# HengyiWang/spann3r

Measured on AMD Instinct MI355X. Metric: frames/sec/GPU (224px, 10-frame seq) + mem-bank cross-attn HBM GB/s, higher is better.
Workload: dtype bf16; 1 GPU; Spann3R.forward, 10-frame 224x224 sequence, batch 1, ViT-L enc / ViT-B dec / DPT heads, eval memory policy; parallelism=sequences sharded 1/GPU x1, hip_graphs=True

## Files before the change

include/spann3r_hip.h:

```cpp
#ifndef SPANN3R_HIP_H
#define SPANN3R_HIP_H

#include <stdint.h>

#ifdef __cplusplus
extern "C" {
#endif

enum { SP3_F32 = 0, SP3_BF16 = 1 };
enum { SP3_ACT_NONE = 0, SP3_ACT_GELU = 1, SP3_ACT_RELU = 2 };
enum { SP3_EPI_PLAIN = 0, SP3_EPI_ROPE_VT = 1, SP3_EPI_PIXSHUF = 2, SP3_EPI_PARTIAL = 3 };
enum { SP3_LOAD_PLAIN = 0, SP3_LOAD_CONV3X3 = 1, SP3_LOAD_SOFTMAX = 2 };

const char* sp3_last_error(void);
int sp3_version(void);

typedef struct sp3_gemm_desc {
  const float* A;
  const float* A2;
  const void* W;
  void* C;
  const float* bias;
  const float* res1;
  const float* res2;
  int32_t M, N, K;
  int32_t batch;
  int32_t K1;
  int64_t lda, lda2, ldw, ldc, ldr1, ldr2;
  int64_t strideA, strideW, strideC;
  float alpha;
  int32_t wdtype;
  int32_t act;
  int32_t out_bf16;
  int32_t relu_in;
  int32_t loader;
  int32_t conv_H, conv_W, conv_C, conv_OH, conv_OW, conv_stride;
  int32_t epi;
  const float* rope_cos;
  const float* rope_sin;
  const int32_t* pos;
  int32_t rope_cols;
  void* vt;
  int32_t tokens;
  int32_t heads;
  int64_t vt_ld;
  int32_t ps_k, ps_H, ps_W, ps_C;
  int32_t tile;
  int32_t a_bf16;
  int32_t splitk;
  int32_t a_packed;
  const float* ln_stats;
  const float* ln_s;
  int32_t ln_nt;
  int32_t ln_C;
  float ln_eps;
  float* stats_out;
  void* c2;
  int32_t qkv_packed;
  int32_t out_packed;
  int32_t w_packed;
  int64_t sb_A2, sb_bias, sb_ln_stats, sb_ln_s, sb_stats_out, sb_c2, sb_vt;
  int64_t* trace;
  float* sm_stats_out;
  const float* sm_stats;
  int32_t sm_nt;
  float sm_thresh;
  float* sm_zout;
  int32_t f32x3;
  int32_t res_bf16;
  const int32_t* dyn_n;
  int32_t res2_up_H, res2_up_W;
} sp3_gemm_desc;
int sp3_gemm(const sp3_gemm_desc* desc_host, void* stream);
int sp3_gemm_n(const sp3_gemm_desc* const* descs, int n, void* stream);
int sp3_gemm_plan_n(const sp3_gemm_desc* const* descs, int n, int* tiles);
int sp3_gemm_plan(const sp3_gemm_desc* desc_host);

int sp3_layernorm(const float* x, int64_t ldx, const float* gamma, const float* beta, float eps,
                  void* out, int64_t ldo, int out_bf16, int rows, int C, void* stream);
int sp3_layernorm_packed(const float* x, int64_t ldx, const float* gamma, const float* beta, float eps,
                         void* out, int out_bf16, int rows, int C, void* stream);
int sp3_layernorm_dual(const float* x, int64_t ldx, const float* gamma, const float* beta, float eps, float* out, int64_t ldo,
                       void* out_packed_bf16, int rows, int C, int group_rows, int group_rows_pad, void* stream);
int sp3_layernorm_t(const float* x, int64_t ldx, const float* gamma, const float* beta, float eps,
                    void* out, int64_t ldo, int out_bf16, int rows, int C, void* stream);

typedef struct sp3_reduce_ln_desc {
  const float* partial;
  int64_t split_stride;
  const float* bias;
  const float* res;
  int64_t ldres;
  float* x_out;
  int64_t ldx;
  const float* g1; const float* b1; void* out1; int64_t ld1; int32_t out1_bf16;
  const float* g2; const float* b2; void* out2; int64_t ld2; int32_t out2_bf16;
  float eps;
  int32_t splits, rows, C;
  int32_t out1_packed, out2_packed;
  int32_t act;
  const float* res2;
  int64_t ldres2;
} sp3_reduce_ln_desc;
int sp3_reduce_ln(const sp3_reduce_ln_desc* desc_host, void* stream);

int sp3_rope_2d(void* tokens, int dtype, int B, int N, int H, int D, int64_t sB, int64_t sN, int64_t sH,
                const int64_t* positions, float base, float fwd, void* stream);

int sp3_attention(const void* q, int64_t sq, int64_t ldq, const void* k, int64_t sk, int64_t ldk,
                  const void* vt, int64_t vt_ld, void* out, int64_t ldo, int out_bf16,
                  int B, int heads, int Nq, int Nk, float scale, int dtype, void* stream);
int sp3_attention_ex(const void* q, int64_t sq, int64_t ldq, const void* k, int64_t sk, int64_t ldk,
                     const void* vt, int64_t vt_ld, void* out, int64_t ldo, int out_bf16, int out_packed,
                     int B, int heads, int Nq, int Nk, float scale, int dtype, void* stream);

int sp3_attention_packed(const void* qp, int q_cols, int q_col0, int npad_q, const void* kp, int k_cols, int k_col0, int npad_k,
                         const void* vtp, void* out, int64_t ldo, int out_bf16, int out_packed,
                         int B, int heads, int Nq, int Nk, float scale, int o_group, int o_group_rows, void* stream);

typedef struct sp3_attn_qproj_desc {
  const void* x_packed; int64_t x_group_stride;
  const float* ln_stats; int64_t stats_group_stride;
  const void* w_packed; int64_t w_group_stride;
  const float* ln_s; const float* bias; int64_t vec_group_stride;
  const int32_t* pos; const float* rope_cos; const float* rope_sin;
  float ln_eps; int32_t D;
  const void* kp; int32_t k_cols, k_col0, npad_k; const void* vtp;
  void* out; int64_t ldo; int32_t out_bf16, out_packed;
  int32_t B, heads, Nq, Nk; float scale; int32_t o_group, o_group_rows;
} sp3_attn_qproj_desc;
int sp3_attention_packed_qproj(const sp3_attn_qproj_desc* desc_host, void* stream);

typedef struct sp3_bank_write_desc {
  const float* feat_k;
  const float* feat_v;
  float* k_raw;
  float* v_raw;
  void* k_hat;
  void* v_hat_t;
  float* s_bank;
  float* b_bank;
  const float *gamma_k, *beta_k, *gamma_v, *beta_v, *gamma_q, *beta_q;
  float eps;
  float alpha;
  int32_t M, P, C, cap;
  int32_t wdtype;
  const int32_t* state;
} sp3_bank_write_desc;
int sp3_bank_write(const sp3_bank_write_desc* desc_host, void* stream);
int sp3_softmax_thresh(const float* S, float* P, int64_t ld, int64_t strideS, int rows, int M, int Mpad,
                       float thresh, int batch, void* P_packed, int64_t stride_packed, int packed_bf16, void* stream);
int sp3_softmax_pack(const float* S, int64_t ld, int64_t strideS, int rows, int M, float thresh, int batch, void* P_packed,
                     int64_t stride_packed, int packed_bf16, float* rowstat_ws, void* stream);
int sp3_colsum_accum(const float* P, int64_t ld, int rows, int M, float* mem_attn, void* stream);
int sp3_colsum_packed(const void* P_packed, int packed_bf16, int rows, int M, float* mem_attn, void* stream);
int sp3_colsum_softmax(const float* S, int64_t ld, int rows, int M, const float* rowz, float thresh, float* mem_attn,
                       float* mem_count, int append_P, void* stream);
int sp3_pack_stats(const float* x, int64_t ldx, int rows, int C, void* packed, int packed_bf16, float* stats, void* stream);
int sp3_gather_packed_rows(const void* src, void* dst, const int32_t* sel, int n_sel, int C, int elem_size, void* stream);
int sp3_gather_packed_cols(const void* src, void* dst, const int32_t* sel, int n_sel, int n_fill, int C, int cap,
                           int elem_size, void* stream);
int sp3_cos_sim(const float* k, const float* wm, int T, int P, int C, float* scratch, float* score, void* stream);
int sp3_bank_state_set(int32_t* state, int M, int wm, void* stream);
int sp3_prob_merge(const float* stats, float* scale, int rows, int M, int cap, const int32_t* dyn_n, void* stream);
int sp3_colsum_prob(const void* P_packed, const float* scale, int rows, int M, int cap, const int32_t* dyn_n, float* mem_attn, void* stream);
int sp3_cos_sim_state(const float* k, const float* k_raw, int Tmax, int P, int C, const int32_t* state, float* scratch, float* score,
                      void* stream);
int sp3_mem_append(float* count, float* attn, int M, int P, void* stream);
int sp3_prune_select(const float* attn, const float* count, int M, float protect, int top_k,
                     int32_t* sel, void* stream);
int sp3_gather_rows(const void* src, void* dst, const int32_t* sel, int n_sel, int C, int elem_size, void* stream);
int sp3_gather_cols(const void* src, int64_t ld_src, void* dst, int64_t ld_dst, const int32_t* sel, int n_sel,
                    int n_fill, int C, int elem_size, void* stream);
int sp3_gather_1d(const float* src, float* dst, const int32_t* sel, int n_sel, void* stream);

int sp3_conv3x3_tile(const void* x, int in_bf16, const void* w_packed, const float* bias, const float* res1,
                     const float* res2, void* out, int out_bf16, int B, int H, int W, int Cin, int Cout,
                     int relu_in, int act, void* stream);
int sp3_im2col_patch(const float* img, int64_t sb, int64_t sc, int64_t sy, int64_t sx, int B, int C, int H, int W,
                     int p, void* out, int out_bf16, int out_packed, void* stream);
int sp3_upsample2x(const float* in, float* out, int B, int H, int W, int C, int outH, int outW, void* stream);
int sp3_upsample2x_bf16(const void* in, void* out, int B, int H, int W, int C, int outH, int outW, void* stream);
int sp3_head_final(const float* feat, const float* w, const float* b, int64_t pixels, int C, float* pts,
                   float* conf, float* raw, void* stream);
int sp3_head_final_bf16(const void* feat, const float* w, const float* b, int64_t pixels, int C, float* pts, float* conf,
                        float* raw, void* stream);

int sp3_preprocess_image(const uint8_t* src, int64_t src_row_stride, int crop_l, int crop_t, int H1, int W1,
                         const int32_t* hbounds, const int32_t* hcoef, int hksize, int W2,
                         const int32_t* vbounds, const int32_t* vcoef, int vksize, int H2,
                         int crop2_l, int crop2_t, int outW, int outH, int transpose, uint8_t* tmp, float* out, void* stream);

int64_t sp3_conf_loss_ws_bytes(int n, int B);
int sp3_conf_loss_forward(const float* P, const float* Cf, const float* G, const uint8_t* V, const float* pose0, int n, int B, int HW,
                          float alpha, int fix_first, void* ws, float* out7, float* ent_out, void* stream);
int sp3_conf_loss_backward(const float* P, const float* Cf, const float* G, const uint8_t* V, const float* pose0, int n, int B, int HW,
                           float alpha, int fix_first, const void* ws, const float* grad_scale2, float* dP, float* dC, void* stream);
int64_t sp3_ssi_loss_ws_bytes(int n, int B, int HW);
int sp3_ssi_loss_forward(const float* P, const float* G, const uint8_t* V, const float* pose0, int n, int B, int HW, int fix_first,
                         int gt_scale, void* ws, float* out, void* stream);

int sp3_transpose(const float* src, int64_t ld_src, float* dst, int64_t ld_dst, int rows, int cols, void* stream);
int sp3_transpose_batched(const float* src, int64_t ld_src, int64_t stride_src, float* dst, int64_t ld_dst, int64_t stride_dst, int rows,
                          int cols, int batch, void* stream);
int sp3_transpose_pad(const float* src, int64_t ld_src, int64_t stride_src, float* dst, int64_t ld_dst, int64_t stride_dst, int rows,
                      int cols, int batch, int pad_to, void* stream);
int sp3_gelu(const float* x, float* y, int64_t n, void* stream);
int sp3_gelu_bwd(const float* x, const float* dy, float* dx, int64_t n, void* stream);
int sp3_im2col3x3(const float* x, float* col, int B, int H, int W, int C, int stride, void* stream);
int sp3_col2im3x3(const float* dcol, float* dx, int B, int H, int W, int C, int stride, void* stream);
int sp3_relu(const float* x, float* y, int64_t n, void* stream);
int sp3_relu_bwd(const float* x, const float* dy, float* dx, int64_t n, void* stream);
int sp3_upsample2x_bwd(const float* dy, float* dx, int B, int H, int W, int C, int outH, int outW, void* stream);
int sp3_postprocess(const float* raw, float* pts, float* conf, int64_t M, void* stream);
int sp3_postprocess_bwd(const float* raw, const float* dpts, const float* dconf, float* draw, int64_t M, void* stream);
int sp3_adamw(float* p, const float* g, float* m, float* v, int64_t n, float lr, float beta1, float beta2, float eps, float weight_decay,
              int step, float grad_scale, void* stream);
int sp3_mul(const float* a, const float* b, float* out, int64_t n, void* stream);
int sp3_pack_bf16(const float* src, int64_t ld, int rows, int cols, void* dst, void* dstT, void* stream);
int sp3_pack_bf16_conv3x3(const float* x, int B, int H, int W, int C, int stride, int act, void* dst, void* dstT, void* stream);
int sp3_pack_bf16_act(const float* src, int64_t ld, int rows, int cols, void* dst, void* dstT, int act, void* stream);
int sp3_pack_bf16_colsum(const float* src, int64_t ld, int rows, int cols, void* dst, void* dstT, float* colsum, int accumulate,
                         float* partial_ws, void* stream);
int64_t sp3_sumsq_blocks(int64_t n);
int64_t sp3_colsum_rows_ws(int rows, int N);
int sp3_colsum_rows(const float* x, int64_t ld, int rows, int N, float* out, int accumulate, float* scratch, void* stream);
int sp3_sumsq_partial(const float* g, int64_t n, double* partial, void* stream);
int sp3_clip_coef(const double* partial, int count, float max_norm, float extra_scale, float* out, int* step_counter, void* stream);
int sp3_adamw_flat(float* p, const float* g, float* m, float* v, int64_t n, const float* chunk_table, float lr, float beta1, float beta2,
                   float eps, int step, const float* grad_scale_dev, float grad_scale, const int* step_dev, const float* lr_dev, void* stream);
int sp3_softmax_bwd(const float* A, const float* dAd, const float* mask, float* dS, int64_t ld, int rows, int T, float alpha, void* stream);
int sp3_softmax_bwd_pad(const float* A, const float* dAd, const float* mask, float* dS, int64_t ld, int rows, int T, int Tpad, float alpha,
                        void* stream);
typedef struct sp3_head_part {
  const float* src;
  int64_t s_b, s_n, s_h;
  float* dst;
  int64_t d_b, d_n, d_h;
  float* dstT;
  const int64_t* pos;
  int32_t N;
  float fwd;
  int64_t ldT;
} sp3_head_part;
int sp3_head_shuffle(const sp3_head_part* parts, int nparts, int B, int H, int hd, float rope_base, const float* cos_tab,
                     const float* sin_tab, int tab_len, void* stream);
int sp3_attention_train_fwd(const float* q, int64_t sq, int64_t ldq, const float* k, int64_t sk, int64_t ldk, const float* vt, int64_t vt_ld,
                            float* out, int64_t ldo, float* lse, int B, int heads, int Nq, int Nk, float scale, int bf16_products, void* stream);
typedef struct sp3_attn_bwd_desc {
  const float *q, *k, *v, *dout;
  int64_t sq, ldq, sk, ldk, sv, ldv, sdo, lddo;
  const float *qT, *kT, *doT;
  int64_t ldTq, ldTk;
  const float* lse;
  float* D;
  float *dq, *dk, *dv;
  int64_t sdq, lddq, sdk, lddk, sdv, lddv;
  int32_t B, heads, Nq, Nk;
  float scale;
  int32_t bf16_products;
} sp3_attn_bwd_desc;
int sp3_attention_train_bwd(const sp3_attn_bwd_desc* d, void* stream);
int sp3_layernorm_bwd(const float* x, int64_t ldx, const float* gamma, const float* dy, int64_t ldy, const float* dx_add, int64_t ld_add,
                      float* dx, int64_t ld_dx, float* dgamma, float* dbeta, int accumulate, float* scratch, int rows, int C, float eps,
                      void* stream);

int sp3_focal_weiszfeld(const float* pts3d, int B, int H, int W, float ppx, float ppy, int iters, float focal_min, float focal_max,
                        float* focal, void* stream);
int sp3_conf_filter(const float* conf, const float* pts, const float* rgb, int64_t n, float thresh, int* scratch, int64_t* total,
                    float* out_pts, float* out_rgb, void* stream);

int sp3_pnp_dlt_accum(const float* pts, int F, int H, int W, float focal, float cx, float cy, const float* norm4, const float* Rt,
                      float thresh, int cv_mode, double* out41, void* stream);
int sp3_pnp_gn_accum(const float* pts, int F, int H, int W, float focal, float cx, float cy, const double* Rt, const float* Rt_mask,
                     float thresh, double* out29, void* stream);
int sp3_pnp_score(const float* pts, int F, int H, int W, float focal, float cx, float cy, const float* Rt, int n_hyp, float thresh,
                  int cv_mode, int* counts, void* stream);

int sp3_copy_multi(int n, const void* const* src, void* const* dst, const int64_t* bytes, void* stream);
int sp3_copy2d_f32(const float* src, int64_t lds, float* dst, int64_t ldd, int rows, int cols, void* stream);
int sp3_fill_f32(float* p, float v, int64_t n, void* stream);
int sp3_cast_f32_to_bf16(const float* src, void* dst, int64_t n, void* stream);
int sp3_spin(int64_t cycles, int64_t* ticks_100mhz, void* stream);

#ifdef __cplusplus
}
#endif
#endif
```

spann3r_amd/csrc/dpt.hip:

```cpp
#include "common.h"
#include <math.h>

namespace {

__global__ __launch_bounds__(256) void im2col_patch_kernel(const float* __restrict__ img, int64_t sb, int64_t sc, int64_t sy,
                                                           int64_t sx, int C, int H, int W, int p, void* __restrict__ out,
                                                           int out_bf16, int out_packed, int64_t total) {
  const int64_t idx = (int64_t)blockIdx.x * 256 + threadIdx.x;
  if (idx >= total) return;
  const int K = C * p * p;
  const int64_t row = idx / K;
  const int k = (int)(idx - row * K);
  const int nw = W / p, nh = H / p;
  const int b = (int)(row / (nh * nw));
  const int rem = (int)(row - (int64_t)b * nh * nw);
  const int ty = rem / nw, tx = rem - ty * nw;
  const int c = k / (p * p), r2 = k - c * p * p;
  const int iy = r2 / p, ix = r2 - iy * p;
  const float val = img[b * sb + c * sc + (int64_t)(ty * p + iy) * sy + (int64_t)(tx * p + ix) * sx];
  const int64_t o = out_packed ? packed_off((int)row, k, K, out_bf16 != 0) : idx;
  if (out_bf16) reinterpret_cast<__bf16*>(out)[o] = (__bf16)val;
  else reinterpret_cast<float*>(out)[o] = val;
}

__device__ __forceinline__ float4 ld4(const float* p) { return *reinterpret_cast<const float4*>(p); }
__device__ __forceinline__ float4 ld4(const __bf16* p) {
  const bf16x4 t = *reinterpret_cast<const bf16x4*>(p);
  return make_float4((float)t[0], (float)t[1], (float)t[2], (float)t[3]);
}
__device__ __forceinline__ void st4(float* p, const float4 v) { st_out(reinterpret_cast<float4*>(p), v); }
__device__ __forceinline__ void st4(__bf16* p, const float4 v) {
  bf16x4 t;
  t[0] = (__bf16)v.x; t[1] = (__bf16)v.y; t[2] = (__bf16)v.z; t[3] = (__bf16)v.w;
  st_out(reinterpret_cast<bf16x4*>(p), t);
}

template <typename T>
__global__ __launch_bounds__(256) void upsample2x_kernel(const T* __restrict__ in, T* __restrict__ out, int H, int W,
                                                         int C, int outH, int outW, int64_t total4) {
  const int64_t idx = (int64_t)blockIdx.x * 256 + threadIdx.x;
  if (idx >= total4) return;
  const int c4 = C >> 2;
  const int cc = (int)(idx % c4);
  int64_t pix = idx / c4;
  const int ox = (int)(pix % outW);
  pix /= outW;
  const int oy = (int)(pix % outH);
  const int b = (int)(pix / outH);
  const int OH = 2 * H, OW = 2 * W;
  const float sh = OH > 1 ? (float)(H - 1) / (float)(OH - 1) : 0.f;
  const float sw = OW > 1 ? (float)(W - 1) / (float)(OW - 1) : 0.f;
  const float fy = sh * (float)oy, fx = sw * (float)ox;
  int y0 = (int)fy, x0 = (int)fx;
  y0 = y0 < H - 1 ? y0 : H - 1;
  x0 = x0 < W - 1 ? x0 : W - 1;
  const int y1 = y0 < H - 1 ? y0 + 1 : y0, x1 = x0 < W - 1 ? x0 + 1 : x0;
  const float ly = fy - (float)y0, lx = fx - (float)x0;
  const float hy = 1.f - ly, hx = 1.f - lx;
  const T* base = in + (int64_t)b * H * W * C;
  const float4 v00 = ld4(base + (((int64_t)y0 * W + x0) * c4 + cc) * 4);
  const float4 v01 = ld4(base + (((int64_t)y0 * W + x1) * c4 + cc) * 4);
  const float4 v10 = ld4(base + (((int64_t)y1 * W + x0) * c4 + cc) * 4);
  const float4 v11 = ld4(base + (((int64_t)y1 * W + x1) * c4 + cc) * 4);
  float4 o;
  o.x = hy * (hx * v00.x + lx * v01.x) + ly * (hx * v10.x + lx * v11.x);
  o.y = hy * (hx * v00.y + lx * v01.y) + ly * (hx * v10.y + lx * v11.y);
  o.z = hy * (hx * v00.z + lx * v01.z) + ly * (hx * v10.z + lx * v11.z);
  o.w = hy * (hx * v00.w + lx * v01.w) + ly * (hx * v10.w + lx * v11.w);
  st4(out + idx * 4, o);
}

__global__ __launch_bounds__(256) void upsample2x_bf16x8_kernel(const __bf16* __restrict__ in, __bf16* __restrict__ out, int H, int W,
                                                                int C, int outH, int outW) {
  const int c8 = C >> 3;
  const int t = blockIdx.x * 256 + threadIdx.x;
  if (t >= outW * c8) return;
  const int ox = t / c8, cg = t - ox * c8;
  const int oy = blockIdx.y, b = blockIdx.z;
  const int OH = 2 * H, OW = 2 * W;
  const float sh = OH > 1 ? (float)(H - 1) / (float)(OH - 1) : 0.f;
  const float sw = OW > 1 ? (float)(W - 1) / (float)(OW - 1) : 0.f;
  const float fy = sh * (float)oy, fx = sw * (float)ox;
  int y0 = (int)fy, x0 = (int)fx;
  y0 = y0 < H - 1 ? y0 : H - 1;
  x0 = x0 < W - 1 ? x0 : W - 1;
  const int y1 = y0 < H - 1 ? y0 + 1 : y0, x1 = x0 < W - 1 ? x0 + 1 : x0;
  const float ly = fy - (float)y0, lx = fx - (float)x0;
  const float hy = 1.f - ly, hx = 1.f - lx;
  const __bf16* base = in + (int64_t)b * H * W * C + cg * 8;
  const bf16x8 v00 = *reinterpret_cast<const bf16x8*>(base + ((int64_t)y0 * W + x0) * C);
  const bf16x8 v01 = *reinterpret_cast<const bf16x8*>(base + ((int64_t)y0 * W + x1) * C);
  const bf16x8 v10 = *reinterpret_cast<const bf16x8*>(base + ((int64_t)y1 * W + x0) * C);
  const bf16x8 v11 = *reinterpret_cast<const bf16x8*>(base + ((int64_t)y1 * W + x1) * C);
  bf16x8 o;
#pragma unroll
  for (int e = 0; e < 8; ++e)
    o[e] = (__bf16)(hy * (hx * (float)v00[e] + lx * (float)v01[e]) + ly * (hx * (float)v10[e] + lx * (float)v11[e]));
  st_out(reinterpret_cast<bf16x8*>(out + (((int64_t)b * outH + oy) * outW + ox) * C + cg * 8), o);
}

template <typename T>
__global__ __launch_bounds__(256) void head_final_kernel(const T* __restrict__ feat, const float* __restrict__ w,
                                                         const float* __restrict__ bias, int64_t pixels, int C,
                                                         float* __restrict__ pts, float* __restrict__ conf,
                                                         float* __restrict__ raw) {
  const int64_t gid = (int64_t)blockIdx.x * 256 + threadIdx.x;
  const int64_t pix = gid >> 3;
  const int sub = (int)(gid & 7);
  const bool valid = pix < pixels;
  const int64_t pp = valid ? pix : pixels - 1;
  float a0 = 0.f, a1 = 0.f, a2 = 0.f, a3 = 0.f;
  const T* f = feat + pp * C;
  for (int c = sub * 4; c < C; c += 32) {
    const float4 x = ld4(f + c);
    const float4 w0 = *reinterpret_cast<const float4*>(w + c);
    const float4 w1 = *reinterpret_cast<const float4*>(w + C + c);
    const float4 w2 = *reinterpret_cast<const float4*>(w + 2 * C + c);
    const float4 w3 = *reinterpret_cast<const float4*>(w + 3 * C + c);
    a0 += (x.x * w0.x + x.y * w0.y) + (x.z * w0.z + x.w * w0.w);
    a1 += (x.x * w1.x + x.y * w1.y) + (x.z * w1.z + x.w * w1.w);
    a2 += (x.x * w2.x + x.y * w2.y) + (x.z * w2.z + x.w * w2.w);
    a3 += (x.x * w3.x + x.y * w3.y) + (x.z * w3.z + x.w * w3.w);
  }
#pragma unroll
  for (int o = 1; o < 8; o <<= 1) {
    a0 += __shfl_xor(a0, o); a1 += __shfl_xor(a1, o); a2 += __shfl_xor(a2, o); a3 += __shfl_xor(a3, o);
  }
  if (valid && sub == 0) {
    const float x = a0 + bias[0], y = a1 + bias[1], z = a2 + bias[2], c = a3 + bias[3];
    if (raw) { raw[pix * 4 + 0] = x; raw[pix * 4 + 1] = y; raw[pix * 4 + 2] = z; raw[pix * 4 + 3] = c; }
    const float d = sqrtf(x * x + y * y + z * z);
    const float sc = expm1f(d) / fmaxf(d, 1e-8f);
    pts[pix * 3 + 0] = x * sc; pts[pix * 3 + 1] = y * sc; pts[pix * 3 + 2] = z * sc;
    conf[pix] = 1.0f + expf(c);
  }
}

template <int LP, int PPT>
__global__ __launch_bounds__(256) void head_final_bf16x8_kernel(const __bf16* __restrict__ feat, const float* __restrict__ w,
                                                                const float* __restrict__ bias, int64_t pixels, float* __restrict__ pts,
                                                                float* __restrict__ conf, float* __restrict__ raw) {
  constexpr int C = 8 * LP, PPB = 256 / LP;
  const int li = threadIdx.x % LP, pl = threadIdx.x / LP;
  float wr[4][8];
#pragma unroll
  for (int f = 0; f < 4; ++f) {
    const float4 a = *reinterpret_cast<const float4*>(w + f * C + li * 8), b = *reinterpret_cast<const float4*>(w + f * C + li * 8 + 4);
    wr[f][0] = a.x; wr[f][1] = a.y; wr[f][2] = a.z; wr[f][3] = a.w; wr[f][4] = b.x; wr[f][5] = b.y; wr[f][6] = b.z; wr[f][7] = b.w;
  }
  const float b0 = bias[0], b1 = bias[1], b2 = bias[2], b3 = bias[3];
  const int64_t p0 = (int64_t)blockIdx.x * PPB * PPT + pl;
  bf16x8 x[PPT];
#pragma unroll
  for (int q = 0; q < PPT; ++q) {
    int64_t pix = p0 + (int64_t)q * PPB;
    pix = pix < pixels ? pix : pixels - 1;
    x[q] = *reinterpret_cast<const bf16x8*>(feat + pix * C + li * 8);
  }
#pragma unroll
  for (int q = 0; q < PPT; ++q) {
    const int64_t pix = p0 + (int64_t)q * PPB;
    float a[4];
#pragma unroll
    for (int f = 0; f < 4; ++f) {
      float t0 = 0.f, t1 = 0.f;
#pragma unroll
      for (int e = 0; e < 4; ++e) { t0 = fmaf((float)x[q][e], wr[f][e], t0); t1 = fmaf((float)x[q][4 + e], wr[f][4 + e], t1); }
      a[f] = t0 + t1;
    }
#pragma unroll
    for (int o = 1; o < LP; o <<= 1) {
      a[0] += __shfl_xor(a[0], o); a[1] += __shfl_xor(a[1], o); a[2] += __shfl_xor(a[2], o); a[3] += __shfl_xor(a[3], o);
    }
    if (li == 0 && pix < pixels) {
      const float X = a[0] + b0, Y = a[1] + b1, Z = a[2] + b2, Cc = a[3] + b3;
      if (raw) *reinterpret_cast<float4*>(raw + pix * 4) = make_float4(X, Y, Z, Cc);
      const float d = sqrtf(X * X + Y * Y + Z * Z);
      const float sc = expm1f(d) / fmaxf(d, 1e-8f);
      pts[pix * 3 + 0] = X * sc; pts[pix * 3 + 1] = Y * sc; pts[pix * 3 + 2] = Z * sc;
      conf[pix] = 1.0f + expf(Cc);
    }
  }
}

}

#define ST(s) reinterpret_cast<hipStream_t>(s)

extern "C" int sp3_im2col_patch(const float* img, int64_t sb, int64_t sc, int64_t sy, int64_t sx, int B, int C, int H, int W,
                                int p, void* out, int out_bf16, int out_packed, void* stream) {
  SP3_CHECK(img && out && B > 0 && C > 0 && p > 0, "sp3_im2col_patch: bad arguments");
  SP3_CHECK(H % p == 0 && W % p == 0, "Input image size (%d,%d) is not a multiple of patch size (%d)", H, W, p);
  const int64_t total = (int64_t)B * (H / p) * (W / p) * C * p * p;
  hipLaunchKernelGGL(im2col_patch_kernel, dim3((unsigned)((total + 255) / 256)), dim3(256), 0, ST(stream), img, sb, sc, sy, sx,
                     C, H, W, p, out, out_bf16, out_packed, total);
  SP3_LAUNCH_CHECK("sp3_im2col_patch");
  return 0;
}

extern "C" int sp3_upsample2x(const float* in, float* out, int B, int H, int W, int C, int outH, int outW, void* stream) {
  SP3_CHECK(in && out && B > 0 && H > 0 && W > 0 && C > 0 && C % 4 == 0, "sp3_upsample2x: bad arguments");
  SP3_CHECK(outH > 0 && outH <= 2 * H && outW > 0 && outW <= 2 * W, "sp3_upsample2x: bad crop");
  const int64_t total4 = (int64_t)B * outH * outW * (C / 4);
  hipLaunchKernelGGL(upsample2x_kernel<float>, dim3((unsigned)((total4 + 255) / 256)), dim3(256), 0, ST(stream), in, out, H, W, C,
                     outH, outW, total4);
  SP3_LAUNCH_CHECK("sp3_upsample2x");
  return 0;
}

extern "C" int sp3_upsample2x_bf16(const void* in, void* out, int B, int H, int W, int C, int outH, int outW, void* stream) {
  SP3_CHECK(in && out && B > 0 && H > 0 && W > 0 && C > 0 && C % 4 == 0, "sp3_upsample2x_bf16: bad arguments");
  SP3_CHECK(outH > 0 && outH <= 2 * H && outW > 0 && outW <= 2 * W, "sp3_upsample2x_bf16: bad crop");
  if (C % 8 == 0 && outH <= 65535 && B <= 65535) {
    hipLaunchKernelGGL(upsample2x_bf16x8_kernel, dim3((unsigned)((outW * (C / 8) + 255) / 256), outH, B), dim3(256), 0, ST(stream),
                       reinterpret_cast<const __bf16*>(in), reinterpret_cast<__bf16*>(out), H, W, C, outH, outW);
    SP3_LAUNCH_CHECK("sp3_upsample2x_bf16");
    return 0;
  }
  const int64_t total4 = (int64_t)B * outH * outW * (C / 4);
  hipLaunchKernelGGL(upsample2x_kernel<__bf16>, dim3((unsigned)((total4 + 255) / 256)), dim3(256), 0, ST(stream),
                     reinterpret_cast<const __bf16*>(in), reinterpret_cast<__bf16*>(out), H, W, C, outH, outW, total4);
  SP3_LAUNCH_CHECK("sp3_upsample2x_bf16");
  return 0;
}

extern "C" int sp3_head_final(const float* feat, const float* w, const float* b, int64_t pixels, int C, float* pts, float* conf,
                              float* raw, void* stream) {
  SP3_CHECK(feat && w && b && pts && conf && pixels > 0 && C > 0 && C % 32 == 0, "sp3_head_final: bad arguments");
  const int64_t threads = pixels * 8;
  hipLaunchKernelGGL(head_final_kernel<float>, dim3((unsigned)((threads + 255) / 256)), dim3(256), 0, ST(stream), feat, w, b, pixels, C,
                     pts, conf, raw);
  SP3_LAUNCH_CHECK("sp3_head_final");
  return 0;
}

extern "C" int sp3_head_final_bf16(const void* feat, const float* w, const float* b, int64_t pixels, int C, float* pts, float* conf,
                                   float* raw, void* stream) {
  SP3_CHECK(feat && w && b && pts && conf && pixels > 0 && C > 0 && C % 32 == 0, "sp3_head_final_bf16: bad arguments");
  if (C == 128 && (reinterpret_cast<uintptr_t>(feat) & 15) == 0 && (reinterpret_cast<uintptr_t>(w) & 15) == 0 && (!raw || (reinterpret_cast<uintptr_t>(raw) & 15) == 0)) {
    constexpr int LP = 16, PPT = 4, PPB = 256 / LP;
    hipLaunchKernelGGL((head_final_bf16x8_kernel<LP, PPT>), dim3((unsigned)((pixels + PPB * PPT - 1) / (PPB * PPT))), dim3(256), 0, ST(stream),
                       reinterpret_cast<const __bf16*>(feat), w, b, pixels, pts, conf, raw);
    SP3_LAUNCH_CHECK("sp3_head_final_bf16");
    return 0;
  }
  const int64_t threads = pixels * 8;
  hipLaunchKernelGGL(head_final_kernel<__bf16>, dim3((unsigned)((threads + 255) / 256)), dim3(256), 0, ST(stream),
                     reinterpret_cast<const __bf16*>(feat), w, b, pixels, C, pts, conf, raw);
  SP3_LAUNCH_CHECK("sp3_head_final_bf16");
  return 0;
}
```

spann3r_amd/csrc/memory.hip:

```cpp
#include "common.h"
#include <math.h>

namespace {

__device__ __forceinline__ float block_reduce_max(float v, float* sh) {
  v = wave_max(v);
  const int lane = threadIdx.x & 63, w = threadIdx.x >> 6;
  __syncthreads();
  if (lane == 0) sh[w] = v;
  __syncthreads();
  float r = sh[0];
  for (int i = 1; i < (int)(blockDim.x >> 6); ++i) r = fmaxf(r, sh[i]);
  return r;
}
__device__ __forceinline__ float block_reduce_sum(float v, float* sh) {
  v = wave_sum(v);
  const int lane = threadIdx.x & 63, w = threadIdx.x >> 6;
  __syncthreads();
  if (lane == 0) sh[w] = v;
  __syncthreads();
  float r = sh[0];
  for (int i = 1; i < (int)(blockDim.x >> 6); ++i) r += sh[i];
  return r;
}
// ... 8 lines not shown
  for (int j = threadIdx.x; j < M; j += 256) {
    const float v = s[j];
    if (v > mx) { sum = sum * expf(mx - v) + 1.0f; mx = v; }
    else sum += expf(v - mx);
  }
  const float gmx = block_reduce_max(mx, sh);
  sum = block_reduce_sum(mx == -INFINITY ? 0.f : sum * expf(mx - gmx), sh);
  mx = gmx;
  float inv = 1.0f / sum, rk = 1.0f;
  if (thresh > 0.f) {
    float kept = 0.f;
    for (int j = threadIdx.x; j < M; j += 256) {
      float v = expf(s[j] - mx) * inv;
      v = v < thresh ? 0.f : v;
      kept += v;
    }
    rk = block_reduce_sum(kept, sh);
  }
  auto prob = [&](int j) -> float {
    float v = expf(s[j] - mx) * inv;
    if (thresh > 0.f) v = (v < thresh ? 0.f : v) / rk;
    return v;
  };
  if (P) {
    float* p = P + (int64_t)blockIdx.y * strideS + (int64_t)blockIdx.x * ld;
    for (int j = threadIdx.x; j < M; j += 256) p[j] = prob(j);
    for (int j = M + threadIdx.x; j < Mpad; j += 256) p[j] = 0.f;
  }
  if (Pk) {
    constexpr int E = 16 / (int)sizeof(TP);
    TP* pk = Pk + (int64_t)blockIdx.y * stridePk;
    const int row = blockIdx.x;
    for (int j0 = threadIdx.x * E; j0 < Kp; j0 += 256 * E) {
      TP o[E];
#pragma unroll
      for (int e = 0; e < E; ++e) o[e] = (TP)((j0 + e) < M ? prob(j0 + e) : 0.f);
      typedef __attribute__((ext_vector_type(4))) unsigned int u4;
      *reinterpret_cast<u4*>(pk + packed_off(row, j0, Kp, sizeof(TP) == 2)) = *reinterpret_cast<const u4*>(o);
    }
  }
}

__global__ __launch_bounds__(256) void softmax_rowstat_kernel(const float* __restrict__ S, int64_t ld, int64_t strideS, int rows, int M, float thresh,
                                                              float4* __restrict__ rowstat) {
  __shared__ float sh[8];
  const float* s = S + (int64_t)blockIdx.y * strideS + (int64_t)blockIdx.x * ld;
  const bool vec = ((ld & 3) == 0) && ((reinterpret_cast<uintptr_t>(S) & 15) == 0) && ((strideS & 3) == 0);
  const int M4 = vec ? (M & ~3) : 0;
  float mx = -INFINITY, sum = 0.f;
  auto upd = [&](float v) {
    if (v > mx) { sum = sum * __expf(mx - v) + 1.0f; mx = v; }
    else sum += __expf(v - mx);
  };
  for (int j = threadIdx.x * 4; j < M4; j += 1024) {
    const float4 v = *reinterpret_cast<const float4*>(s + j);
    const float m4 = fmaxf(fmaxf(v.x, v.y), fmaxf(v.z, v.w));
    if (m4 > mx) { sum *= __expf(mx - m4); mx = m4; }
    sum += (__expf(v.x - mx) + __expf(v.y - mx)) + (__expf(v.z - mx) + __expf(v.w - mx));
  }
  for (int j = M4 + threadIdx.x; j < M; j += 256) upd(s[j]);
  const float gmx = block_reduce_max(mx, sh);
  sum = block_reduce_sum(mx == -INFINITY ? 0.f : sum * __expf(mx - gmx), sh);
  const float inv = 1.0f / sum;
  float rk = 1.0f;
  if (thresh > 0.f) {
    float kept = 0.f;
    for (int j = threadIdx.x * 4; j < M4; j += 1024) {
      const float4 v = *reinterpret_cast<const float4*>(s + j);
      const float p[4] = {__expf(v.x - gmx) * inv, __expf(v.y - gmx) * inv, __expf(v.z - gmx) * inv, __expf(v.w - gmx) * inv};
#pragma unroll
      for (int e = 0; e < 4; ++e) kept += p[e] < thresh ? 0.f : p[e];
    }
    for (int j = M4 + threadIdx.x; j < M; j += 256) { const float p = __expf(s[j] - gmx) * inv; kept += p < thresh ? 0.f : p; }
    rk = 1.0f / block_reduce_sum(kept, sh);
  }
  if (threadIdx.x == 0) rowstat[(int64_t)blockIdx.y * rows + blockIdx.x] = make_float4(gmx, inv, rk, 0.f);
}

template <typename TP>
__global__ __launch_bounds__(256) void softmax_pack_kernel(const float* __restrict__ S, int64_t ld, int64_t strideS, int rows, int M, int Kp,
                                                           float thresh, const float4* __restrict__ rowstat, TP* __restrict__ Pk,
                                                           int64_t stridePk) {
  constexpr int E = 16 / (int)sizeof(TP), KB = 8 * E;
  const int t = threadIdx.x & 127, kb = blockIdx.x * 2 + (threadIdx.x >> 7), nkb = Kp / KB;
  if (kb >= nkb) return;
  const int h = t >> 6, g = (t >> 4) & 3, r = t & 15;
  const int row = blockIdx.y * 16 + r;
  const int k0 = kb * KB + g * 2 * E + h * E;
  float p[E];
#pragma unroll
  for (int e = 0; e < E; ++e) p[e] = 0.f;
  if (row < rows && k0 < M) {
    const float* s = S + (int64_t)blockIdx.z * strideS + (int64_t)row * ld + k0;
    const float4 st = rowstat[(int64_t)blockIdx.z * rows + row];
    float v[E];
    if (k0 + E <= M && ((reinterpret_cast<uintptr_t>(s) & 15) == 0)) {
#pragma unroll
      for (int q = 0; q < E / 4; ++q) {
        const float4 x = reinterpret_cast<const float4*>(s)[q];
        v[4 * q] = x.x; v[4 * q + 1] = x.y; v[4 * q + 2] = x.z; v[4 * q + 3] = x.w;
      }
    } else {
#pragma unroll
      for (int e = 0; e < E; ++e) v[e] = (k0 + e) < M ? s[e] : -INFINITY;
    }
#pragma unroll
    for (int e = 0; e < E; ++e) {
      float q = __expf(v[e] - st.x) * st.y;
      if (thresh > 0.f) q = (q < thresh ? 0.f : q) * st.z;
      p[e] = (k0 + e) < M ? q : 0.f;
    }
  }
  TP o[E];
#pragma unroll
  for (int e = 0; e < E; ++e) o[e] = (TP)p[e];
  typedef __attribute__((ext_vector_type(4))) unsigned int u4;
  TP* dst = Pk + (int64_t)blockIdx.z * stridePk + (((int64_t)blockIdx.y * nkb + kb) * 128 + t) * E;
  *reinterpret_cast<u4*>(dst) = *reinterpret_cast<const u4*>(o);
}

template <typename TP>
__global__ __launch_bounds__(256) void colsum_packed_kernel(const TP* __restrict__ Pk, int rows, int M, int Kp,
                                                            float* __restrict__ mem_attn) {
  constexpr int E = 16 / (int)sizeof(TP), KB = 8 * E, TPB = 2048 / 16;
  __shared__ float sh[2][KB][17];
  const int kb = blockIdx.x, nkb = Kp / KB, nrb = (rows + 15) / 16;
  const int t = threadIdx.x & (TPB - 1), half_wg = threadIdx.x / TPB;
  const int h = t >> 6, l = t & 63, g = l >> 4, r = l & 15;
  float acc[E];
#pragma unroll
  for (int e = 0; e < E; ++e) acc[e] = 0.f;
  for (int rb = half_wg; rb < nrb; rb += 2) {
    typedef __attribute__((ext_vector_type(4))) unsigned int u4;
    const u4 raw = *reinterpret_cast<const u4*>(reinterpret_cast<const char*>(Pk) + ((int64_t)rb * nkb + kb) * 2048 + t * 16);
    const TP* v = reinterpret_cast<const TP*>(&raw);
    const bool ok = rb * 16 + r < rows;
#pragma unroll
    for (int e = 0; e < E; ++e) acc[e] += ok ? (float)v[e] : 0.f;
  }
#pragma unroll
  for (int e = 0; e < E; ++e) sh[half_wg][g * 2 * E + h * E + e][r] = acc[e];
  __syncthreads();
  if (threadIdx.x < KB) {
    const int j = kb * KB + threadIdx.x;
    float sum = 0.f;
#pragma unroll
    for (int q = 0; q < 2; ++q)
#pragma unroll
      for (int rr = 0; rr < 16; ++rr) sum += sh[q][threadIdx.x][rr];
    if (j < M) mem_attn[j] += sum;
  }
}

__global__ __launch_bounds__(1024) void colsum_softmax_kernel(const float* __restrict__ S, int64_t ld, int rows, int M,
                                                              const float4* __restrict__ rowz, float thr, float* __restrict__ mem_attn,
                                                              float* __restrict__ mem_count, int app_P) {
  __shared__ float sh[16][64];
  const int lane = threadIdx.x & 63, w = threadIdx.x >> 6;
  const int j = blockIdx.x * 64 + lane;
  const int jc = j < M ? j : M - 1;
  float acc = 0.f;
  for (int r0 = w; r0 < rows && blockIdx.x * 64 < M; r0 += 16 * 8) {
    float sv[8];
    float4 rz[8];
#pragma unroll
    for (int c = 0; c < 8; ++c) {
      const int r = r0 + 16 * c, rc = r < rows ? r : rows - 1;
      sv[c] = S[(int64_t)rc * ld + jc];
      rz[c] = rowz[rc];
    }
#pragma unroll
    for (int c = 0; c < 8; ++c) {
      const float p = __expf(sv[c] - rz[c].y) * rz[c].z;
      acc += (p < thr || r0 + 16 * c >= rows) ? 0.f : p / rz[c].x;
    }
  }
  sh[w][lane] = acc;
  __syncthreads();
  if (w == 0 && j < M) {
    float t = 0.f;
#pragma unroll
    for (int q = 0; q < 16; ++q) t += sh[q][lane];
    mem_attn[j] += t;
  }
  if (w == 0 && app_P > 0) {
    if (j < M) mem_count[j] += 1.0f;
    else if (j < M + app_P) { mem_count[j] = 0.f; mem_attn[j] = 0.f; }
  }
}

__global__ __launch_bounds__(256) void colsum_accum_kernel(const float* __restrict__ P, int64_t ld, int rows, int M,
                                                           float* __restrict__ mem_attn) {
  __shared__ float sh[4][64];
  const int lane = threadIdx.x & 63, w = threadIdx.x >> 6;
  const int j = blockIdx.x * 64 + lane;
  float s0 = 0.f, s1 = 0.f;
  if (j < M) {
    int r = w;
    for (; r + 4 < rows; r += 8) { s0 += P[(int64_t)r * ld + j]; s1 += P[(int64_t)(r + 4) * ld + j]; }
    if (r < rows) s0 += P[(int64_t)r * ld + j];
  }
  sh[w][lane] = s0 + s1;
  __syncthreads();
  if (w == 0 && j < M) mem_attn[j] += (sh[0][lane] + sh[1][lane]) + (sh[2][lane] + sh[3][lane]);
}

__global__ __launch_bounds__(256) void cos_pair_kernel(const float* __restrict__ k, const float* __restrict__ wm, int TP, int P, int C,
                                                       float* __restrict__ cosv, const int* __restrict__ state) {
  const int lane = threadIdx.x & 63, j = blockIdx.x * 4 + (threadIdx.x >> 6);
  if (state) {
    const int M = state[0], T = state[1];
    TP = T * P < TP ? T * P : TP;
    wm += (int64_t)(M - TP) * C;
  }
  if (j >= TP) return;
  const float* a = k + (int64_t)(j % P) * C;
  const float* b = wm + (int64_t)j * C;
  float dot = 0.f, na = 0.f, nb = 0.f;
  for (int c = lane * 4; c < C; c += 256) {
    const float4 x = *reinterpret_cast<const float4*>(a + c);
    const float4 y = *reinterpret_cast<const float4*>(b + c);
    dot += (x.x * y.x + x.y * y.y) + (x.z * y.z + x.w * y.w);
    na += (x.x * x.x + x.y * x.y) + (x.z * x.z + x.w * x.w);
    nb += (y.x * y.x + y.y * y.y) + (y.z * y.z + y.w * y.w);
  }
  dot = wave_sum(dot); na = wave_sum(na); nb = wave_sum(nb);
  if (lane == 0) cosv[j] = dot / (fmaxf(sqrtf(na), 1e-12f) * fmaxf(sqrtf(nb), 1e-12f));
}

__global__ __launch_bounds__(256) void cos_mean_kernel(const float* __restrict__ cosv, int P, float* __restrict__ score, const int* __restrict__ state) {
  __shared__ float sh[4];
  const int t = blockIdx.x, lane = threadIdx.x & 63, w = threadIdx.x >> 6;
  if (state && t >= state[1]) return;
  float acc = 0.f;
  for (int p = threadIdx.x; p < P; p += 256) acc += cosv[(int64_t)t * P + p];
  acc = wave_sum(acc);
  if (lane == 0) sh[w] = acc;
  __syncthreads();
  if (threadIdx.x == 0) score[t] = ((sh[0] + sh[1]) + (sh[2] + sh[3])) / (float)P;
}

__global__ __launch_bounds__(1024) void prob_merge_kernel(const float2* __restrict__ stats, float* __restrict__ scale, int rows, long rows_pad,
                                                          int Mk, const int* __restrict__ dyn) {
  __shared__ float red[64][17];
  __shared__ float rowm[16], rowiz[16];
  const int r = threadIdx.x & 15, gl = threadIdx.x >> 4, row = blockIdx.x * 16 + r;
  if (dyn) Mk = dyn[0];
  const int ng = (Mk + 63) >> 6;
  const float2* st = stats + row;
  float mx = -INFINITY;
  for (int gq = gl; gq < ng; gq += 64) mx = fmaxf(mx, st[(long)gq * rows_pad].x);
  red[gl][r] = mx;
  __syncthreads();
  if (gl == 0) {
    float m = red[0][r];
#pragma unroll 8
    for (int j = 1; j < 64; ++j) m = fmaxf(m, red[j][r]);
    rowm[r] = m;
  }
  __syncthreads();
  const float m = rowm[r];
  float z = 0.f;
  for (int gq = gl; gq < ng; gq += 64) {
    const float2 v = st[(long)gq * rows_pad];
    z += v.y * __expf(v.x - m);
  }
  __syncthreads();
  red[gl][r] = z;
  __syncthreads();
  if (gl == 0) {
    float t = 0.f;
#pragma unroll 8
    for (int j = 0; j < 64; ++j) t += red[j][r];
    rowiz[r] = 1.0f / t;
  }
  __syncthreads();
  const float iz = row < rows ? rowiz[r] : 0.f;
  for (int gq = gl; gq < ng; gq += 64) scale[(long)gq * rows_pad + row] = row < rows ? __expf(st[(long)gq * rows_pad].x - m) * iz : 0.f;
}

__global__ __launch_bounds__(256) void colsum_prob_kernel(const __bf16* __restrict__ P, const float* __restrict__ scale, int rows, long rows_pad,
                                                          int nkbc, int Mk, const int* __restrict__ dyn, float* __restrict__ mem_attn) {
  __shared__ float part[4][64];
  if (dyn) Mk = dyn[0];
  const int kb = blockIdx.x;
  if (kb * 64 >= Mk) return;
  const int lane = threadIdx.x & 63, w = threadIdx.x >> 6, g = lane >> 4, r = lane & 15;
  const int nrb = (rows + 15) >> 4;
  float sum[16];
#pragma unroll
  for (int e = 0; e < 16; ++e) sum[e] = 0.f;
  for (int rb = w; rb < nrb; rb += 4) {
    const __bf16* piece = P + ((long)rb * nkbc + kb) * 1024 + lane * 8;
    const bf16x8 p0 = *reinterpret_cast<const bf16x8*>(piece), p1 = *reinterpret_cast<const bf16x8*>(piece + 512);
    const float sc = scale[(long)kb * rows_pad + rb * 16 + r];
#pragma unroll
    for (int e = 0; e < 8; ++e) {
      sum[e] = fmaf(sc, (float)p0[e], sum[e]);
      sum[8 + e] = fmaf(sc, (float)p1[e], sum[8 + e]);
    }
  }
#pragma unroll
  for (int e = 0; e < 16; ++e) {
    float v = sum[e];
    v += __shfl_xor(v, 1); v += __shfl_xor(v, 2); v += __shfl_xor(v, 4); v += __shfl_xor(v, 8);
    if (r == 0) part[w][g * 16 + e] = v;
  }
  __syncthreads();
  if (threadIdx.x < 64) {
    const int key = kb * 64 + threadIdx.x;
    if (key < Mk) mem_attn[key] += (part[0][threadIdx.x] + part[1][threadIdx.x]) + (part[2][threadIdx.x] + part[3][threadIdx.x]);
  }
}

__global__ void bank_state_kernel(int* __restrict__ state, int M, int wm) {
  if (threadIdx.x == 0) { state[0] = M; state[1] = wm; }
}

__global__ __launch_bounds__(256) void mem_append_kernel(float* __restrict__ count, float* __restrict__ attn, int M, int P) {
  const int j = blockIdx.x * 256 + threadIdx.x;
  if (j < M) count[j] += 1.0f;
  else if (j < M + P) { count[j] = 0.f; attn[j] = 0.f; }
}

struct CopyMultiArgs { const char* src[8]; char* dst[8]; int64_t bytes[8]; };
__global__ __launch_bounds__(256) void copy_multi_kernel(const CopyMultiArgs a) {
  const int e = blockIdx.y;
  const int64_t n16 = a.bytes[e] >> 4;
  const uint4* s = reinterpret_cast<const uint4*>(a.src[e]);
  uint4* d = reinterpret_cast<uint4*>(a.dst[e]);
  for (int64_t i = (int64_t)blockIdx.x * 256 + threadIdx.x; i < n16; i += (int64_t)gridDim.x * 256) d[i] = s[i];
}

constexpr int PRUNE_MAX = 16384;
__global__ __launch_bounds__(1024) void prune_select_kernel(const float* __restrict__ attn, const float* __restrict__ count,
                                                            int M, float protect, int top_k, int32_t* __restrict__ sel) {
  extern __shared__ __attribute__((aligned(16))) unsigned char raw[];
  float* w = reinterpret_cast<float*>(raw);
  int32_t* id = reinterpret_cast<int32_t*>(raw + PRUNE_MAX * sizeof(float));
  int n = 1;
  while (n < M) n <<= 1;
  for (int j = threadIdx.x; j < n; j += 1024) {
    if (j < M) {
      const float c = count[j];
      w[j] = c < protect ? 1e8f : attn[j] / c;
      id[j] = j;
    } else {
      w[j] = -INFINITY;
      id[j] = 0x7fffffff;
    }
  }
  __syncthreads();
  for (int k = 2; k <= n; k <<= 1) {
    for (int s = k >> 1; s > 0; s >>= 1) {
      for (int j = threadIdx.x; j < n; j += 1024) {
        const int l = j ^ s;
        if (l > j) {
          const float wj = w[j], wl = w[l];
          const int ij = id[j], il = id[l];
          const bool j_first = (wj > wl) || (wj == wl && ij < il);
          const bool up = (j & k) == 0;
          if (up != j_first) { w[j] = wl; w[l] = wj; id[j] = il; id[l] = ij; }
        }
      }
      __syncthreads();
    }
  }
  for (int j = threadIdx.x; j < top_k; j += 1024) sel[j] = id[j];
}

template <typename T>
__global__ __launch_bounds__(256) void gather_rows_kernel(const T* __restrict__ src, T* __restrict__ dst,
                                                          const int32_t* __restrict__ sel, int C) {
  const int i = blockIdx.x;
  const T* s = src + (int64_t)sel[i] * C;
  T* d = dst + (int64_t)i * C;
  for (int c = threadIdx.x; c < C; c += 256) d[c] = s[c];
}

template <typename T>
__global__ __launch_bounds__(256) void gather_cols_kernel(const T* __restrict__ src, int64_t ld_src, T* __restrict__ dst,
                                                          int64_t ld_dst, const int32_t* __restrict__ sel, int n_sel, int n_fill) {
  const int c = blockIdx.y;
  const int i = blockIdx.x * 256 + threadIdx.x;
  if (i < n_sel) dst[(int64_t)c * ld_dst + i] = src[(int64_t)c * ld_src + sel[i]];
  else if (i < n_fill) dst[(int64_t)c * ld_dst + i] = (T)0.f;
}

__global__ __launch_bounds__(256) void gather_1d_kernel(const float* __restrict__ src, float* __restrict__ dst,
                                                        const int32_t* __restrict__ sel, int n) {
  const int i = blockIdx.x * 256 + threadIdx.x;
  if (i < n) dst[i] = src[sel[i]];
}

__global__ __launch_bounds__(256) void fill_kernel(float* __restrict__ p, float v, int64_t n) {
  const int64_t i = (int64_t)blockIdx.x * 256 + threadIdx.x;
  if (i < n) p[i] = v;
}

__global__ __launch_bounds__(256) void copy2d_kernel(const float* __restrict__ s, int64_t lds, float* __restrict__ d, int64_t ldd,
                                                     int cols4, int64_t total4) {
  const int64_t i = (int64_t)blockIdx.x * 256 + threadIdx.x;
  if (i >= total4) return;
  const int64_t r = i / cols4;
  const int c = (int)(i - r * cols4);
  reinterpret_cast<float4*>(d + r * ldd)[c] = reinterpret_cast<const float4*>(s + r * lds)[c];
}

__global__ __launch_bounds__(256) void cast_bf16_kernel(const float* __restrict__ s, __bf16* __restrict__ d, int64_t n) {
  const int64_t i = (int64_t)blockIdx.x * 256 + threadIdx.x;
  if (i < n) d[i] = (__bf16)s[i];
}


struct BankWriteArgs {
  const float *fk, *fv;
  float *k_raw, *v_raw;
  void *k_hat, *v_hat_t;
  float *s_bank, *b_bank;
  const float *gk, *bk, *gv, *bv, *gq, *bq;
  float eps, alpha;
  int M, P, C, cap;
  const int* state;
};

template <typename TW>
__global__ __launch_bounds__(128 * (16 / (int)sizeof(TW))) void bank_write_kernel(const BankWriteArgs a) {
  constexpr int TG = 16 / (int)sizeof(TW), NTH = 128 * TG;
  constexpr bool BF = sizeof(TW) == 2;
  extern __shared__ __attribute__((aligned(16))) unsigned char raw_[];
  TW* stage = reinterpret_cast<TW*>(raw_);
  const int lane = threadIdx.x & 63, wave = threadIdx.x >> 6;
  const int M0 = a.state ? __builtin_amdgcn_readfirstlane(a.state[0]) : a.M;
  const int t0 = (M0 / TG + blockIdx.x) * TG;
  const int C = a.C;
  {
    const int j = wave % TG;
    const bool is_key = wave < TG;
    const int t = t0 + j;
    const bool live = t >= M0 && t < M0 + a.P;
    const int pr = t - M0;
    if (live && is_key) {
      const float* x = a.fk + (int64_t)pr * C;
      float s1 = 0.f, s2 = 0.f;
      for (int c = lane * 4; c < C; c += 256) {
        const float4 v = *reinterpret_cast<const float4*>(x + c);
        *reinterpret_cast<float4*>(a.k_raw + (int64_t)t * C + c) = v;
        s1 += (v.x + v.y) + (v.z + v.w);
        s2 += (v.x * v.x + v.y * v.y) + (v.z * v.z + v.w * v.w);
      }
      s1 = wave_sum(s1); s2 = wave_sum(s2);
      const float mean = s1 / (float)C;
      const float rstd = 1.0f / sqrtf(fmaxf(s2 / (float)C - mean * mean, 0.f) + a.eps);
      float ss = 0.f, sb = 0.f;
      for (int c = lane * 4; c < C; c += 256) {
        const float4 v = *reinterpret_cast<const float4*>(x + c);
        const float4 g = *reinterpret_cast<const float4*>(a.gk + c), be = *reinterpret_cast<const float4*>(a.bk + c);
        const float4 gq = *reinterpret_cast<const float4*>(a.gq + c), bq = *reinterpret_cast<const float4*>(a.bq + c);
        const float kh[4] = {(v.x - mean) * rstd * g.x + be.x, (v.y - mean) * rstd * g.y + be.y,
                             (v.z - mean) * rstd * g.z + be.z, (v.w - mean) * rstd * g.w + be.w};
        const float gqa[4] = {gq.x, gq.y, gq.z, gq.w}, bqa[4] = {bq.x, bq.y, bq.z, bq.w};
        TW w[4];
#pragma unroll
        for (int e = 0; e < 4; ++e) {
          w[e] = (TW)(kh[e] * gqa[e]);
          ss += (float)w[e];
          sb += bqa[e] * kh[e];
        }
        TW* dst = reinterpret_cast<TW*>(a.k_hat) + packed_off(t, c, C, BF);
        if constexpr (BF) {
          bf16x4 o4;
          o4[0] = w[0]; o4[1] = w[1]; o4[2] = w[2]; o4[3] = w[3];
          *reinterpret_cast<bf16x4*>(dst) = o4;
        } else {
#pragma unroll
          for (int e = 0; e < 4; ++e) dst[e] = w[e];
        }
      }
      ss = wave_sum(ss); sb = wave_sum(sb);
      if (lane == 0) { a.s_bank[t] = a.alpha * ss; a.b_bank[t] = a.alpha * sb; }
    }
    if (live && !is_key) {
      const float* x = a.fv + (int64_t)pr * C;
      float s1 = 0.f, s2 = 0.f;
// ... 106 lines not shown
  float4* rs = reinterpret_cast<float4*>(rowstat_ws);
  hipLaunchKernelGGL(softmax_rowstat_kernel, dim3(rows, batch), dim3(256), 0, ST(stream), S, ld, strideS, rows, M, thresh, rs);
  const int KB = packed_bf16 ? 64 : 32, Kp = (M + KB - 1) / KB * KB, nkb = Kp / KB, nrb = (rows + 15) / 16;
  const dim3 grid((nkb + 1) / 2, nrb, batch);
  if (packed_bf16) hipLaunchKernelGGL(softmax_pack_kernel<__bf16>, grid, dim3(256), 0, ST(stream), S, ld, strideS, rows, M, Kp, thresh, rs,
                                      reinterpret_cast<__bf16*>(P_packed), stride_packed);
  else hipLaunchKernelGGL(softmax_pack_kernel<float>, grid, dim3(256), 0, ST(stream), S, ld, strideS, rows, M, Kp, thresh, rs,
                          reinterpret_cast<float*>(P_packed), stride_packed);
  SP3_LAUNCH_CHECK("sp3_softmax_pack");
  return 0;
}

extern "C" int sp3_colsum_packed(const void* P_packed, int packed_bf16, int rows, int M, float* mem_attn, void* stream) {
  SP3_CHECK(P_packed && mem_attn && rows > 0 && M > 0, "sp3_colsum_packed: bad arguments");
  if (packed_bf16) {
    const int Kp = (M + 63) / 64 * 64;
    hipLaunchKernelGGL(colsum_packed_kernel<__bf16>, dim3(Kp / 64), dim3(256), 0, ST(stream), (const __bf16*)P_packed, rows, M, Kp, mem_attn);
  } else {
    const int Kp = (M + 31) / 32 * 32;
    hipLaunchKernelGGL(colsum_packed_kernel<float>, dim3(Kp / 32), dim3(256), 0, ST(stream), (const float*)P_packed, rows, M, Kp, mem_attn);
  }
  SP3_LAUNCH_CHECK("sp3_colsum_packed");
  return 0;
}

extern "C" int sp3_colsum_softmax(const float* S, int64_t ld, int rows, int M, const float* rowz, float thresh, float* mem_attn,
                                  float* mem_count, int append_P, void* stream) {
  SP3_CHECK(S && rowz && mem_attn && rows > 0 && M > 0 && ld >= M, "sp3_colsum_softmax: bad arguments");
  SP3_CHECK((reinterpret_cast<uintptr_t>(rowz) & 15) == 0, "sp3_colsum_softmax: rowz must be 16-byte aligned");
  SP3_CHECK(append_P == 0 || (append_P > 0 && mem_count), "sp3_colsum_softmax: append needs mem_count");
  hipLaunchKernelGGL(colsum_softmax_kernel, dim3((M + append_P + 63) / 64), dim3(1024), 0, ST(stream), S, ld, rows, M,
                     reinterpret_cast<const float4*>(rowz), thresh, mem_attn, mem_count, append_P);
  SP3_LAUNCH_CHECK("sp3_colsum_softmax");
  return 0;
}

extern "C" int sp3_bank_write(const sp3_bank_write_desc* dp, void* stream) {
  SP3_CHECK(dp != nullptr, "sp3_bank_write: null descriptor");
  const sp3_bank_write_desc& d = *dp;
  SP3_CHECK(d.feat_k && d.feat_v && d.k_raw && d.v_raw && d.k_hat && d.v_hat_t && d.s_bank && d.b_bank, "sp3_bank_write: null pointer");
  SP3_CHECK(d.gamma_k && d.beta_k && d.gamma_v && d.beta_v && d.gamma_q && d.beta_q, "sp3_bank_write: null LayerNorm parameter");
  SP3_CHECK(d.P > 0 && d.C > 0 && d.C % 256 == 0 && d.cap % 64 == 0 && (d.state ? d.P <= d.cap : (d.M >= 0 && d.M + d.P <= d.cap)),
            "sp3_bank_write: bad geometry M=%d P=%d C=%d cap=%d", d.M, d.P, d.C, d.cap);
  SP3_CHECK(d.wdtype == SP3_F32 || d.wdtype == SP3_BF16, "sp3_bank_write: bad wdtype %d", d.wdtype);
  BankWriteArgs a{d.feat_k, d.feat_v, d.k_raw, d.v_raw, d.k_hat, d.v_hat_t, d.s_bank, d.b_bank, d.gamma_k, d.beta_k,
                  d.gamma_v, d.beta_v, d.gamma_q, d.beta_q, d.eps, d.alpha, d.M, d.P, d.C, d.cap, d.state};
  const int TG = d.wdtype == SP3_BF16 ? 8 : 4;
  const int groups = d.state ? (d.P + TG - 1) / TG + 1 : (d.M + d.P + TG - 1) / TG - d.M / TG;
  const size_t lds = (size_t)TG * d.C * (d.wdtype == SP3_BF16 ? 2 : 4);
  if (d.wdtype == SP3_BF16) hipLaunchKernelGGL(bank_write_kernel<__bf16>, dim3(groups), dim3(1024), lds, ST(stream), a);
  else hipLaunchKernelGGL(bank_write_kernel<float>, dim3(groups), dim3(512), lds, ST(stream), a);
  SP3_LAUNCH_CHECK("sp3_bank_write");
  return 0;
}

extern "C" int sp3_pack_stats(const float* x, int64_t ldx, int rows, int C, void* packed, int packed_bf16, float* stats, void* stream) {
  SP3_CHECK(x && packed && stats && rows > 0 && C > 0 && C % 256 == 0 && ldx % 4 == 0, "sp3_pack_stats: bad arguments");
  if (packed_bf16) hipLaunchKernelGGL(pack_stats_kernel<__bf16>, dim3((rows + 3) / 4), dim3(256), 0, ST(stream), x, ldx, rows, C, (__bf16*)packed, stats);
  else hipLaunchKernelGGL(pack_stats_kernel<float>, dim3((rows + 3) / 4), dim3(256), 0, ST(stream), x, ldx, rows, C, (float*)packed, stats);
  SP3_LAUNCH_CHECK("sp3_pack_stats");
  return 0;
}

extern "C" int sp3_gather_packed_rows(const void* src, void* dst, const int32_t* sel, int n_sel, int C, int elem_size, void* stream) {
  SP3_CHECK(src && dst && sel && n_sel > 0 && C > 0 && C % 64 == 0 && (elem_size == 2 || elem_size == 4), "sp3_gather_packed_rows: bad arguments");
  hipLaunchKernelGGL(gather_packed_rows_kernel, dim3(n_sel), dim3(256), 0, ST(stream), (const char*)src, (char*)dst, sel, C, elem_size);
  SP3_LAUNCH_CHECK("sp3_gather_packed_rows");
  return 0;
}

extern "C" int sp3_gather_packed_cols(const void* src, void* dst, const int32_t* sel, int n_sel, int n_fill, int C, int cap,
                                      int elem_size, void* stream) {
  SP3_CHECK(src && dst && sel && n_sel > 0 && C > 0 && C % 16 == 0 && cap % 64 == 0 && n_fill <= cap && n_sel <= n_fill,
            "sp3_gather_packed_cols: bad arguments");
  const int TG = 16 / elem_size;
  dim3 grid((n_fill / TG + 255) / 256, C);
  if (elem_size == 2)
    hipLaunchKernelGGL(gather_packed_cols_kernel<__bf16>, grid, dim3(256), 0, ST(stream), (const __bf16*)src, (__bf16*)dst, sel, n_sel, n_fill, cap);
  else if (elem_size == 4)
    hipLaunchKernelGGL(gather_packed_cols_kernel<float>, grid, dim3(256), 0, ST(stream), (const float*)src, (float*)dst, sel, n_sel, n_fill, cap);
  else SP3_CHECK(false, "sp3_gather_packed_cols: elem_size %d", elem_size);
  SP3_LAUNCH_CHECK("sp3_gather_packed_cols");
  return 0;
}

extern "C" int sp3_colsum_accum(const float* P, int64_t ld, int rows, int M, float* mem_attn, void* stream) {
  SP3_CHECK(P && mem_attn && rows > 0 && M > 0, "sp3_colsum_accum: bad arguments");
  hipLaunchKernelGGL(colsum_accum_kernel, dim3((M + 63) / 64), dim3(256), 0, ST(stream), P, ld, rows, M, mem_attn);
  SP3_LAUNCH_CHECK("sp3_colsum_accum");
  return 0;
}

extern "C" int sp3_cos_sim(const float* k, const float* wm, int T, int P, int C, float* scratch, float* score, void* stream) {
  SP3_CHECK(k && wm && scratch && score && T > 0 && P > 0 && C > 0 && C % 4 == 0, "sp3_cos_sim: bad arguments");
  hipLaunchKernelGGL(cos_pair_kernel, dim3((T * P + 3) / 4), dim3(256), 0, ST(stream), k, wm, T * P, P, C, scratch, (const int*)nullptr);
  hipLaunchKernelGGL(cos_mean_kernel, dim3(T), dim3(256), 0, ST(stream), scratch, P, score, (const int*)nullptr);
  SP3_LAUNCH_CHECK("sp3_cos_sim");
  return 0;
}

extern "C" int sp3_cos_sim_state(const float* k, const float* k_raw, int Tmax, int P, int C, const int32_t* state, float* scratch, float* score,
                                 void* stream) {
  SP3_CHECK(k && k_raw && state && scratch && score && Tmax > 0 && P > 0 && C > 0 && C % 4 == 0, "sp3_cos_sim_state: bad arguments");
  hipLaunchKernelGGL(cos_pair_kernel, dim3((Tmax * P + 3) / 4), dim3(256), 0, ST(stream), k, k_raw, Tmax * P, P, C, scratch, state);
  hipLaunchKernelGGL(cos_mean_kernel, dim3(Tmax), dim3(256), 0, ST(stream), scratch, P, score, state);
  SP3_LAUNCH_CHECK("sp3_cos_sim_state");
  return 0;
}

extern "C" int sp3_prob_merge(const float* stats, float* scale, int rows, int M, int cap, const int32_t* dyn_n, void* stream) {
  SP3_CHECK(stats && scale && rows > 0 && M > 0 && cap % 64 == 0 && M <= cap, "sp3_prob_merge: bad arguments");
  const long rows_pad = (long)((rows + 255) & ~255);
  hipLaunchKernelGGL(prob_merge_kernel, dim3((unsigned)(rows_pad / 16)), dim3(1024), 0, ST(stream), reinterpret_cast<const float2*>(stats), scale, rows,
                     rows_pad, M, dyn_n);
  SP3_LAUNCH_CHECK("sp3_prob_merge");
  return 0;
}

extern "C" int sp3_colsum_prob(const void* P_packed, const float* scale, int rows, int M, int cap, const int32_t* dyn_n, float* mem_attn, void* stream) {
  SP3_CHECK(P_packed && scale && mem_attn && rows > 0 && M > 0 && cap % 64 == 0 && M <= cap, "sp3_colsum_prob: bad arguments");
  const long rows_pad = (long)((rows + 255) & ~255);
  hipLaunchKernelGGL(colsum_prob_kernel, dim3((unsigned)((M + 63) / 64)), dim3(256), 0, ST(stream), reinterpret_cast<const __bf16*>(P_packed), scale, rows,
                     rows_pad, cap / 64, M, dyn_n, mem_attn);
  SP3_LAUNCH_CHECK("sp3_colsum_prob");
  return 0;
}

extern "C" int sp3_bank_state_set(int32_t* state, int M, int wm, void* stream) {
  SP3_CHECK(state && M >= 0 && wm >= 0, "sp3_bank_state_set: bad arguments");
  hipLaunchKernelGGL(bank_state_kernel, dim3(1), dim3(64), 0, ST(stream), state, M, wm);
  SP3_LAUNCH_CHECK("sp3_bank_state_set");
  return 0;
}

extern "C" int sp3_copy_multi(int n, const void* const* src, void* const* dst, const int64_t* bytes, void* stream) {
  SP3_CHECK(n >= 1 && n <= 8 && src && dst && bytes, "sp3_copy_multi: 1..8 copies");
  CopyMultiArgs a;
  int64_t mx = 0;
  for (int i = 0; i < 8; ++i) {
    const int j = i < n ? i : 0;
    SP3_CHECK(src[j] && dst[j] && bytes[j] > 0 && bytes[j] % 16 == 0 &&
              ((reinterpret_cast<uintptr_t>(src[j]) | reinterpret_cast<uintptr_t>(dst[j])) & 15) == 0,
              "sp3_copy_multi: copy %d must be non-empty, 16-byte aligned and a multiple of 16 bytes", j);
    a.src[i] = reinterpret_cast<const char*>(src[j]); a.dst[i] = reinterpret_cast<char*>(dst[j]); a.bytes[i] = bytes[j];
    mx = bytes[j] > mx ? bytes[j] : mx;
  }
  int64_t bx = (mx / 16 + 256 * 4 - 1) / (256 * 4);
  bx = bx < 1 ? 1 : (bx > 1024 ? 1024 : bx);
  hipLaunchKernelGGL(copy_multi_kernel, dim3((unsigned)bx, n), dim3(256), 0, ST(stream), a);
  SP3_LAUNCH_CHECK("sp3_copy_multi");
  return 0;
}

extern "C" int sp3_mem_append(float* count, float* attn, int M, int P, void* stream) {
  SP3_CHECK(count && attn && M >= 0 && P > 0, "sp3_mem_append: bad arguments");
  hipLaunchKernelGGL(mem_append_kernel, dim3((M + P + 255) / 256), dim3(256), 0, ST(stream), count, attn, M, P);
  SP3_LAUNCH_CHECK("sp3_mem_append");
  return 0;
}

extern "C" int sp3_prune_select(const float* attn, const float* count, int M, float protect, int top_k, int32_t* sel,
                                void* stream) {
  SP3_CHECK(attn && count && sel, "sp3_prune_select: null pointer");
  SP3_CHECK(M > 0 && M <= PRUNE_MAX && top_k > 0 && top_k <= M, "sp3_prune_select: M=%d top_k=%d (M <= %d)", M, top_k, PRUNE_MAX);
  static bool raised = false;
  if (!raised) {
    hipError_t e = hipFuncSetAttribute(reinterpret_cast<const void*>(prune_select_kernel), hipFuncAttributeMaxDynamicSharedMemorySize, PRUNE_MAX * 8);
    SP3_CHECK(e == hipSuccess, "sp3_prune_select: cannot raise dynamic LDS: %s", hipGetErrorString(e));
    raised = true;
  }
  hipLaunchKernelGGL(prune_select_kernel, dim3(1), dim3(1024), PRUNE_MAX * 8, ST(stream), attn, count, M, protect, top_k, sel);
  SP3_LAUNCH_CHECK("sp3_prune_select");
  return 0;
}

extern "C" int sp3_gather_rows(const void* src, void* dst, const int32_t* sel, int n_sel, int C, int elem_size, void* stream) {
  SP3_CHECK(src && dst && sel && n_sel > 0 && C > 0, "sp3_gather_rows: bad arguments");
  if (elem_size == 4)
    hipLaunchKernelGGL(gather_rows_kernel<float>, dim3(n_sel), dim3(256), 0, ST(stream), (const float*)src, (float*)dst, sel, C);
  else if (elem_size == 2)
    hipLaunchKernelGGL(gather_rows_kernel<uint16_t>, dim3(n_sel), dim3(256), 0, ST(stream), (const uint16_t*)src, (uint16_t*)dst, sel, C);
  else SP3_CHECK(false, "sp3_gather_rows: elem_size %d", elem_size);
  SP3_LAUNCH_CHECK("sp3_gather_rows");
  return 0;
}

extern "C" int sp3_gather_cols(const void* src, int64_t ld_src, void* dst, int64_t ld_dst, const int32_t* sel, int n_sel,
                               int n_fill, int C, int elem_size, void* stream) {
  SP3_CHECK(src && dst && sel && n_sel > 0 && C > 0, "sp3_gather_cols: bad arguments");
  const int n = n_fill > n_sel ? n_fill : n_sel;
  dim3 grid((n + 255) / 256, C);
  if (elem_size == 4)
    hipLaunchKernelGGL(gather_cols_kernel<float>, grid, dim3(256), 0, ST(stream), (const float*)src, ld_src, (float*)dst, ld_dst, sel, n_sel, n);
  else if (elem_size == 2)
    hipLaunchKernelGGL(gather_cols_kernel<__bf16>, grid, dim3(256), 0, ST(stream), (const __bf16*)src, ld_src, (__bf16*)dst, ld_dst, sel, n_sel, n);
  else SP3_CHECK(false, "sp3_gather_cols: elem_size %d", elem_size);
  SP3_LAUNCH_CHECK("sp3_gather_cols");
  return 0;
}

extern "C" int sp3_gather_1d(const float* src, float* dst, const int32_t* sel, int n_sel, void* stream) {
  SP3_CHECK(src && dst && sel && n_sel > 0, "sp3_gather_1d: bad arguments");
  hipLaunchKernelGGL(gather_1d_kernel, dim3((n_sel + 255) / 256), dim3(256), 0, ST(stream), src, dst, sel, n_sel);
  SP3_LAUNCH_CHECK("sp3_gather_1d");
  return 0;
}

__global__ void spin_kernel(int64_t cycles, int64_t* ticks) {
  const int64_t t0 = wall_clock64();
  const int64_t c0 = clock64();
  while (clock64() - c0 < cycles) __builtin_amdgcn_s_sleep(2);
  if (threadIdx.x == 0) ticks[0] = wall_clock64() - t0;
}

extern "C" int sp3_spin(int64_t cycles, int64_t* ticks_100mhz, void* stream) {
  SP3_CHECK(ticks_100mhz && cycles >= 0, "sp3_spin: bad arguments");
  hipLaunchKernelGGL(spin_kernel, dim3(1), dim3(64), 0, ST(stream), cycles, ticks_100mhz);
  SP3_LAUNCH_CHECK("sp3_spin");
  return 0;
}

extern "C" int sp3_fill_f32(float* p, float v, int64_t n, void* stream) {
  SP3_CHECK(p && n > 0, "sp3_fill_f32: bad arguments");
  hipLaunchKernelGGL(fill_kernel, dim3((unsigned)((n + 255) / 256)), dim3(256), 0, ST(stream), p, v, n);
  SP3_LAUNCH_CHECK("sp3_fill_f32");
  return 0;
}

extern "C" int sp3_cast_f32_to_bf16(const float* src, void* dst, int64_t n, void* stream) {
  SP3_CHECK(src && dst && n > 0, "sp3_cast_f32_to_bf16: bad arguments");
  hipLaunchKernelGGL(cast_bf16_kernel, dim3((unsigned)((n + 255) / 256)), dim3(256), 0, ST(stream), src, (__bf16*)dst, n);
  SP3_LAUNCH_CHECK("sp3_cast_f32_to_bf16");
  return 0;
}

extern "C" int sp3_copy2d_f32(const float* src, int64_t lds, float* dst, int64_t ldd, int rows, int cols, void* stream) {
  SP3_CHECK(src && dst && rows > 0 && cols > 0 && cols % 4 == 0 && lds % 4 == 0 && ldd % 4 == 0, "sp3_copy2d_f32: bad arguments");
  const int64_t total4 = (int64_t)rows * (cols / 4);
  hipLaunchKernelGGL(copy2d_kernel, dim3((unsigned)((total4 + 255) / 256)), dim3(256), 0, ST(stream), src, lds, dst, ldd, cols / 4, total4);
  SP3_LAUNCH_CHECK("sp3_copy2d_f32");
  return 0;
}
```

spann3r_amd/engine.py:

```python
import math
import os

import torch

from . import ops
from .lib import ACT_NONE, ACT_GELU, ACT_RELU
from .config import Spann3RConfig


def _rope_tables(max_pos, base, device):
    half = 32
    inv_freq = 1.0 / (base ** (torch.arange(0, half, 2).float() / half))
    t = torch.arange(max_pos, dtype=torch.float32)
    ang = torch.einsum("i,j->ij", t, inv_freq)
    return ang.cos().contiguous().to(device), ang.sin().contiguous().to(device)


def _rope_tables_narrow(max_pos, base, head_dim, device):
    D = head_dim // 2
    nf = D // 2
    assert nf <= 16 and head_dim % 4 == 0
    inv_freq = 1.0 / (base ** (torch.arange(0, D, 2).float() / D))
    t = torch.arange(max_pos, dtype=torch.float32)
    ang = torch.einsum("i,j->ij", t, inv_freq)
# ... 439 lines not shown
        if f1p is not None and f2p is not None:
            dA = f2p.data_ptr() - f1p.data_ptr()
            assert dA % 16 == 0
            ops.gemm(f1p, w["dec_embed.w"], x[0], M=R, N=D, K=E, lda=E, ldc=D, bias=w["dec_embed.b"], stats_out=st[0], c2=xp[0],
                     batch=2, strideA=dA // 2, strideC=R * D, sb={"stats_out": sb_st, "c2": xp[0].stride * es})
        else:
            dA = f2.data_ptr() - f1.data_ptr()
            assert dA % 16 == 0 and f1.dtype == f2.dtype == torch.float32
            ops.gemm(f1, w["dec_embed.w"], x[0], M=R, N=D, K=E, lda=E, ldc=D, bias=w["dec_embed.b"], stats_out=st[0], c2=xp[0],
                     batch=2, strideA=dA // 4, strideC=R * D, sb={"stats_out": sb_st, "c2": xp[0].stride * es})
        rope = dict(pos=pos, cos=self.cos, sin=self.sin, tokens=P, heads=Hh, qkv_packed=True, batch=2)
        for i in range(depth):
            cur, nx = i % 2, (i + 1) % 2
            g = "decg_%d." % i
            last = i == depth - 1
            xi, xo = x[i], x[i + 1]

            def upd(A, K, pre, res, stats, c2):
                sb = {"bias": D * 4}
                if stats is not None:
                    sb["stats_out"], sb["c2"] = sb_st, c2.stride * es
                ops.gemm(A, w[g + pre + ".w"], xo, M=R, N=D, K=K, lda=K, ldc=D, bias=w[g + pre + ".b"], res1=res, ldr1=D,
                         stats_out=stats, c2=c2, batch=2, strideA=A.stride, strideW=w[g + pre + ".w"].stride, strideC=R * D, sb=sb)

            with ops.pair():
                ops.proj_rope_vt(xp[cur], w[g + "qkv.w"], w[g + "qkv.b"], qkp, 0, vtp, npad, M=R, N=3 * D, K=D, lda=D, rope_cols=2 * D,
                                 ln=ops.LnFold(st[cur], D, w[g + "qkv.s"], 1e-6, sb_stats=sb_st, sb_s=3 * D * 4),
                                 strideA=xp[cur].stride, strideW=w[g + "qkv.w"].stride, strideC=B * npad * 2 * D,
                                 sb={"bias": 3 * D * 4, "vt": sb_vt}, **rope)
                ops.proj_rope_vt(xp[cur].at(1), w[g + "ckv.w"], w[g + "ckv.b"], ckp, 0, cvtp, npad, M=R, N=2 * D, K=D, lda=D, rope_cols=D,
                                 ln=ops.LnFold(st[cur][1], D, w[g + "ckv.s"], 1e-6, sb_stats=-sb_st, sb_s=2 * D * 4),
                                 strideA=-xp[cur].stride, strideW=w[g + "ckv.w"].stride, strideC=B * npad * D,
                                 sb={"bias": 2 * D * 4, "vt": sb_vt}, **rope)
            ops.attention_packed(qkp, 2 * D, 0, npad, qkp, 2 * D, D, npad, vtp, ao, D, B=2 * B, heads=Hh, Nq=P, Nk=P,
                                 scale=64 ** -0.5, o_group=B, o_group_rows=Rp)
            upd(ao, D, "proj", xi, stq, xq)
            if self.fuse_cross_q and P < 512 and D == 768 and ops.LEAN:
                ops.attention_packed_qproj(xq, stq, w[g + "cq.w"], w[g + "cq.s"], w[g + "cq.b"], pos, self.cos, self.sin, ckp, D, 0, npad, cvtp,
                                           ao, D, B=2 * B, heads=Hh, Nq=P, Nk=P, scale=64 ** -0.5, o_group=B, o_group_rows=Rp, eps=1e-6,
                                           stats_group_stride=sb_st // 4, vec_group_stride=D)
            else:
                ops.proj_rope_vt(xq, w[g + "cq.w"], w[g + "cq.b"], cqp, 0, None, npad, M=R, N=D, K=D, lda=D, rope_cols=D,
                                 ln=ops.LnFold(stq, D, w[g + "cq.s"], 1e-6, sb_stats=sb_st, sb_s=D * 4),
                                 strideA=xq.stride, strideW=w[g + "cq.w"].stride, strideC=B * npad * D, sb={"bias": D * 4}, **rope)
                ops.attention_packed(cqp, D, 0, npad, ckp, D, 0, npad, cvtp, ao, D, B=2 * B, heads=Hh, Nq=P, Nk=P,
                                     scale=64 ** -0.5, o_group=B, o_group_rows=Rp)
            upd(ao, D, "cproj", xo, stq, xq)
            Hd = D * cfg.mlp_ratio
            ops.gemm(xq, w[g + "fc1.w"], h, M=R, N=Hd, K=D, lda=D, ldc=Hd, bias=w[g + "fc1.b"], act=ACT_GELU,
                     ln=ops.LnFold(stq, D, w[g + "fc1.s"], 1e-6, sb_stats=sb_st, sb_s=Hd * 4),
                     batch=2, strideA=xq.stride, strideW=w[g + "fc1.w"].stride, strideC=h.stride, sb={"bias": Hd * 4})
            if last:
                upd(h, Hd, "fc2", xo, None, None)
            else:
                upd(h, Hd, "fc2", xo, st[nx], xp[nx])
        normed = self.ws("decg_normed", (2, R, D))
        ops.layernorm(x[depth], w["dec_norm.w"], w["dec_norm.b"], 1e-6, normed, rows=2 * R, C_=D,
                      dual=self.wspg("decg_normed_packed", R, D) if self.adt == torch.bfloat16 else None, group_rows=R)
        outs = {}
        for s_ in (0, 1):
            outs[s_] = [(f1, f2)[s_]] + [x[l][s_].view(B, P, D) for l in range(1, depth)] + [normed[s_].view(B, P, D)]
        return outs[0], outs[1]

    def key_aux(self, R):
        E = self.cfg.enc_dim
        return self.wspg("keyg_packed", R, E), self.ws("keyg_stats", (2, R, E // 32, 2))

    def encode_feat_keys_grouped(self, feat1, feat2, normed1, normed2, R, out1, out2, feat1p=None, feat2p=None):
        self.activate()
        cfg, w = self.cfg, self.w
        E, D, Kd = cfg.enc_dim, cfg.dec_dim, cfg.key_dim
        dF, dN, dO = feat2.data_ptr() - feat1.data_ptr(), normed2.data_ptr() - normed1.data_ptr(), out2.data_ptr() - out1.data_ptr()
        assert dF % 16 == 0 and dN % 16 == 0 and dO % 16 == 0
        es = 2 if self.adt == torch.bfloat16 else 4
        h = self.wspg("keyg_hidden", R, Kd)
        packed = None
        if feat1p is not None and feat2p is not None and self.adt == torch.bfloat16 and ops.LEAN:
            np_ = self.wspg("decg_normed_packed", R, D)
            dFp = feat2p.data_ptr() - feat1p.data_ptr()
            assert dFp % 16 == 0
            packed = dict(A2=np_, lda2=D, K1=E, batch=2, strideA=dFp // 2, strideW=w["keyg.0.w"].stride, strideC=h.stride,
                          sb={"bias": Kd * 4, "A2": np_.stride * 2})
            ok = self._splitA_plan.get(R)
            if ok is None:
                ok = self._splitA_plan[R] = ops.gemm(feat1p, w["keyg.0.w"], h, M=R, N=Kd, K=Kd, lda=E, ldc=Kd, bias=w["keyg.0.b"],
                                                     act=ACT_GELU, plan_only=True, **packed) >= 30
            if not ok:
                packed = None
        if packed is not None:
            ops.gemm(feat1p, w["keyg.0.w"], h, M=R, N=Kd, K=Kd, lda=E, ldc=Kd, bias=w["keyg.0.b"], act=ACT_GELU, **packed)
        else:
            ops.gemm(feat1, w["keyg.0.w"], h, M=R, N=Kd, K=Kd, lda=E, ldc=Kd, bias=w["keyg.0.b"], act=ACT_GELU, A2=normed1, lda2=D, K1=E,
                     batch=2, strideA=dF // 4, strideW=w["keyg.0.w"].stride, strideC=h.stride, sb={"bias": Kd * 4, "A2": dN})
        kp, kst = self.key_aux(R)
        ops.gemm(h, w["keyg.2.w"], out1, M=R, N=E, K=Kd, lda=Kd, ldc=E, bias=w["keyg.2.b"], stats_out=kst, c2=kp,
                 batch=2, strideA=h.stride, strideW=w["keyg.2.w"].stride, strideC=dO // 4,
                 sb={"bias": E * 4, "stats_out": R * (E // 32) * 8, "c2": kp.stride * es})
        return kp.at(1), kst[1]

    def encode_feat_key(self, feat, dec_last, R, num, out, aux=False):
        self.activate()
        cfg, w = self.cfg, self.w
        E, D, Kd = cfg.enc_dim, cfg.dec_dim, cfg.key_dim
        h = self.wsp("key_hidden%d" % num, R, Kd)
        pre = "key%d." % num
        ops.gemm(feat, w[pre + "0.w"], h, M=R, N=Kd, K=Kd, lda=E, ldc=Kd, bias=w[pre + "0.b"], act=ACT_GELU,
                 A2=dec_last, lda2=D, K1=E)
        if aux:
            kp, kst = self.key_aux(R)
            ops.gemm(h, w[pre + "2.w"], out, M=R, N=E, K=Kd, lda=Kd, ldc=E, bias=w[pre + "2.b"], stats_out=kst[num - 1],
                     c2=kp.at(num - 1))
            return kp.at(num - 1), kst[num - 1]
        ops.gemm(h, w[pre + "2.w"], out, M=R, N=E, K=Kd, lda=Kd, ldc=E, bias=w[pre + "2.b"])
        return out

    def _conv_ws(self, head):
        return self.ws("conv_splitk_ws" + str(head), (1 << 23,))

    def _rcu_c1(self, x, pre, B, H, W_, tag=""):
        w, F = self.w, self.cfg.dpt_feat
        t = self.ws("rcu_tmp" + tag, (B * H * W_, F), self.mdt)
        ops.conv3x3(x, w[pre + "c1.w"], t, B=B, H=H, W_=W_, Cin=F, Cout=F, bias=w[pre + "c1.b"], relu_in=True, act=ACT_RELU,
                    splitk_ws=self._conv_ws(tag[:1]))
        return t

    def _rcu(self, x, pre, B, H, W_, out, extra_res=None, tag="", c1_done=False, extra_up=None):
        w, F = self.w, self.cfg.dpt_feat
        t = self.ws("rcu_tmp" + tag, (B * H * W_, F), self.mdt)
        if not c1_done:
            self._rcu_c1(x, pre, B, H, W_, tag)
        ops.conv3x3(t, w[pre + "c2.w"], out, B=B, H=H, W_=W_, Cin=F, Cout=F, bias=w[pre + "c2.b"], res1=x, res2=extra_res,
                    splitk_ws=self._conv_ws(tag[:1]), res2_up=extra_up)
        return out

    def _fusion(self, pre, B, H, W_, x0, x1, tag, crop=None, c1_done=False, x0_up=None, fold_up=False):
        w, F = self.w, self.cfg.dpt_feat
        M = B * H * W_
        cur = x0
        if x1 is not None:
            s = self.ws("fus_sum_" + tag, (M, F), self.mdt)
            self._rcu(x1, pre + "u1", B, H, W_, s, extra_res=x0, tag=tag, c1_done=c1_done, extra_up=x0_up)
            cur = s
        r = self.ws("fus_rcu2_" + tag, (M, F), self.mdt)
        self._rcu(cur, pre + "u2", B, H, W_, r, tag=tag, c1_done=c1_done and x1 is None)
        oc = self.ws("fus_oc_" + tag, (M, F), self.mdt)
        ops.gemm(r, w[pre + "out.w"], oc, M=M, N=F, K=F, lda=F, ldc=F, bias=w[pre + "out.b"])
        OH, OW = (2 * H, 2 * W_) if crop is None else crop
        if fold_up:
            return oc, OH, OW
        up = self.ws("fus_up_" + tag, (B * OH * OW, F), self.mdt)
        ops.upsample2x(oc, up, B=B, H=H, W_=W_, C_=F, outH=OH, outW=OW)
        return up, OH, OW

    def dpt_head(self, dec, B, nh, nw, num, want_raw=False):
        self.activate()
        cfg, w = self.cfg, self.w
        F, Lc = cfg.dpt_feat, cfg.dpt_last
        pre = "dpt%d." % num
        R = B * nh * nw
        hk = cfg.hooks
        dims = (cfg.enc_dim, cfg.dec_dim, cfg.dec_dim, cfg.dec_dim)
        ld = (96, 192, 384, 768)
        mdt = self.mdt
        t = [self.ws("dpt%d_pp%d" % (num, i), (R, ld[i]), mdt) for i in range(4)]
        import contextlib
        lv = ops.HEAD_LEVELS
        group = ops.level if len({dec[hk[i]].dtype for i in range(4)}) == 1 else contextlib.nullcontext
        with (group if lv else contextlib.nullcontext)():
            for i0 in (0, 2):
                with (contextlib.nullcontext if lv else group)():
                    for i in (i0, i0 + 1):
                        ops.gemm(dec[hk[i]], w[pre + "pp%d.w" % i], t[i], M=R, N=ld[i], K=dims[i], lda=dims[i], ldc=ld[i], bias=w[pre + "pp%d.b" % i])
        c0 = 128 if self.wdt == torch.bfloat16 else ld[0]
        l0 = self.ws("dpt%d_l0" % num, (B * 16 * nh * nw, c0), mdt)
        l1 = self.ws("dpt%d_l1" % num, (B * 4 * nh * nw, ld[1]), mdt)
        with group():
            ops.conv_transpose_ks(t[0], w[pre + "pp0t.w"], l0, B=B, H=nh, W_=nw, Cin=ld[0], Cout=c0, ks=4, bias=w[pre + "pp0t.b"])
            ops.conv_transpose_ks(t[1], w[pre + "pp1t.w"], l1, B=B, H=nh, W_=nw, Cin=ld[1], Cout=ld[1], ks=2, bias=w[pre + "pp1t.b"])
        l2 = t[2]
        h3, w3 = (nh - 1) // 2 + 1, (nw - 1) // 2 + 1
        l3 = self.ws("dpt%d_l3" % num, (B * h3 * w3, ld[3]), mdt)
        sk = self._conv_ws(num)
        geo = ((4 * nh, 4 * nw), (2 * nh, 2 * nw), (nh, nw), (h3, w3))
        srcs = (l0, l1, l2, l3)
        rn = [self.ws("dpt%d_rn%d" % (num, i), (B * geo[i][0] * geo[i][1], F), mdt) for i in range(4)]

        def layer_rn(i):
            ops.conv3x3(srcs[i], w[pre + "rn%d.w" % i], rn[i], B=B, H=geo[i][0], W_=geo[i][1], Cin=(c0 if i == 0 else ld[i]), Cout=F, splitk_ws=sk)

        def pp3c():
            ops.conv3x3(t[3], w[pre + "pp3c.w"], l3, B=B, H=nh, W_=nw, Cin=ld[3], Cout=ld[3], stride=2, bias=w[pre + "pp3c.b"], splitk_ws=sk)

        refs = [(pre + "ref%d." % (4 - j), "%d_%d" % (num, 4 - j)) for j in range(4)]
        if lv:
            with ops.level():
                pp3c()
                layer_rn(2)
            with ops.level():
                layer_rn(0)
                layer_rn(1)
                layer_rn(3)
                self._rcu_c1(rn[2], refs[1][0] + "u1", B, geo[2][0], geo[2][1], refs[1][1])
            with ops.level():
                self._rcu_c1(rn[3], refs[0][0] + "u2", B, geo[3][0], geo[3][1], refs[0][1])
                self._rcu_c1(rn[1], refs[2][0] + "u1", B, geo[1][0], geo[1][1], refs[2][1])
                self._rcu_c1(rn[0], refs[3][0] + "u1", B, geo[0][0], geo[0][1], refs[3][1])
        else:
            pp3c()
            for i in range(4):
                layer_rn(i)
        path, up, Hc, Wc = rn[3], None, h3, w3
        for j in range(4):
            Hn, Wn = geo[3 - j]
            fold = lv and j < 3 and ops.conv3x3_takes_res2_up(w[refs[j + 1][0] + "u1c2.w"], mdt, B, *geo[2 - j])
            nxt, OH_, OW_ = self._fusion(refs[j][0], B, Hn, Wn, path, rn[3 - j] if j else None, refs[j][1], crop=(nh, nw) if j == 0 else None,
                                         c1_done=lv, x0_up=up, fold_up=fold)
            path, up = nxt, ((Hn, Wn) if fold else None)
        p1, H1, W1 = path, OH_, OW_
        a = self.ws("dpt%d_h0" % num, (B * H1 * W1, Lc), mdt)
        ops.conv3x3(p1, w[pre + "h0.w"], a, B=B, H=H1, W_=W1, Cin=F, Cout=Lc, bias=w[pre + "h0.b"])
        OH, OW = 2 * H1, 2 * W1
        u = self.ws("dpt%d_h0up" % num, (B * OH * OW, Lc), mdt)
        ops.upsample2x(a, u, B=B, H=H1, W_=W1, C_=Lc)
        c = self.ws("dpt%d_h2" % num, (B * OH * OW, Lc), mdt)
        ops.conv3x3(u, w[pre + "h2.w"], c, B=B, H=OH, W_=OW, Cin=Lc, Cout=Lc, bias=w[pre + "h2.b"], act=ACT_RELU)
        pts = self.ws("dpt_pts%d" % num, (B, OH, OW, 3))
        conf = self.ws("dpt_conf%d" % num, (B, OH, OW))
        raw = self.ws("dpt_raw%d" % num, (B, OH, OW, 4)) if want_raw else None
        ops.head_final(c, w[pre + "h4.w"], w[pre + "h4.b"], B * OH * OW, Lc, pts, conf, raw)
        return pts, conf, raw

    def encode_cur_value_feat(self, tok, out, res, pos32=None):
        self.activate()
        cfg, w = self.cfg, self.w
        B, P, Cv = tok.shape
        assert Cv == cfg.val_dim
        R, E = B * P, cfg.enc_dim
        zero_pos = self.ws("valf_zero_pos", (R, 2), torch.int32, zero=True)
        rope_tab = None
        if cfg.mem_pos_enc:
            assert pos32 is not None and self.rope_narrow is not None
            zero_pos, rope_tab = pos32, self.rope_narrow
        x = self.ws("valf_x", (R, Cv))
        xpA, xpB = self.wsp("valf_xpA", R, Cv), self.wsp("valf_xpB", R, Cv)
        stA, stB = self.stats("valf_stA", R, Cv), self.stats("valf_stB", R, Cv)
        ops.copy2d(tok.reshape(R, Cv), Cv, x, Cv, R, Cv)
        ops.pack_stats(x, xpA, stA, rows=R, C_=Cv)
        for i in range(cfg.val_depth):
            self._block(x, xpA, stA, xpB, stB, R, B, P, Cv, cfg.enc_heads, "val%d." % i, zero_pos, tag="_valf",
                        head_dim=Cv // cfg.enc_heads, rope_tab=rope_tab)
        ops.gemm(xpA, w["value_out.w"], out, M=R, N=E, K=Cv, lda=Cv, ldc=E, bias=w["value_out.b"], res1=res, ldr1=E,
                 ln=ops.LnFold(stA, Cv, w["value_out.s"], 1e-6))
        return out

    def encode_cur_value(self, pts3d, out, res):
        self.activate()
        cfg, w = self.cfg, self.w
        B, H, W_, _ = pts3d.shape
        p, E = cfg.patch, cfg.enc_dim
        nh, nw = H // p, W_ // p
        P = nh * nw
        R = B * P
        _, pos32, zero_pos = self.positions(B, nh, nw)
        col = self.wsp("im2col_val", R, 3 * p * p)
        sb, sy, sx, sc = pts3d.stride()
        ops.im2col_patch(pts3d, col, B=B, C_=3, H=H, W_=W_, p=p, strides=(sb, sc, sy, sx))
        x, xp, st = self._vit(col, R, B, P, "pospatch", "val", cfg.val_depth, pos32 if cfg.mem_pos_enc else zero_pos, tag="_val")
        ops.gemm(xp, w["value_out.w"], out, M=R, N=E, K=E, lda=E, ldc=E, bias=w["value_out.b"], res1=res, ldr1=E,
                 ln=ops.LnFold(st, E, w["value_out.s"], 1e-6))
        return out
```

spann3r_amd/lib.py:

```python
import ctypes as C
import os

import torch

_HERE = os.path.dirname(os.path.abspath(__file__))
LIB_PATH = os.environ.get("SP3_LIB_PATH") or os.path.join(_HERE, "libspann3r_hip.so")

F32, BF16 = 0, 1
ACT_NONE, ACT_GELU, ACT_RELU = 0, 1, 2
EPI_PLAIN, EPI_ROPE_VT, EPI_PIXSHUF, EPI_PARTIAL = 0, 1, 2, 3
LOAD_PLAIN, LOAD_CONV3X3, LOAD_SOFTMAX = 0, 1, 2


class GemmDesc(C.Structure):
    _fields_ = [
        ("A", C.c_void_p), ("A2", C.c_void_p), ("W", C.c_void_p), ("C", C.c_void_p), ("bias", C.c_void_p),
        ("res1", C.c_void_p), ("res2", C.c_void_p),
        ("M", C.c_int32), ("N", C.c_int32), ("K", C.c_int32), ("batch", C.c_int32),
        ("K1", C.c_int32),
        ("lda", C.c_int64), ("lda2", C.c_int64), ("ldw", C.c_int64), ("ldc", C.c_int64),
        ("ldr1", C.c_int64), ("ldr2", C.c_int64),
        ("strideA", C.c_int64), ("strideW", C.c_int64), ("strideC", C.c_int64),
        ("alpha", C.c_float), ("wdtype", C.c_int32), ("act", C.c_int32), ("out_bf16", C.c_int32),
        ("relu_in", C.c_int32), ("loader", C.c_int32),
        ("conv_H", C.c_int32), ("conv_W", C.c_int32), ("conv_C", C.c_int32),
        ("conv_OH", C.c_int32), ("conv_OW", C.c_int32), ("conv_stride", C.c_int32),
        ("epi", C.c_int32),
        ("rope_cos", C.c_void_p), ("rope_sin", C.c_void_p), ("pos", C.c_void_p),
        ("rope_cols", C.c_int32), ("vt", C.c_void_p), ("tokens", C.c_int32), ("heads", C.c_int32),
        ("vt_ld", C.c_int64),
        ("ps_k", C.c_int32), ("ps_H", C.c_int32), ("ps_W", C.c_int32), ("ps_C", C.c_int32),
        ("tile", C.c_int32), ("a_bf16", C.c_int32), ("splitk", C.c_int32), ("a_packed", C.c_int32),
        ("ln_stats", C.c_void_p), ("ln_s", C.c_void_p), ("ln_nt", C.c_int32), ("ln_C", C.c_int32), ("ln_eps", C.c_float),
        ("stats_out", C.c_void_p), ("c2", C.c_void_p), ("qkv_packed", C.c_int32), ("out_packed", C.c_int32), ("w_packed", C.c_int32),
        ("sb_A2", C.c_int64), ("sb_bias", C.c_int64), ("sb_ln_stats", C.c_int64), ("sb_ln_s", C.c_int64),
        ("sb_stats_out", C.c_int64), ("sb_c2", C.c_int64), ("sb_vt", C.c_int64),
        ("trace", C.c_void_p),
        ("sm_stats_out", C.c_void_p), ("sm_stats", C.c_void_p), ("sm_nt", C.c_int32), ("sm_thresh", C.c_float), ("sm_zout", C.c_void_p),
        ("f32x3", C.c_int32), ("res_bf16", C.c_int32), ("dyn_n", C.c_void_p),
        ("res2_up_H", C.c_int32), ("res2_up_W", C.c_int32),
    ]


class HeadPart(C.Structure):
    _fields_ = [
        ("src", C.c_void_p), ("s_b", C.c_int64), ("s_n", C.c_int64), ("s_h", C.c_int64),
        ("dst", C.c_void_p), ("d_b", C.c_int64), ("d_n", C.c_int64), ("d_h", C.c_int64),
        ("dstT", C.c_void_p), ("pos", C.c_void_p), ("N", C.c_int32), ("fwd", C.c_float), ("ldT", C.c_int64),
    ]


class AttnBwdDesc(C.Structure):
    _fields_ = ([(n, C.c_void_p) for n in ("q", "k", "v", "dout")]
                + [(n, C.c_int64) for n in ("sq", "ldq", "sk", "ldk", "sv", "ldv", "sdo", "lddo")]
                + [(n, C.c_void_p) for n in ("qT", "kT", "doT")] + [("ldTq", C.c_int64), ("ldTk", C.c_int64)]
                + [("lse", C.c_void_p), ("D", C.c_void_p), ("dq", C.c_void_p), ("dk", C.c_void_p), ("dv", C.c_void_p)]
                + [(n, C.c_int64) for n in ("sdq", "lddq", "sdk", "lddk", "sdv", "lddv")]
                + [("B", C.c_int32), ("heads", C.c_int32), ("Nq", C.c_int32), ("Nk", C.c_int32), ("scale", C.c_float), ("bf16_products", C.c_int32)])


class AttnQProjDesc(C.Structure):
    _fields_ = [
        ("x_packed", C.c_void_p), ("x_group_stride", C.c_int64), ("ln_stats", C.c_void_p), ("stats_group_stride", C.c_int64),
        ("w_packed", C.c_void_p), ("w_group_stride", C.c_int64), ("ln_s", C.c_void_p), ("bias", C.c_void_p), ("vec_group_stride", C.c_int64),
        ("pos", C.c_void_p), ("rope_cos", C.c_void_p), ("rope_sin", C.c_void_p), ("ln_eps", C.c_float), ("D", C.c_int32),
        ("kp", C.c_void_p), ("k_cols", C.c_int32), ("k_col0", C.c_int32), ("npad_k", C.c_int32), ("vtp", C.c_void_p),
        ("out", C.c_void_p), ("ldo", C.c_int64), ("out_bf16", C.c_int32), ("out_packed", C.c_int32),
        ("B", C.c_int32), ("heads", C.c_int32), ("Nq", C.c_int32), ("Nk", C.c_int32), ("scale", C.c_float),
        ("o_group", C.c_int32), ("o_group_rows", C.c_int32),
    ]


class ReduceLnDesc(C.Structure):
    _fields_ = [
        ("partial", C.c_void_p), ("split_stride", C.c_int64), ("bias", C.c_void_p), ("res", C.c_void_p),
        ("ldres", C.c_int64), ("x_out", C.c_void_p), ("ldx", C.c_int64),
        ("g1", C.c_void_p), ("b1", C.c_void_p), ("out1", C.c_void_p), ("ld1", C.c_int64), ("out1_bf16", C.c_int32),
        ("g2", C.c_void_p), ("b2", C.c_void_p), ("out2", C.c_void_p), ("ld2", C.c_int64), ("out2_bf16", C.c_int32),
        ("eps", C.c_float), ("splits", C.c_int32), ("rows", C.c_int32), ("C", C.c_int32),
        ("out1_packed", C.c_int32), ("out2_packed", C.c_int32),
            ("act", C.c_int32), ("res2", C.c_void_p), ("ldres2", C.c_int64),
    ]


class BankWriteDesc(C.Structure):
    _fields_ = [
        ("feat_k", C.c_void_p), ("feat_v", C.c_void_p), ("k_raw", C.c_void_p), ("v_raw", C.c_void_p),
        ("k_hat", C.c_void_p), ("v_hat_t", C.c_void_p), ("s_bank", C.c_void_p), ("b_bank", C.c_void_p),
        ("gamma_k", C.c_void_p), ("beta_k", C.c_void_p), ("gamma_v", C.c_void_p), ("beta_v", C.c_void_p),
        ("gamma_q", C.c_void_p), ("beta_q", C.c_void_p),
        ("eps", C.c_float), ("alpha", C.c_float),
        ("M", C.c_int32), ("P", C.c_int32), ("C", C.c_int32), ("cap", C.c_int32), ("wdtype", C.c_int32), ("state", C.c_void_p),
    ]


_lib = None

_PROTOS = {
    "sp3_gemm": [C.POINTER(GemmDesc), C.c_void_p],
    "sp3_gemm_n": [C.POINTER(C.POINTER(GemmDesc)), C.c_int, C.c_void_p],
    "sp3_gemm_plan_n": [C.POINTER(C.POINTER(GemmDesc)), C.c_int, C.POINTER(C.c_int)],
    "sp3_gemm_plan": [C.POINTER(GemmDesc)],
    "sp3_layernorm": [C.c_void_p, C.c_int64, C.c_void_p, C.c_void_p, C.c_float, C.c_void_p, C.c_int64, C.c_int,
                      C.c_int, C.c_int, C.c_void_p],
    "sp3_reduce_ln": [C.POINTER(ReduceLnDesc), C.c_void_p],
    "sp3_layernorm_dual": [C.c_void_p, C.c_int64, C.c_void_p, C.c_void_p, C.c_float, C.c_void_p, C.c_int64, C.c_void_p, C.c_int, C.c_int,
                           C.c_int, C.c_int, C.c_void_p],
    "sp3_layernorm_packed": [C.c_void_p, C.c_int64, C.c_void_p, C.c_void_p, C.c_float, C.c_void_p, C.c_int,
                             C.c_int, C.c_int, C.c_void_p],
    "sp3_attention_ex": [C.c_void_p, C.c_int64, C.c_int64, C.c_void_p, C.c_int64, C.c_int64, C.c_void_p, C.c_int64,
                         C.c_void_p, C.c_int64, C.c_int, C.c_int, C.c_int, C.c_int, C.c_int, C.c_int, C.c_float, C.c_int,
                         C.c_void_p],
    "sp3_layernorm_t": [C.c_void_p, C.c_int64, C.c_void_p, C.c_void_p, C.c_float, C.c_void_p, C.c_int64, C.c_int,
                        C.c_int, C.c_int, C.c_void_p],
    "sp3_rope_2d": [C.c_void_p, C.c_int, C.c_int, C.c_int, C.c_int, C.c_int, C.c_int64, C.c_int64, C.c_int64,
                    C.c_void_p, C.c_float, C.c_float, C.c_void_p],
    "sp3_attention": [C.c_void_p, C.c_int64, C.c_int64, C.c_void_p, C.c_int64, C.c_int64, C.c_void_p, C.c_int64,
                      C.c_void_p, C.c_int64, C.c_int, C.c_int, C.c_int, C.c_int, C.c_int, C.c_float, C.c_int, C.c_void_p],
    "sp3_attention_packed": [C.c_void_p, C.c_int, C.c_int, C.c_int, C.c_void_p, C.c_int, C.c_int, C.c_int, C.c_void_p,
                             C.c_void_p, C.c_int64, C.c_int, C.c_int, C.c_int, C.c_int, C.c_int, C.c_int, C.c_float, C.c_int, C.c_int,
                             C.c_void_p],
    "sp3_attention_packed_qproj": [C.POINTER(AttnQProjDesc), C.c_void_p],
    "sp3_softmax_thresh": [C.c_void_p, C.c_void_p, C.c_int64, C.c_int64, C.c_int, C.c_int, C.c_int, C.c_float,
                           C.c_int, C.c_void_p, C.c_int64, C.c_int, C.c_void_p],
    "sp3_softmax_pack": [C.c_void_p, C.c_int64, C.c_int64, C.c_int, C.c_int, C.c_float, C.c_int, C.c_void_p, C.c_int64, C.c_int, C.c_void_p,
                         C.c_void_p],
    "sp3_colsum_packed": [C.c_void_p, C.c_int, C.c_int, C.c_int, C.c_void_p, C.c_void_p],
    "sp3_colsum_softmax": [C.c_void_p, C.c_int64, C.c_int, C.c_int, C.c_void_p, C.c_float, C.c_void_p, C.c_void_p, C.c_int, C.c_void_p],
    "sp3_bank_write": [C.POINTER(BankWriteDesc), C.c_void_p],
    "sp3_pack_stats": [C.c_void_p, C.c_int64, C.c_int, C.c_int, C.c_void_p, C.c_int, C.c_void_p, C.c_void_p],
    "sp3_gather_packed_rows": [C.c_void_p, C.c_void_p, C.c_void_p, C.c_int, C.c_int, C.c_int, C.c_void_p],
    "sp3_gather_packed_cols": [C.c_void_p, C.c_void_p, C.c_void_p, C.c_int, C.c_int, C.c_int, C.c_int, C.c_int, C.c_void_p],
    "sp3_colsum_accum": [C.c_void_p, C.c_int64, C.c_int, C.c_int, C.c_void_p, C.c_void_p],
    "sp3_cos_sim": [C.c_void_p, C.c_void_p, C.c_int, C.c_int, C.c_int, C.c_void_p, C.c_void_p, C.c_void_p],
    "sp3_mem_append": [C.c_void_p, C.c_void_p, C.c_int, C.c_int, C.c_void_p],
    "sp3_bank_state_set": [C.c_void_p, C.c_int, C.c_int, C.c_void_p],
    "sp3_prob_merge": [C.c_void_p, C.c_void_p, C.c_int, C.c_int, C.c_int, C.c_void_p, C.c_void_p],
    "sp3_colsum_prob": [C.c_void_p, C.c_void_p, C.c_int, C.c_int, C.c_int, C.c_void_p, C.c_void_p, C.c_void_p],
    "sp3_cos_sim_state": [C.c_void_p, C.c_void_p, C.c_int, C.c_int, C.c_int, C.c_void_p, C.c_void_p, C.c_void_p, C.c_void_p],
    "sp3_prune_select": [C.c_void_p, C.c_void_p, C.c_int, C.c_float, C.c_int, C.c_void_p, C.c_void_p],
    "sp3_gather_rows": [C.c_void_p, C.c_void_p, C.c_void_p, C.c_int, C.c_int, C.c_int, C.c_void_p],
    "sp3_gather_cols": [C.c_void_p, C.c_int64, C.c_void_p, C.c_int64, C.c_void_p, C.c_int, C.c_int, C.c_int,
                        C.c_int, C.c_void_p],
    "sp3_gather_1d": [C.c_void_p, C.c_void_p, C.c_void_p, C.c_int, C.c_void_p],
    "sp3_im2col_patch": [C.c_void_p, C.c_int64, C.c_int64, C.c_int64, C.c_int64, C.c_int, C.c_int, C.c_int, C.c_int,
                         C.c_int, C.c_void_p, C.c_int, C.c_int, C.c_void_p],
    "sp3_conv3x3_tile": [C.c_void_p, C.c_int, C.c_void_p, C.c_void_p, C.c_void_p, C.c_void_p, C.c_void_p, C.c_int, C.c_int, C.c_int,
                         C.c_int, C.c_int, C.c_int, C.c_int, C.c_int, C.c_void_p],
    "sp3_upsample2x": [C.c_void_p, C.c_void_p, C.c_int, C.c_int, C.c_int, C.c_int, C.c_int, C.c_int, C.c_void_p],
    "sp3_head_final": [C.c_void_p, C.c_void_p, C.c_void_p, C.c_int64, C.c_int, C.c_void_p, C.c_void_p, C.c_void_p,
                       C.c_void_p],
    "sp3_upsample2x_bf16": [C.c_void_p, C.c_void_p, C.c_int, C.c_int, C.c_int, C.c_int, C.c_int, C.c_int, C.c_void_p],
    "sp3_head_final_bf16": [C.c_void_p, C.c_void_p, C.c_void_p, C.c_int64, C.c_int, C.c_void_p, C.c_void_p, C.c_void_p,
                            C.c_void_p],
    "sp3_fill_f32": [C.c_void_p, C.c_float, C.c_int64, C.c_void_p],
    "sp3_cast_f32_to_bf16": [C.c_void_p, C.c_void_p, C.c_int64, C.c_void_p],
    "sp3_copy2d_f32": [C.c_void_p, C.c_int64, C.c_void_p, C.c_int64, C.c_int, C.c_int, C.c_void_p],
    "sp3_spin": [C.c_int64, C.c_void_p, C.c_void_p],
    "sp3_conf_loss_forward": [C.c_void_p, C.c_void_p, C.c_void_p, C.c_void_p, C.c_void_p, C.c_int, C.c_int, C.c_int, C.c_float, C.c_int,
                              C.c_void_p, C.c_void_p, C.c_void_p, C.c_void_p],
    "sp3_conf_loss_backward": [C.c_void_p, C.c_void_p, C.c_void_p, C.c_void_p, C.c_void_p, C.c_int, C.c_int, C.c_int, C.c_float, C.c_int,
                               C.c_void_p, C.c_void_p, C.c_void_p, C.c_void_p, C.c_void_p],
    "sp3_transpose": [C.c_void_p, C.c_int64, C.c_void_p, C.c_int64, C.c_int, C.c_int, C.c_void_p],
    "sp3_transpose_batched": [C.c_void_p, C.c_int64, C.c_int64, C.c_void_p, C.c_int64, C.c_int64, C.c_int, C.c_int, C.c_int, C.c_void_p],
    "sp3_transpose_pad": [C.c_void_p, C.c_int64, C.c_int64, C.c_void_p, C.c_int64, C.c_int64, C.c_int, C.c_int, C.c_int, C.c_int, C.c_void_p],
    "sp3_softmax_bwd_pad": [C.c_void_p, C.c_void_p, C.c_void_p, C.c_void_p, C.c_int64, C.c_int, C.c_int, C.c_int, C.c_float, C.c_void_p],
    "sp3_head_shuffle": [C.c_void_p, C.c_int, C.c_int, C.c_int, C.c_int, C.c_float, C.c_void_p, C.c_void_p, C.c_int, C.c_void_p],
    "sp3_attention_train_fwd": [C.c_void_p, C.c_int64, C.c_int64, C.c_void_p, C.c_int64, C.c_int64, C.c_void_p, C.c_int64, C.c_void_p, C.c_int64,
                                C.c_void_p, C.c_int, C.c_int, C.c_int, C.c_int, C.c_float, C.c_int, C.c_void_p],
    "sp3_attention_train_bwd": [C.c_void_p, C.c_void_p],
    "sp3_gelu": [C.c_void_p, C.c_void_p, C.c_int64, C.c_void_p],
    "sp3_gelu_bwd": [C.c_void_p, C.c_void_p, C.c_void_p, C.c_int64, C.c_void_p],
    "sp3_im2col3x3": [C.c_void_p, C.c_void_p, C.c_int, C.c_int, C.c_int, C.c_int, C.c_int, C.c_void_p],
    "sp3_col2im3x3": [C.c_void_p, C.c_void_p, C.c_int, C.c_int, C.c_int, C.c_int, C.c_int, C.c_void_p],
    "sp3_relu": [C.c_void_p, C.c_void_p, C.c_int64, C.c_void_p],
    "sp3_relu_bwd": [C.c_void_p, C.c_void_p, C.c_void_p, C.c_int64, C.c_void_p],
    "sp3_upsample2x_bwd": [C.c_void_p, C.c_void_p, C.c_int, C.c_int, C.c_int, C.c_int, C.c_int, C.c_int, C.c_void_p],
    "sp3_postprocess": [C.c_void_p, C.c_void_p, C.c_void_p, C.c_int64, C.c_void_p],
    "sp3_postprocess_bwd": [C.c_void_p, C.c_void_p, C.c_void_p, C.c_void_p, C.c_int64, C.c_void_p],
    "sp3_adamw": [C.c_void_p, C.c_void_p, C.c_void_p, C.c_void_p, C.c_int64, C.c_float, C.c_float, C.c_float, C.c_float, C.c_float, C.c_int,
                  C.c_float, C.c_void_p],
    "sp3_mul": [C.c_void_p, C.c_void_p, C.c_void_p, C.c_int64, C.c_void_p],
    "sp3_pack_bf16": [C.c_void_p, C.c_int64, C.c_int, C.c_int, C.c_void_p, C.c_void_p, C.c_void_p],
    "sp3_pack_bf16_conv3x3": [C.c_void_p, C.c_int, C.c_int, C.c_int, C.c_int, C.c_int, C.c_int, C.c_void_p, C.c_void_p, C.c_void_p],
    "sp3_pack_bf16_act": [C.c_void_p, C.c_int64, C.c_int, C.c_int, C.c_void_p, C.c_void_p, C.c_int, C.c_void_p],
    "sp3_pack_bf16_colsum": [C.c_void_p, C.c_int64, C.c_int, C.c_int, C.c_void_p, C.c_void_p, C.c_void_p, C.c_int, C.c_void_p, C.c_void_p],
    "sp3_colsum_rows": [C.c_void_p, C.c_int64, C.c_int, C.c_int, C.c_void_p, C.c_int, C.c_void_p, C.c_void_p],
    "sp3_sumsq_partial": [C.c_void_p, C.c_int64, C.c_void_p, C.c_void_p],
    "sp3_clip_coef": [C.c_void_p, C.c_int, C.c_float, C.c_float, C.c_void_p, C.c_void_p, C.c_void_p],
    "sp3_adamw_flat": [C.c_void_p, C.c_void_p, C.c_void_p, C.c_void_p, C.c_int64, C.c_void_p, C.c_float, C.c_float, C.c_float, C.c_float,
                       C.c_int, C.c_void_p, C.c_float, C.c_void_p, C.c_void_p, C.c_void_p],
    "sp3_softmax_bwd": [C.c_void_p, C.c_void_p, C.c_void_p, C.c_void_p, C.c_int64, C.c_int, C.c_int, C.c_float, C.c_void_p],
    "sp3_layernorm_bwd": [C.c_void_p, C.c_int64, C.c_void_p, C.c_void_p, C.c_int64, C.c_void_p, C.c_int64, C.c_void_p, C.c_int64,
                          C.c_void_p, C.c_void_p, C.c_int, C.c_void_p, C.c_int, C.c_int, C.c_float, C.c_void_p],
    "sp3_focal_weiszfeld": [C.c_void_p, C.c_int, C.c_int, C.c_int, C.c_float, C.c_float, C.c_int, C.c_float, C.c_float, C.c_void_p, C.c_void_p],
    "sp3_conf_filter": [C.c_void_p, C.c_void_p, C.c_void_p, C.c_int64, C.c_float, C.c_void_p, C.c_void_p, C.c_void_p, C.c_void_p, C.c_void_p],
    "sp3_copy_multi": [C.c_int, C.c_void_p, C.c_void_p, C.c_void_p, C.c_void_p],
    "sp3_pnp_dlt_accum": [C.c_void_p, C.c_int, C.c_int, C.c_int, C.c_float, C.c_float, C.c_float, C.c_void_p, C.c_void_p, C.c_float, C.c_int,
                          C.c_void_p, C.c_void_p],
    "sp3_pnp_gn_accum": [C.c_void_p, C.c_int, C.c_int, C.c_int, C.c_float, C.c_float, C.c_float, C.c_void_p, C.c_void_p, C.c_float, C.c_void_p, C.c_void_p],
    "sp3_pnp_score": [C.c_void_p, C.c_int, C.c_int, C.c_int, C.c_float, C.c_float, C.c_float, C.c_void_p, C.c_int, C.c_float, C.c_int, C.c_void_p, C.c_void_p],
    "sp3_ssi_loss_forward": [C.c_void_p, C.c_void_p, C.c_void_p, C.c_void_p, C.c_int, C.c_int, C.c_int, C.c_int, C.c_int, C.c_void_p, C.c_void_p,
                             C.c_void_p],
    "sp3_preprocess_image": [C.c_void_p, C.c_int64, C.c_int, C.c_int, C.c_int, C.c_int, C.c_void_p, C.c_void_p, C.c_int, C.c_int,
                             C.c_void_p, C.c_void_p, C.c_int, C.c_int, C.c_int, C.c_int, C.c_int, C.c_int, C.c_int, C.c_void_p,
                             C.c_void_p, C.c_void_p],
}
EXPORTS = sorted(list(_PROTOS) + ["sp3_last_error", "sp3_version", "sp3_conf_loss_ws_bytes", "sp3_ssi_loss_ws_bytes", "sp3_sumsq_blocks", "sp3_colsum_rows_ws"])


def load():
    global _lib
    if _lib is not None:
        return _lib
    if not os.path.exists(LIB_PATH):
        raise RuntimeError("libspann3r_hip.so not built: run `python -c 'import __graft_entry__ as g; g.build()'` "
                           "(there is no CPU fallback for the hot path)")
    lib = C.CDLL(LIB_PATH)
    lib.sp3_last_error.restype = C.c_char_p
    lib.sp3_last_error.argtypes = []
    lib.sp3_version.restype = C.c_int
    lib.sp3_conf_loss_ws_bytes.restype = C.c_int64
    lib.sp3_conf_loss_ws_bytes.argtypes = [C.c_int, C.c_int]
    lib.sp3_ssi_loss_ws_bytes.restype = C.c_int64
    lib.sp3_ssi_loss_ws_bytes.argtypes = [C.c_int, C.c_int, C.c_int]
    lib.sp3_sumsq_blocks.restype = C.c_int64
    lib.sp3_sumsq_blocks.argtypes = [C.c_int64]
    lib.sp3_colsum_rows_ws.restype = C.c_int64
    lib.sp3_colsum_rows_ws.argtypes = [C.c_int, C.c_int]
    for name, argtypes in _PROTOS.items():
        fn = getattr(lib, name)
        fn.restype = C.c_int
        fn.argtypes = argtypes
    _lib = lib
    return lib


def check(rc, what):
    if rc != 0:
        msg = load().sp3_last_error().decode(errors="replace")
        raise RuntimeError("%s failed (%d): %s" % (what, rc, msg))


_raw_stream = getattr(torch._C, "_cuda_getCurrentRawStream", None)
_raw_device = getattr(torch._C, "_cuda_getDevice", None)


def stream_ptr():
    if _raw_stream is not None and _raw_device is not None:
        return _raw_stream(_raw_device())
    return torch.cuda.current_stream().cuda_stream


def ptr(t):
    return 0 if t is None else t.data_ptr()
```

spann3r_amd/model.py:

```python
import argparse
import collections
import os
import weakref

import torch
import torch.nn as nn

from . import ops
from .config import Spann3RConfig, FULL
from .engine import Engine
from .weights import param_spec, alias_of, synth_state_dict


def _build_param_tree(root: nn.Module, spec):
    made = {}
    for key, shape in spec.items():
        parts = key.split(".")
        mod = root
        for name in parts[:-1]:
            if not hasattr(mod, name) or not isinstance(getattr(mod, name), nn.Module):
                mod.add_module(name, nn.Module())
            mod = getattr(mod, name)
        src = alias_of(key)
        if src is not None:
# ... 224 lines not shown
        if prof is not None:
            es = bk["k_hat"].element_size()
            prof.region_end("memread", e0, B * (2.0 * M * C * es + 2.0 * P * C * 4),
                            info={"M": M, "tokens_per_frame": P, "flops": 4.0 * B * P * M * C})
        return out

    def _memory_read_prob(self, feat, out, qp, qs, alpha):
        eng, bk = self.eng, self.bank
        B, P, C, M, cap = self.B, self.P, self.C, self.M, self.cap
        dyn = self.state
        Mg = self._bucket(self.PROB_BUCKET) if dyn is not None else M
        S_k = 8
        Pp = (P + 15) // 16 * 16
        rows_pad = (P + 255) // 256 * 256
        ngc = cap // 64
        pk = eng.ws("mem_P_packed", (B, Pp * cap), eng.adt, zero=True)
        stats = eng.ws("mem_prob_stats", (B, ngc * rows_pad * 2))
        scale = eng.ws("mem_prob_scale", (B, ngc * rows_pad))
        part = eng.ws("mem_pv_partial", (16 * P * C,))
        for b in range(B):
            pt = ops.PackedAct(P, cap, eng.adt, eng.device, data=pk[b])
            ops.gemm(qp[b], ops.PackedWeight.wrap(bk["k_hat"][b], Mg, C), pt, M=P, N=Mg, K=C, lda=C, ldc=cap, alpha=alpha,
                     bias=bk["b_bank"][b], ln=ops.LnFold(qs[b], C, bk["s_bank"][b], 1e-5), sm_stats_out=stats[b], dyn_n=dyn)
            ops.prob_merge(stats[b], scale[b], P, Mg, cap, dyn_n=dyn)
            ops.gemm(pt, ops.PackedWeight.wrap(bk["v_hat_t"][b], C, cap), part, M=P, N=C, K=Mg, lda=cap, ldc=C, ldw=cap, splitk=S_k,
                     softmax=(scale[b], 0.0, None), dyn_n=dyn)
            ops.reduce_ln(part, S_k, P, C, res=feat[b], ldres=C, x_out=out[b], ldx=C)
            ops.colsum_prob(pk[b], scale[b], P, Mg, cap, bk["attn"][b], dyn_n=dyn)

    def stage_write(self, feat_k, feat_v):
        bk = self.bank
        B, P, C, M = self.B, self.P, self.C, self.M
        assert M + P <= self.cap, "spatial memory capacity exceeded"
        for b in range(B):
            ops.bank_write(feat_k[b], feat_v[b], self._bank_of(bk, b), M, P, C, self.cap, self._norms, 1.0 / (C ** 0.5), state=self.state)

    def _read_plan(self):
        M, kb = self.M, self.kb
        Kp = (M + kb - 1) // kb * kb
        S_k = 1
        while Kp // (2 * S_k) >= 2048 and S_k < 16:
            S_k *= 2
        fused = S_k == 1 and self.P * M <= self.FUSED_READ_MAX and M % 4 == 0
        if self.read_dyn:
            fused = fused and self._bucket() <= self.STATE_READ_MAX
        return S_k, fused

    def note_deferred_read(self):
        if self.M > 0 and self._read_plan()[1]:
            eng = self.eng
            self._pending_attn = (eng.ws("mem_S", (self.B, self.P, self.cap)), self.cap, self.M, eng.ws("mem_sm_rowz", (self.B, self.P, 4)))

    def _flush_attn(self, append=False):
        pend, self._pending_attn = self._pending_attn, None
        if pend is None:
            return False
        S, ld, M, zk = pend
        bk = self.bank
        fuse = append and M == self.M
        for b in range(self.B):
            ops.colsum_softmax(S[b], ld, self.P, M, zk[b], self.attn_thresh, bk["attn"][b],
                               bk["count"][b] if fuse else None, self.P if fuse else 0)
        return fuse

    def commit(self):
        bk = self.bank
        if not self._flush_attn(append=True):
            for b in range(self.B):
                ops.mem_append(bk["count"][b], bk["attn"][b], self.M, self.P)
        self.M += self.P

    def add_mem(self, feat_k, feat_v):
        self.stage_write(feat_k, feat_v)
        self.commit()
        self._push_state()

    def sim_scores(self, feat_k, to_host=False):
        B, P, C = self.B, self.P, self.C
        n = self.wm * P
        for b in range(B):
            if self.state is not None:
                dst = self._host_scores()[b] if to_host else self._score[b]
                ops.cos_sim_state(feat_k[b], self.bank["k_raw"][b], max(self.work_mem_size, 1), P, C, self.state, dst, self._cos_scratch)
            else:
                ops.cos_sim(feat_k[b], self.bank["k_raw"][b, self.M - n:self.M], self.wm, P, C, self._score[b], self._cos_scratch)
        return self._score[:, :self.wm]

    def sim_needed(self):
        if self.M == 0 or self.sim_thresh == 1.0 or self.wm == 0:
            return False
        if self.wm * self.P > self.M:
            raise RuntimeError("working memory (%d tokens) larger than the bank (%d): reference check_sim is undefined"
                               % (self.wm * self.P, self.M))
        return True

    def _host_scores(self):
        if self._score_host is None:
            self._score_host = torch.empty(self._score.shape, dtype=torch.float32).pin_memory()
            self._score_event = torch.cuda.Event()
        return self._score_host

    def fetch_scores_async(self):
        self._host_scores().copy_(self._score, non_blocking=True)
        self._score_event.record()
        self._score_pending = True

    def copy_scores_in_graph(self):
        self._host_scores().copy_(self._score, non_blocking=True)

    _SENTINEL = 2.0

    def arm_score_poll(self):
        self._host_scores().fill_(self._SENTINEL)
        self._score_pending = "poll"

    def sim_verdict(self):
        if self._score_pending == "poll":
            import time
            self._score_pending = False
            view = self._score_host[:, :self.wm]
            t0 = time.perf_counter()
            while bool((view == self._SENTINEL).any()):
                if time.perf_counter() - t0 > 0.25:
                    torch.cuda.current_stream().synchronize()
                    if bool((view == self._SENTINEL).any()):
                        view = self._score[:, :self.wm].cpu()
                    break
            mx = float(view.max())
        elif self._score_pending:
            self._score_event.synchronize()
            self._score_pending = False
            mx = float(self._score_host[:, :self.wm].max())
        else:
            mx = float(self._score[:, :self.wm].max())
        if mx > self.sim_thresh:
            print("Similarity detected:", mx)
            return True
        return False

    def check_sim(self, feat_k):
        if not self.sim_needed():
            return False
        self.sim_scores(feat_k)
        return self.sim_verdict()

    def add_mem_check(self, feat_k, feat_v):
        if self.check_sim(feat_k):
            self.events.append("skip")
            return
        self.add_mem(feat_k, feat_v)
        self._after_write()
        self._push_state()

    def finish_staged(self, similar):
        if similar:
            self.events.append("skip")
            self._flush_attn()
            return
        self.commit()
        self._after_write()
        self._push_state()

    def _after_write(self):
        self.wm += 1
        if self.wm > self.work_mem_size:
            self.wm -= 1
            if self.long_mem_size == 0:
                self._drop_oldest()
            else:
                self.lm += self.P
        if self.lm > self.long_mem_size:
            self.memory_prune()
            self.lm = self.top_k - self.wm * self.P

    def _drop_oldest(self):
        self._flush_attn()
        B, C, M, P = self.B, self.C, self.M, self.P
        k = M - P
        src = self.bank
        if self._banks[1 - self._cur] is None:
            self._banks[1 - self._cur] = self._alloc(self.eng.device, self.eng.wdt)
        dst = self._banks[1 - self._cur]
        sel = self._window_sel.get((P, M))
        if sel is None:
            sel = self._window_sel[(P, M)] = torch.arange(P, M, dtype=torch.int32, device=self.eng.device)
        for b in range(B):
            ops.gather_rows(src["k_raw"][b], dst["k_raw"][b], sel, k, C)
            ops.gather_rows(src["v_raw"][b], dst["v_raw"][b], sel, k, C)
            ops.gather_packed_rows(src["k_hat"][b], dst["k_hat"][b], sel, k, C)
            ops.gather_packed_cols(src["v_hat_t"][b], dst["v_hat_t"][b], sel, k, self.cap, C, self.cap)
            for name in ("s_bank", "b_bank", "attn", "count"):
                ops.gather_1d(src[name][b], dst[name][b], sel, k)
        print("Memory pruned:", torch.Size((B, k, C)))
        self.events.append("window %d->%d" % (M, k))
        self._cur = 1 - self._cur
        self.M = k

    def memory_prune(self):
        self._flush_attn()
        B, C, M, k = self.B, self.C, self.M, self.top_k
        src = self.bank
        if self._banks[1 - self._cur] is None:
            self._banks[1 - self._cur] = self._alloc(self.eng.device, self.eng.wdt)
        dst = self._banks[1 - self._cur]
        for b in range(B):
            ops.prune_select(src["attn"][b], src["count"][b], M, self.work_mem_size + 5, k, self._sel[b])
            sel = self._sel[b]
            ops.gather_rows(src["k_raw"][b], dst["k_raw"][b], sel, k, C)
            ops.gather_rows(src["v_raw"][b], dst["v_raw"][b], sel, k, C)
            ops.gather_packed_rows(src["k_hat"][b], dst["k_hat"][b], sel, k, C)
            ops.gather_packed_cols(src["v_hat_t"][b], dst["v_hat_t"][b], sel, k, self.cap, C, self.cap)
            for name in ("s_bank", "b_bank", "attn", "count"):
                ops.gather_1d(src[name][b], dst[name][b], sel, k)
        print("Memory pruned:", M, "->", k)
        self.events.append("prune %d->%d" % (M, k))
        self._cur = 1 - self._cur
        self.M = k


class MemorySnapshot:
    mem_k = mem_v = mem_attn = mem_count = None
    wm = lm = M = 0


class _SequenceRunner:

    def __init__(self, model, eng, B, H, W, training, true_hw=None):
        cfg = model.cfg
        self._model_ref = weakref.ref(model)
        self.eng, self.B, self.H, self.W, self.training = eng, B, H, W, training
        p = cfg.patch
        self.nh, self.nw = H // p, W // p
        th, tw = true_hw or (H, W)
        self.hh, self.hw = th // p, tw // p
        self.swap = th > tw
        self.P, self.E = self.nh * self.nw, cfg.enc_dim
        dev = eng.device
        self.img_pair = torch.empty(2 * B, 3, H, W, device=dev)
        self.img_next = torch.empty(B, 3, H, W, device=dev)
        self.feat_pre = torch.empty(B, self.P, self.E, device=dev)
        self.featpair = torch.empty(2 * B, self.P, self.E, device=dev)
        self.feat1, self.feat2 = self.featpair[:B], self.featpair[B:]
        self.fuse = torch.empty(B, self.P, self.E, device=dev)
        self.packed_feats = eng.packed_attn
        self.feats_p = None
        self.featpair_p = ops.PackedAct.group(2, B * self.P, self.E, torch.bfloat16, dev) if self.packed_feats else None
        self.fuse_p = ops.PackedAct(B * self.P, self.E, torch.bfloat16, dev) if self.packed_feats else None
        self.k1 = torch.empty(B, self.P, self.E, device=dev)
        self.k2 = torch.empty(B, self.P, self.E, device=dev)
        self.v = torch.empty(B, self.P, self.E, device=dev)
        self.mem = None
        self.k2_aux = (None, None)
        self.graphs = collections.OrderedDict()
        self.graph_bytes = 0
        self.seen = set()
        self.length_keys, self.length_keys_eager = set(), False
        self.out = None
        self._scores_to_host = False
        self.batched = False
        self.img_all = self.feats = None
        self.defer2 = False
        self.seq_dec2 = None
        self.dec2_hooks = None
        self.head2_out = {}

    @property
    def model(self):
        m = self._model_ref()
        if m is None:
            raise RuntimeError("the Spann3R model this runner belongs to is gone")
        return m

    def ensure_memory(self, n_frames):
        need = (n_frames - 1) * self.P if self.training else 4000 + 8 * self.P
        if self.mem is None or self.mem.cap < need:
            self.mem = SpatialMemory(self.eng, self.B, self.P, capacity=need, attn_thresh=0.0 if self.training else 5e-4, device_state=True)
            self.graphs.clear()
            self.graph_bytes = 0
            self.seen.clear()
            self.length_keys, self.length_keys_eager = set(), False
        self.mem.reset()
        return self.mem

    ENC_CHUNK_ROWS = 16

    def encode_sequence(self, frames, use_graphs):
        B, n = self.B, len(frames)
        if self.feats is None or self.feats.shape[0] < n * B:
            self.img_all = torch.empty(n * B, 3, self.H, self.W, device=self.eng.device)
            self.feats = torch.empty(n * B, self.P, self.E, device=self.eng.device)
            self.feats_p = ops.PackedAct.group(n, B * self.P, self.E, torch.bfloat16, self.eng.device) if self.packed_feats else None
            self._drop_graphs(lambda k: k[0] in ("enc", "head2"))
            self.seen = {k for k in self.seen if k[0] not in ("enc", "head2")}
        slots = [(f["img"], self.img_all[i * B:(i + 1) * B]) for i, f in enumerate(frames)]
        fast = [p for p in slots if p[0].is_cuda and p[0].dtype == torch.float32 and p[0].is_contiguous() and p[0].shape == p[1].shape]
        for c0 in range(0, len(fast), 8):
            ops.copy_multi(fast[c0:c0 + 8])
        for src, dst in slots:
            if not any(src is q[0] for q in fast):
                dst.copy_(src)
        per = max(1, self.ENC_CHUNK_ROWS // B)
        for c0 in range(0, n, per):
            c1 = min(n, c0 + per)
            img, out = self.img_all[c0 * B:c1 * B], self.feats[c0 * B:c1 * B]
            outp = self.feats_p.at(c0) if self.feats_p is not None else None
            self._graphed(("enc", c0, c1), lambda: self.eng.encode_image(img, out=out, tag="_seq", out_packed=outp, group_rows=B * self.P),
                          use_graphs)
        self.batched = True

    HEAD_CHUNK = 16

    def enable_deferred_head2(self, n_frames):
        rows = (n_frames - 1) * self.B * self.P
        D = self.model.cfg.dec_dim
# ... 19 lines not shown
            for j, t in enumerate(self.seq_dec2):
                dec[hk[j + 1]] = t[c0 * B * P:c1 * B * P]
            key = ("head2", c0, c1)

            def fn(dec=dec, key=key, nb=(c1 - c0) * B):
                pts, conf, _ = self.eng.dpt_head(dec, nb, self.hh, self.hw, 2)
                self.head2_out[key] = (pts, conf)
            self._graphed(key, fn, use_graphs)
            pts, conf = self.head2_out[key]
            pts, conf = pts.clone(), conf.clone()
            for j in range(c1 - c0):
                outs.append((pts[j * B:(j + 1) * B], conf[j * B:(j + 1) * B]))
        return outs

    def begin_outputs(self, n_steps):
        self._out_slabs, self._out_steps, self._out_i = None, n_steps, 0
        if self.mem is not None and self.mem.state is None and not self.length_keys_eager:
            per_step = 1 if self.model.single_graph_step else 2
            if n_steps * per_step > self.MAX_GRAPHS - 4:
                self.length_keys_eager = True
                self._drop_graphs(lambda k: k in self.length_keys)

    def _step_outputs(self, srcs):
        if getattr(self, "_out_steps", 0) <= 0 or self._out_i >= self._out_steps:
            return [torch.empty_like(t) for t in srcs]
        if self._out_slabs is None or len(self._out_slabs) != len(srcs):
            self._out_slabs = [t.new_empty((self._out_steps,) + tuple(t.shape)) for t in srcs]
        i, self._out_i = self._out_i, self._out_i + 1
        return [slab[i] for slab in self._out_slabs]

    def pair_copies(self, i):
        B = self.B
        pairs = [(self.feats[i * B:(i + 2) * B], self.featpair)]
        if self.feats_p is not None:
            st = self.feats_p.stride
            pairs.append((self.feats_p.data.view(-1)[i * st:(i + 2) * st], self.featpair_p.data.view(-1)[:2 * st]))
        return pairs

    def load_pair(self, i):
        ops.copy_multi(self.pair_copies(i))

    def _drop_graphs(self, pred):
        for k in [k for k in self.graphs if pred(k)]:
            self.graph_bytes -= self.graphs.pop(k)[1]

    MAX_GRAPHS = 16
    MAX_GRAPH_BYTES = 1 << 30

    def _graphed(self, key, fn, use_graphs, per_length=False):
        if per_length and use_graphs and not self.length_keys_eager and key not in self.graphs and key in self.seen \
                and len(self.graphs) >= self.MAX_GRAPHS - 2:
            self.length_keys_eager = True
            self._drop_graphs(lambda k: k in self.length_keys)
        if per_length:
            self.length_keys.add(key)
        if not use_graphs or (per_length and self.length_keys_eager):
            fn()
        elif key in self.graphs:
            self.graphs.move_to_end(key)
            self.graphs[key][0].replay()
        elif key in self.seen:
            if getattr(self, "_pool", None) is None or not self.graphs:
                self._pool = torch.cuda.graph_pool_handle()
            if getattr(self, "_capture_stream", None) is None:
                self._capture_stream = torch.cuda.Stream()
            before = torch.cuda.memory_allocated()
            g = torch.cuda.CUDAGraph()
            import gc
            gc_was = gc.isenabled()
            gc.disable()
            main = torch.cuda.current_stream()
            cap = self._capture_stream
            cap.wait_stream(main)
            try:
                with torch.cuda.stream(cap):
                    g.capture_begin(self._pool, capture_error_mode="thread_local")
                    try:
                        fn()
                    finally:
                        g.capture_end()
            finally:
                if gc_was:
                    gc.enable()
            main.wait_stream(cap)
            nbytes = max(0, torch.cuda.memory_allocated() - before)
            self.graphs[key] = (g, nbytes)
            self.graph_bytes += nbytes
            while len(self.graphs) > self.MAX_GRAPHS or (self.graph_bytes > self.MAX_GRAPH_BYTES and len(self.graphs) > 1):
                _, (old, ob) = self.graphs.popitem(last=False)
                self.graph_bytes -= ob
                del old
            g.replay()
        else:
            self.seen.add(key)
            fn()

    def _part1(self, first, has_next):
        eng, mem, B, P, E = self.eng, self.mem, self.B, self.P, self.E
        main = torch.cuda.current_stream()
        st = eng.side_streams()
        packed = self.packed_feats and self.model.packed_features and self.batched and self.feats_p is not None
        p1 = p2 = f1p = None
        if packed:
            p1, p2 = self.featpair_p.at(0), self.featpair_p.at(1)
        if first:
            if not self.batched:
                eng.encode_image(self.img_pair, out=self.featpair)
            f1, f1p = self.feat1, p1
        else:
            if not self.batched:
                ops.copy2d(self.feat2, E, self.feat1, E, B * P, E)
                ops.copy2d(self.feat_pre, E, self.feat2, E, B * P, E)
            mem.memory_read(self.k2, self.fuse, *(self.k2_aux if B == 1 else (None, None)), defer_attn=True,
                            out_packed=self.fuse_p if packed else None)
            f1 = self.fuse
            f1p = self.fuse_p if (packed and mem.wrote_packed) else None
        if has_next:
            st[3].wait_stream(main)
            with torch.cuda.stream(st[3]):
                eng.encode_image(self.img_next, out=self.feat_pre, tag="_pre")
        if eng.packed_attn and self.model.grouped_decoder:
            dec1, dec2 = eng.decoder_grouped(f1, self.feat2, B, self.nh, self.nw, f1p=f1p, f2p=p2 if f1p is not None else None)
            self.k2_aux = eng.encode_feat_keys_grouped(self.feat1, self.feat2, dec1[-1], dec2[-1], B * P, self.k1, self.k2,
                                                       feat1p=p1, feat2p=p2)
        else:
            if self.model.decoder_streams:
                dec1, dec2 = eng.decoder(f1, self.feat2, B, self.nh, self.nw, self.nh, self.nw, streams=st)
                st[2].wait_stream(main)
                with torch.cuda.stream(st[2]):
                    self.k2_aux = eng.encode_feat_key(self.feat2, dec2[-1], B * P, 2, self.k2, aux=True)
                eng.encode_feat_key(self.feat1, dec1[-1], B * P, 1, self.k1)
                main.wait_stream(st[2])
            else:
                dec1, dec2 = eng.decoder(f1, self.feat2, B, self.nh, self.nw, self.nh, self.nw, streams=None)
                self.k2_aux = eng.encode_feat_key(self.feat2, dec2[-1], B * P, 2, self.k2, aux=True)
                eng.encode_feat_key(self.feat1, dec1[-1], B * P, 1, self.k1)
        if not self.training and mem.sim_needed():
            mem.sim_scores(self.k1, to_host=self._scores_to_host and mem.state is not None)
        if has_next:
            main.wait_stream(st[3])
        self.dec = (dec1, dec2)
        self.dec2_hooks = [dec2[h] for h in self.model.cfg.hooks[1:]]

    def _part2(self):
        eng, mem, B = self.eng, self.mem, self.B
        dec1, dec2 = self.dec
        main = torch.cuda.current_stream()
        st = eng.side_streams()
        pts2 = conf2 = None
        if not self.defer2:
            st[2].wait_stream(main)
            with torch.cuda.stream(st[2]):
                pts2, conf2, _ = eng.dpt_head(dec2, B, self.hh, self.hw, 2)
        pts1, conf1, _ = eng.dpt_head(dec1, B, self.hh, self.hw, 1)
        if eng.cfg.use_feat:
            eng.encode_cur_value_feat(dec1[-1], self.v, self.k1,
                                      pos32=eng.positions(B, self.nh, self.nw)[1] if eng.cfg.mem_pos_enc else None)
        else:
            eng.encode_cur_value(pts1.swapaxes(1, 2) if self.swap else pts1, self.v, self.k1)
        mem.stage_write(self.k1, self.v)
        if not self.defer2:
            main.wait_stream(st[2])
        self.out = (pts1, conf1, pts2, conf2)

    def run(self, first, has_next, use_graphs, post_copies=()):
        mem = self.mem
        has_next = has_next and not self.batched
        gk = mem.graph_key()
        per_length = gk[0] not in ("s", "p")
        key = gk + (mem._cur, has_next, self.batched, self.defer2, self.model.grouped_decoder, self.model.packed_features)
        if not use_graphs and ops._prof is not None:
            ops._prof.step_begin()
        need_sim = not self.training and mem.sim_needed()
        if self.model.single_graph_step and use_graphs and ops._prof is None:
            if need_sim:
                mem.arm_score_poll()

            def whole():
                self._scores_to_host = need_sim
                try:
                    self._part1(first, has_next)
                finally:
                    self._scores_to_host = False
                if need_sim and mem.state is None:
                    mem.copy_scores_in_graph()
                self._part2()
            self._graphed(("whole", first, need_sim) + key, whole, use_graphs, per_length)
            if not first:
                mem.note_deferred_read()
        else:
            self._graphed(("first" if first else "step",) + key, lambda: self._part1(first, has_next), use_graphs, per_length)
            if not first:
                mem.note_deferred_read()
            if need_sim:
                mem.fetch_scores_async()
            self._graphed(("tail",) + key, self._part2, use_graphs, per_length)
        pts1, conf1, pts2, conf2 = self.out
        srcs = (pts1, conf1) + (() if pts2 is None else (pts2, conf2))
        outs = self._step_outputs(srcs)
        copies = list(zip(srcs, outs))
        copies += list(post_copies() if callable(post_copies) else post_copies)
        for c0 in range(0, len(copies), 8):
            ops.copy_multi(copies[c0:c0 + 8])
        res1 = {"pts3d": outs[0], "conf": outs[1]}
        res2 = {} if pts2 is None else {"pts3d": outs[2], "conf": outs[3]}
        if self.swap:
            res1 = {k: v.swapaxes(1, 2) for k, v in res1.items()}
            res2 = {k: v.swapaxes(1, 2) for k, v in res2.items()}
        if self.training:
            mem.commit()
            mem._push_state()
        else:
            mem.finish_staged(mem.sim_verdict() if need_sim else False)
        return res1, res2


class Spann3R(nn.Module):

    def __init__(self, dus3r_name="./checkpoints/DUSt3R_ViTLarge_BaseDecoder_512_dpt.pth",
                 use_feat=False, mem_pos_enc=False, memory_dropout=0.15, cfg: Spann3RConfig = None,
                 init_weights=True):
        super().__init__()
        self.use_feat = use_feat
        self.mem_pos_enc = mem_pos_enc
        self.mem_dropout = nn.Dropout(memory_dropout)
        ckpt = None
        if dus3r_name is not None and not os.path.isfile(dus3r_name):
            raise FileNotFoundError("DUSt3R checkpoint %r not found (pass dus3r_name=None to build without one)" % dus3r_name)
        if dus3r_name is not None:
            torch.serialization.add_safe_globals([argparse.Namespace])
            ckpt = torch.load(dus3r_name, map_location="cpu", weights_only=True)
            cfg = Spann3RConfig.from_ctor_string(ckpt["args"].model)
        self.cfg = cfg or FULL
        if mem_pos_enc != self.cfg.mem_pos_enc or use_feat != self.cfg.use_feat:
            import dataclasses
            self.cfg = dataclasses.replace(self.cfg, mem_pos_enc=bool(mem_pos_enc), use_feat=bool(use_feat))
        self.add_module("dust3r", _Dust3RFacade(self))
        self._params = _build_param_tree(self, param_spec(self.cfg))
        if init_weights:
            with torch.no_grad():
                for k, v in synth_state_dict(0, self.cfg).items():
                    if alias_of(k) is None:
                        self._params[k].copy_(v)
        if ckpt is not None:
            sd = {("dust3r." + k): v for k, v in ckpt["model"].items()}
            if not any(k.startswith("dust3r.dec_blocks2") for k in sd):
                for k, v in list(sd.items()):
                    if k.startswith("dust3r.dec_blocks."):
                        sd[k.replace("dust3r.dec_blocks.", "dust3r.dec_blocks2.")] = v
            own = self.state_dict()
            missing = [k for k in own if k.startswith("dust3r.") and k not in sd and alias_of(k) is None]
            unexpected = [k for k in sd if k not in own]
            print("<checkpoint %s: missing keys %s, unexpected keys %s>" % (dus3r_name, missing, unexpected))
            with torch.no_grad():
                for k, v in sd.items():
                    if k in own:
                        own[k].copy_(v)
                if not self.cfg.use_feat:
                    self._params["pos_patch_embed.proj.weight"].copy_(self._params["dust3r.patch_embed.proj.weight"])
                    self._params["pos_patch_embed.proj.bias"].copy_(self._params["dust3r.patch_embed.proj.bias"])
        self.precision = "fp32"
        self._engine = None
        self._engine_key = None
        self._pinned = None
        self._runners = {}
        self.use_graphs = True
        self.batch_encode = True
        self.defer_head2 = True
        self.grouped_decoder = True
        self.single_graph_step = True
        self.packed_features = True
        self.decoder_streams = True
        self.force_general = False
        self.max_runners = 4

    f16x3_range_guard = True

    def set_precision(self, precision):
        assert precision in ("fp32", "f32x3", "f32x6", "f16x3", "bf16")
        self.precision = precision
        return self

    def _versions(self):
        return tuple(p._version for p in self._params.values())

    @property
    def engine(self) -> Engine:
        if self._pinned is not None:
            return self._pinned.activate()
        dev = self._params["norm_q.weight"].device
        if dev.type != "cuda":
            raise RuntimeError("spann3r_amd.Spann3R runs on an MI355X only: call .to('cuda') first "
                               "(there is no CPU fallback; the CPU reference lives in oracle/ for tests)")
        key = (dev, self.precision, self._versions(), ops.WEIGHTS_EPOCH)
        if self._engine is None or self._engine_key != key:
            self._engine = Engine(self.cfg, dict(self._params), dev, self.precision)
            self._engine_key = key
            self._runners = {}
        return self._engine.activate()

    def _runner(self, key, make):
        run = self._runners.pop(key, None)
        if run is None:
            run = make()
            while len(self._runners) >= self.max_runners:
                self._runners.pop(next(iter(self._runners)))
        self._runners[key] = run
        return run

    @staticmethod
    def _true_shape(view):
        img = view["img"]
        return view.get("true_shape", torch.tensor(img.shape[-2:])[None].repeat(img.shape[0], 1))

    def _tag_grid(self, pos, img):
        pos._sp3_grid = (img.shape[-2] // self.cfg.patch, img.shape[-1] // self.cfg.patch)
        return pos

    def encode_image(self, view):
        img = view["img"]
        feat, pos = self.engine.encode_image(img.float())
        return feat, self._tag_grid(pos[:], img), self._true_shape(view)

    def encode_image_pairs(self, view1, view2):
        img = torch.cat((view1["img"], view2["img"]), dim=0).float()
        feat, pos = self.engine.encode_image(img)
        f1, f2 = feat.chunk(2, dim=0)
        p1, p2 = pos.chunk(2, dim=0)
        return (f1.contiguous(), f2.contiguous(), self._tag_grid(p1, img), self._tag_grid(p2, img),
                self._true_shape(view1), self._true_shape(view2))

    def encode_frames(self, view1, view2, feat1, feat2, pos1, pos2, shape1, shape2):
        if feat1 is None:
            return self.encode_image_pairs(view1, view2)
        feat1, pos1, shape1 = feat2, pos2, shape2
        feat2, pos2, shape2 = self.encode_image(view2)
        return feat1, feat2, pos1, pos2, shape1, shape2

    def decode(self, feat1, pos1, feat2, pos2):
        B = feat1.shape[0]
        g1, g2 = self._grid_from_pos(pos1), self._grid_from_pos(pos2)
        return self.engine.decoder(feat1, feat2, B, g1[0], g1[1], g2[0], g2[1])

    @staticmethod
    def _grid_from_pos(pos):
        g = getattr(pos, "_sp3_grid", None)
        if g is not None:
            return g
        return int(pos[0, :, 0].max()) + 1, int(pos[0, :, 1].max()) + 1

    def encode_feat_key(self, feat1, feat2, num=1):
        B, P = feat1.shape[:2]
        out = torch.empty(B, P, self.cfg.enc_dim, device=feat1.device)
        return self.engine.encode_feat_key(feat1, feat2, B * P, num, out)

    def downstream_head(self, dec, true_shape, num=1):
        hs, ws = true_shape[:, 0], true_shape[:, 1]
        B = dec[-1].shape[0]
        H, W = int(true_shape[0, 0]), int(true_shape[0, 1])
        p = self.cfg.patch
        if not bool((true_shape == true_shape[0:1]).all()):
            H, W = int(true_shape.min()), int(true_shape.max())
            land = (ws >= hs).to(dec[-1].device)
            if not bool(((hs == H) & (ws == W) | (hs == W) & (ws == H)).all()):
                raise ValueError("true_shape: one image size per batch, in either orientation (got %s)" % true_shape.tolist())
            res = None
# ... 291 lines not shown
```

spann3r_amd/ops.py:

```python
import ctypes as C

import torch

from . import lib as L
from .lib import GemmDesc, F32, BF16, ACT_NONE, ACT_GELU, ACT_RELU


_prof = None


class Profiler:

    def __init__(self, blocker_ms=12.0):
        self.rec = []
        self.regions = []
        self.blocker_cycles = int(blocker_ms * 2.4e6)

    def step_begin(self):
        torch.cuda._sleep(self.blocker_cycles)

    def region_begin(self):
        return (self.begin(), len(self.rec))

    def region_end(self, key, e0, nbytes, info=None):
# ... 504 lines not shown
    return out


def proj_rope_vt(A, W, bias, out_qk, ldc, vt, vt_ld, *, M, N, K, lda, rope_cols, pos, cos, sin, tokens, heads, tile=-1,
                 qkv_packed=False, ln=None, batch=1, strideA=0, strideW=0, strideC=0, sb=None):
    d = GemmDesc()
    d.a_bf16 = _act(A, "A")
    d.a_packed = _is_packed(A)
    _w(d, W)
    d.A, d.C, d.bias = A.data_ptr(), L.ptr(out_qk), L.ptr(bias)
    d.M, d.N, d.K, d.batch = M, N, K, 1
    d.lda, d.ldc = lda, ldc
    d.alpha = 1.0
    d.loader, d.epi, d.tile = L.LOAD_PLAIN, L.EPI_ROPE_VT, tile
    d.rope_cos, d.rope_sin, d.pos, d.rope_cols = cos.data_ptr(), sin.data_ptr(), pos.data_ptr(), rope_cols
    d.vt, d.vt_ld, d.tokens, d.heads = L.ptr(vt), vt_ld, tokens, heads
    d.qkv_packed = int(qkv_packed)
    _ln(d, ln)
    if out_qk is None:
        d.C = vt.data_ptr()
    if batch > 1:
        _group(d, batch, strideA, strideW, strideC, sb)
    _gemm_launch(d, "sp3_gemm(rope_vt)", "plain")


def layernorm(x, gamma, beta, eps, out, *, rows, C_, ldx=None, ldo=None, transposed=False, dual=None, group_rows=0):
    _f32(x, "x")
    ldx = C_ if ldx is None else ldx
    ldo = C_ if ldo is None else ldo
    if dual is not None:
        assert dual.dtype == torch.bfloat16 and not transposed and not _is_packed(out)
        pad = getattr(dual, "rows_pad", (group_rows + 15) // 16 * 16)
        _timed("layernorm", 8.0 * rows * C_, rows * C_ * 10.0,
               lambda: L.check(L.load().sp3_layernorm_dual(x.data_ptr(), ldx, gamma.data_ptr(), beta.data_ptr(), eps, out.data_ptr(), ldo,
                                                           dual.data_ptr(), rows, C_, group_rows or rows, pad, L.stream_ptr()),
                               "sp3_layernorm_dual"))
        return out
    if _is_packed(out):
        _timed("layernorm", 8.0 * rows * C_, rows * C_ * 6.0,
               lambda: L.check(L.load().sp3_layernorm_packed(x.data_ptr(), ldx, gamma.data_ptr(), beta.data_ptr(), eps,
                                                             out.data_ptr(), int(out.dtype == torch.bfloat16), rows, C_,
                                                             L.stream_ptr()), "sp3_layernorm_packed"))
        return out
    fn = L.load().sp3_layernorm_t if transposed else L.load().sp3_layernorm
    _timed("layernorm_t" if transposed else "layernorm", 8.0 * rows * C_, rows * C_ * (4.0 + out.element_size()),
           lambda: L.check(fn(x.data_ptr(), ldx, gamma.data_ptr(), beta.data_ptr(), eps, out.data_ptr(), ldo,
                              int(out.dtype == torch.bfloat16), rows, C_, L.stream_ptr()), "sp3_layernorm"))
    return out


def rope_2d(tokens, positions, base, fwd):
    if tokens.dim() != 4:
        raise RuntimeError("tokens must have 4 dimensions")
    if positions.dim() != 3:
        raise RuntimeError("positions must have 3 dimensions")
    if tokens.size(0) != positions.size(0):
        raise RuntimeError("batch size differs between tokens & positions")
    if tokens.size(1) != positions.size(1):
        raise RuntimeError("seq_length differs between tokens & positions")
    if positions.size(2) != 2:
        raise RuntimeError("positions.shape[2] must be equal to 2")
    if tokens.is_cuda != positions.is_cuda:
        raise RuntimeError("tokens and positions are not on the same device")
    if not tokens.is_cuda:
        raise RuntimeError("spann3r_amd rope_2d is the MI355X kernel: tokens must be on the GPU (no CPU fallback)")
    if tokens.stride(3) != 1:
        raise RuntimeError("tokens are not contiguous")
    if not positions.is_contiguous() or positions.dtype != torch.int64:
        raise RuntimeError("positions are not contiguous int64")
    B, N, H, D = tokens.shape
    dt = wdtype_of(tokens)
    L.check(L.load().sp3_rope_2d(tokens.data_ptr(), dt, B, N, H, D, tokens.stride(0), tokens.stride(1), tokens.stride(2),
                                 positions.data_ptr(), float(base), float(fwd), L.stream_ptr()), "sp3_rope_2d")
    return tokens


def attention(q, sq, ldq, k, sk, ldk, vt, vt_ld, out, ldo, *, B, heads, Nq, Nk, scale):
    es = vt.element_size()
    _timed("attention<%s>" % ("f32" if es == 4 else "bf16"), 4.0 * B * heads * Nq * Nk * 64,
           B * heads * 64.0 * (es * (Nq + 2 * Nk) + 4 * Nq),
           lambda: L.check(L.load().sp3_attention_ex(q.data_ptr(), sq, ldq, k.data_ptr(), sk, ldk, vt.data_ptr(), vt_ld,
                                                     out.data_ptr(), ldo, int(out.dtype == torch.bfloat16), _is_packed(out),
                                                     B, heads, Nq, Nk, float(scale), (2 if (get_product_mode() == 1 and es == 4) else 3 if (get_product_mode() == 4 and es == 4) else wdtype_of(vt)),
                                                     L.stream_ptr()),
                           "sp3_attention"))
    return out


def attention_packed(qp, q_cols, q_col0, npad_q, kp, k_cols, k_col0, npad_k, vtp, out, ldo, *, B, heads, Nq, Nk, scale,
                     o_group=0, o_group_rows=0):
    _timed("attention_packed<bf16>", 4.0 * B * heads * Nq * Nk * 64, B * heads * 64.0 * (2 * (Nq + 2 * Nk) + 4 * Nq),
           lambda: L.check(L.load().sp3_attention_packed(qp.data_ptr(), q_cols, q_col0, npad_q, kp.data_ptr(), k_cols, k_col0,
                                                         npad_k, vtp.data_ptr(), out.data_ptr(), ldo,
                                                         int(out.dtype == torch.bfloat16), _is_packed(out), B, heads, Nq, Nk,
                                                         float(scale), o_group, o_group_rows, L.stream_ptr()),
                           "sp3_attention_packed"))
    return out


def attention_packed_qproj(xq, stats, Wq, ln_s, bias, pos, cos, sin, kp, k_cols, k_col0, npad_k, vtp, out, ldo, *, B, heads, Nq, Nk, scale,
                           o_group, o_group_rows, eps=1e-6, stats_group_stride=0, vec_group_stride=0):
    d = L.AttnQProjDesc()
    D = heads * 64
    d.x_packed, d.x_group_stride = xq.data_ptr(), getattr(xq, "stride", 0)
    d.ln_stats, d.stats_group_stride = stats.data_ptr(), stats_group_stride
    d.w_packed, d.w_group_stride = Wq.data_ptr(), getattr(Wq, "stride", 0)
    d.ln_s, d.bias, d.vec_group_stride = ln_s.data_ptr(), bias.data_ptr(), vec_group_stride
    d.pos, d.rope_cos, d.rope_sin, d.ln_eps, d.D = pos.data_ptr(), cos.data_ptr(), sin.data_ptr(), eps, D
    d.kp, d.k_cols, d.k_col0, d.npad_k, d.vtp = kp.data_ptr(), k_cols, k_col0, npad_k, vtp.data_ptr()
    d.out, d.ldo, d.out_bf16, d.out_packed = out.data_ptr(), ldo, int(out.dtype == torch.bfloat16), _is_packed(out)
    d.B, d.heads, d.Nq, d.Nk, d.scale, d.o_group, d.o_group_rows = B, heads, Nq, Nk, float(scale), o_group, o_group_rows
    _timed("attention_packed_qproj<bf16>", 4.0 * B * heads * Nq * Nk * 64 + 2.0 * B * Nq * D * D,
           B * heads * 64.0 * (2 * (2 * Nk) + 4 * Nq) + 2.0 * B * Nq * D + 2.0 * (B // max(o_group, 1)) * D * D,
           lambda: L.check(L.load().sp3_attention_packed_qproj(C.byref(d), L.stream_ptr()), "sp3_attention_packed_qproj"))
    return out


def softmax_thresh(S, P, *, ld, rows, M, Mpad, thresh, batch=1, strideS=0, packed=None, stride_packed=0):
    pbf = packed is not None and packed.dtype == torch.bfloat16
    _timed("softmax_thresh", 8.0 * batch * rows * M, (4.0 + (0.0 if P is None else 4.0) + (0.0 if packed is None else packed.element_size())) * batch * rows * M,
           lambda: L.check(L.load().sp3_softmax_thresh(S.data_ptr(), L.ptr(P), ld, strideS, rows, M, Mpad, float(thresh),
                                                       batch, L.ptr(packed), stride_packed, int(pbf), L.stream_ptr()), "sp3_softmax_thresh"))


def softmax_pack(S, packed, rowstat, *, ld, rows, M, thresh, batch=1, strideS=0, stride_packed=0):
    _timed("softmax_pack", 8.0 * batch * rows * M, (4.0 + packed.element_size()) * batch * rows * M,
           lambda: L.check(L.load().sp3_softmax_pack(S.data_ptr(), ld, strideS, rows, M, float(thresh), batch, packed.data_ptr(), stride_packed,
                                                     int(packed.dtype == torch.bfloat16), rowstat.data_ptr(), L.stream_ptr()), "sp3_softmax_pack"))


def colsum_accum(P, ld, rows, M, mem_attn):
    L.check(L.load().sp3_colsum_accum(P.data_ptr(), ld, rows, M, mem_attn.data_ptr(), L.stream_ptr()), "sp3_colsum_accum")


def colsum_packed(packed, rows, M, mem_attn):
    _timed("colsum_packed", 1.0 * rows * M, 1.0 * packed.element_size() * rows * M,
           lambda: L.check(L.load().sp3_colsum_packed(packed.data_ptr(), int(packed.dtype == torch.bfloat16), rows, M, mem_attn.data_ptr(),
                                                      L.stream_ptr()), "sp3_colsum_packed"))


def copy_multi(pairs):
    n = len(pairs)
    if not 1 <= n <= 8:
        raise ValueError("copy_multi: 1..8 copies")
    S, D, Bt = (C.c_void_p * n)(), (C.c_void_p * n)(), (C.c_int64 * n)()
    for i, (s_, d_) in enumerate(pairs):
        nb = s_.numel() * s_.element_size()
        if not (s_.is_contiguous() and d_.is_contiguous()) or nb != d_.numel() * d_.element_size():
            raise ValueError("copy_multi: pair %d must be contiguous and of equal size" % i)
        S[i], D[i], Bt[i] = s_.data_ptr(), d_.data_ptr(), nb
    _timed("copy_multi", 0.0, 2.0 * sum(Bt), lambda: L.check(L.load().sp3_copy_multi(n, S, D, Bt, L.stream_ptr()), "sp3_copy_multi"))


def colsum_softmax(S, ld, rows, M, rowz, thresh, mem_attn, mem_count=None, append_P=0):
    _timed("colsum_softmax", 4.0 * rows * M, 4.0 * rows * M,
           lambda: L.check(L.load().sp3_colsum_softmax(S.data_ptr(), ld, rows, M, rowz.data_ptr(), float(thresh), mem_attn.data_ptr(),
                                                       L.ptr(mem_count), append_P, L.stream_ptr()), "sp3_colsum_softmax"))


def bank_write(feat_k, feat_v, bank, M, P, C_, cap, norms, alpha, eps=1e-5, state=None):
    d = L.BankWriteDesc()
    d.state = L.ptr(state)
    d.feat_k, d.feat_v = feat_k.data_ptr(), feat_v.data_ptr()
    d.k_raw, d.v_raw, d.k_hat, d.v_hat_t = bank["k_raw"].data_ptr(), bank["v_raw"].data_ptr(), bank["k_hat"].data_ptr(), bank["v_hat_t"].data_ptr()
    d.s_bank, d.b_bank = bank["s_bank"].data_ptr(), bank["b_bank"].data_ptr()
    d.gamma_k, d.beta_k, d.gamma_v, d.beta_v, d.gamma_q, d.beta_q = [t.data_ptr() for t in norms]
    d.eps, d.alpha, d.M, d.P, d.C, d.cap, d.wdtype = eps, alpha, M, P, C_, cap, wdtype_of(bank["k_hat"])
    es = bank["k_hat"].element_size()
    _timed("bank_write", 20.0 * P * C_, P * C_ * (16.0 + 2 * es),
           lambda: L.check(L.load().sp3_bank_write(C.byref(d), L.stream_ptr()), "sp3_bank_write"))


def pack_stats(x, packed, stats, *, rows, C_, ldx=None):
    _f32(x, "x")
    L.check(L.load().sp3_pack_stats(x.data_ptr(), C_ if ldx is None else ldx, rows, C_, packed.data_ptr(),
                                    int(packed.dtype == torch.bfloat16), stats.data_ptr(), L.stream_ptr()), "sp3_pack_stats")


_pack_ws = {}


def _pack_colsum_ws(device, nby, nbx):
    ws = _pack_ws.get(str(device))
    need = nby * nbx * 64
    if ws is None or ws.numel() < need:
        ws = torch.empty(max(need, 1 << 18), device=device)
        _pack_ws[str(device)] = ws
    return ws


def pack_bf16(x2d, want=True, want_t=False, colsum=None, accumulate=False, act=0):
    rows, cols = x2d.shape
    _f32(x2d, "x")
    if x2d.stride(1) != 1:
        x2d = x2d.contiguous()
    alloc = lambda r, c: torch.empty(packed_shape(r, c, torch.bfloat16), dtype=torch.bfloat16, device=x2d.device)
    a = PackedAct(rows, cols, torch.bfloat16, x2d.device, data=alloc(rows, cols)) if want else None
    t = PackedAct(cols, rows, torch.bfloat16, x2d.device, data=alloc(cols, rows)) if want_t else None
    if act:
        assert colsum is None
        _timed("pack_bf16", 0.0, rows * cols * (4.0 + 2.0 * (bool(want) + bool(want_t))),
               lambda: L.check(L.load().sp3_pack_bf16_act(x2d.data_ptr(), x2d.stride(0), rows, cols, L.ptr(a), L.ptr(t), int(act), L.stream_ptr()), "sp3_pack_bf16_act"))
        return a, t
    if colsum is not None:
        pw = _pack_colsum_ws(x2d.device, (rows + 63) // 64, (cols + 63) // 64)
        _timed("pack_bf16", 0.0, rows * cols * (4.0 + 2.0 * (bool(want) + bool(want_t))),
               lambda: L.check(L.load().sp3_pack_bf16_colsum(x2d.data_ptr(), x2d.stride(0), rows, cols, L.ptr(a), L.ptr(t), colsum.data_ptr(), int(accumulate),
                                                             pw.data_ptr(), L.stream_ptr()), "sp3_pack_bf16_colsum"))
        return a, t
    _timed("pack_bf16", 0.0, rows * cols * (4.0 + 2.0 * (bool(want) + bool(want_t))),
           lambda: L.check(L.load().sp3_pack_bf16(x2d.data_ptr(), x2d.stride(0), rows, cols, L.ptr(a), L.ptr(t), L.stream_ptr()), "sp3_pack_bf16"))
    return a, t


def pack_bf16_conv3x3(x, stride, want=True, want_t=False, act=0):
    B, H, W_, C_ = x.shape
    _f32(x, "x")
    assert x.is_contiguous()
    OH, OW = (H - 1) // stride + 1, (W_ - 1) // stride + 1
    rows, cols = B * OH * OW, 9 * C_
    alloc = lambda r, c: torch.empty(packed_shape(r, c, torch.bfloat16), dtype=torch.bfloat16, device=x.device)
    a = PackedAct(rows, cols, torch.bfloat16, x.device, data=alloc(rows, cols)) if want else None
    t = PackedAct(cols, rows, torch.bfloat16, x.device, data=alloc(cols, rows)) if want_t else None
    _timed("pack_bf16_conv3x3", 0.0, rows * cols * 2.0 * (bool(want) + bool(want_t)) + x.numel() * 4.0,
           lambda: L.check(L.load().sp3_pack_bf16_conv3x3(x.data_ptr(), B, H, W_, C_, stride, int(act), L.ptr(a), L.ptr(t), L.stream_ptr()), "sp3_pack_bf16_conv3x3"))
    return a, t


def gather_packed_rows(src, dst, sel, n_sel, C_):
    L.check(L.load().sp3_gather_packed_rows(src.data_ptr(), dst.data_ptr(), sel.data_ptr(), n_sel, C_, src.element_size(),
                                            L.stream_ptr()), "sp3_gather_packed_rows")


def gather_packed_cols(src, dst, sel, n_sel, n_fill, C_, cap):
    L.check(L.load().sp3_gather_packed_cols(src.data_ptr(), dst.data_ptr(), sel.data_ptr(), n_sel, n_fill, C_, cap, src.element_size(),
                                            L.stream_ptr()), "sp3_gather_packed_cols")


def prob_merge(stats, scale, rows, M, cap, dyn_n=None):
    L.check(L.load().sp3_prob_merge(stats.data_ptr(), scale.data_ptr(), rows, M, cap, L.ptr(dyn_n), L.stream_ptr()), "sp3_prob_merge")


def colsum_prob(p_packed, scale, rows, M, cap, mem_attn, dyn_n=None):
    _timed("colsum_prob", 2.0 * rows * M, 2.0 * rows * M,
           lambda: L.check(L.load().sp3_colsum_prob(p_packed.data_ptr(), scale.data_ptr(), rows, M, cap, L.ptr(dyn_n), mem_attn.data_ptr(), L.stream_ptr()),
                           "sp3_colsum_prob"))


def bank_state_set(state, M, wm):
    L.check(L.load().sp3_bank_state_set(state.data_ptr(), int(M), int(wm), L.stream_ptr()), "sp3_bank_state_set")


def cos_sim_state(k, k_raw, Tmax, P, C_, state, score, scratch):
    assert scratch.numel() >= Tmax * P and scratch.dtype == torch.float32 and state.dtype == torch.int32
    L.check(L.load().sp3_cos_sim_state(k.data_ptr(), k_raw.data_ptr(), Tmax, P, C_, state.data_ptr(), scratch.data_ptr(), score.data_ptr(),
                                       L.stream_ptr()), "sp3_cos_sim_state")


def cos_sim(k, wm, T, P, C_, score, scratch):
    assert scratch.numel() >= T * P and scratch.dtype == torch.float32
    L.check(L.load().sp3_cos_sim(k.data_ptr(), wm.data_ptr(), T, P, C_, scratch.data_ptr(), score.data_ptr(), L.stream_ptr()),
            "sp3_cos_sim")


def mem_append(count, attn, M, P):
    L.check(L.load().sp3_mem_append(count.data_ptr(), attn.data_ptr(), M, P, L.stream_ptr()), "sp3_mem_append")


def prune_select(attn, count, M, protect, top_k, sel):
    L.check(L.load().sp3_prune_select(attn.data_ptr(), count.data_ptr(), M, float(protect), top_k, sel.data_ptr(),
                                      L.stream_ptr()), "sp3_prune_select")


def gather_rows(src, dst, sel, n_sel, C_):
    L.check(L.load().sp3_gather_rows(src.data_ptr(), dst.data_ptr(), sel.data_ptr(), n_sel, C_, src.element_size(),
                                     L.stream_ptr()), "sp3_gather_rows")


def gather_cols(src, ld_src, dst, ld_dst, sel, n_sel, n_fill, C_):
    L.check(L.load().sp3_gather_cols(src.data_ptr(), ld_src, dst.data_ptr(), ld_dst, sel.data_ptr(), n_sel, n_fill, C_,
                                     src.element_size(), L.stream_ptr()), "sp3_gather_cols")


def gather_1d(src, dst, sel, n_sel):
    L.check(L.load().sp3_gather_1d(src.data_ptr(), dst.data_ptr(), sel.data_ptr(), n_sel, L.stream_ptr()), "sp3_gather_1d")


def im2col_patch(img, out, *, B, C_, H, W_, p, strides):
    _f32(img, "img")
    sb, sc, sy, sx = strides
    L.check(L.load().sp3_im2col_patch(img.data_ptr(), sb, sc, sy, sx, B, C_, H, W_, p, out.data_ptr(),
                                      int(out.dtype == torch.bfloat16), _is_packed(out), L.stream_ptr()), "sp3_im2col_patch")
    return out


def upsample2x(x, out, *, B, H, W_, C_, outH=None, outW=None):
    outH = 2 * H if outH is None else outH
    outW = 2 * W_ if outW is None else outW
    if x.dtype != out.dtype or x.dtype not in (torch.float32, torch.bfloat16):
        raise TypeError("upsample2x: fp32 or bf16 maps, input and output alike")
    fn = L.load().sp3_upsample2x_bf16 if x.dtype == torch.bfloat16 else L.load().sp3_upsample2x
    _timed("upsample2x", 8.0 * B * outH * outW * C_, float(x.element_size()) * B * C_ * (H * W_ + outH * outW),
           lambda: L.check(fn(x.data_ptr(), out.data_ptr(), B, H, W_, C_, outH, outW, L.stream_ptr()), "sp3_upsample2x"))
    return out


def head_final(feat, w, b, pixels, C_, pts, conf, raw=None):
    fn = L.load().sp3_head_final_bf16 if feat.dtype == torch.bfloat16 else L.load().sp3_head_final
    _timed("head_final", 8.0 * pixels * C_, pixels * (float(feat.element_size()) * C_ + 16.0),
           lambda: L.check(fn(feat.data_ptr(), w.data_ptr(), b.data_ptr(), pixels, C_, pts.data_ptr(),
                              conf.data_ptr(), L.ptr(raw), L.stream_ptr()), "sp3_head_final"))


def fill(t, v):
    L.check(L.load().sp3_fill_f32(t.data_ptr(), float(v), t.numel(), L.stream_ptr()), "sp3_fill_f32")


def copy2d(src, lds, dst, ldd, rows, cols):
    L.check(L.load().sp3_copy2d_f32(src.data_ptr(), lds, dst.data_ptr(), ldd, rows, cols, L.stream_ptr()), "sp3_copy2d_f32")
```

Baseline: 639.1 frames/s.

## Fuse per-step colsum, output copies and state push; emit patch rows from head

Adds a single step-prologue kernel that takes pending memory-attention column sums, the output copies and the bank-state write, and runs them as one launch with a per-block job map. This replaces separate copy_multi, colsum and state-set launches. It also adds a variant of the DPT head's final kernel that writes the bf16 im2col patch rows of the predicted points directly, so the value encoder can skip a separate im2col pass. The cost is a more complex job-dispatch kernel whose jobs all use 1024-thread blocks, plus new index-mapping logic for patch and swap layouts.

```diff
diff --git a/include/spann3r_hip.h b/include/spann3r_hip.h
--- a/include/spann3r_hip.h
+++ b/include/spann3r_hip.h
@@ -162,6 +162,25 @@
                            int elem_size, void* stream);
 int sp3_cos_sim(const float* k, const float* wm, int T, int P, int C, float* scratch, float* score, void* stream);
 int sp3_bank_state_set(int32_t* state, int M, int wm, void* stream);
+#define SP3_PROLOGUE_MAX_COLSUM 8
+#define SP3_PROLOGUE_MAX_COPIES 8
+typedef struct sp3_step_prologue_desc {
+  const float* S[SP3_PROLOGUE_MAX_COLSUM];
+  const float* rowz[SP3_PROLOGUE_MAX_COLSUM];
+  float* mem_attn[SP3_PROLOGUE_MAX_COLSUM];
+  float* mem_count[SP3_PROLOGUE_MAX_COLSUM];
+  const void* src[SP3_PROLOGUE_MAX_COPIES];
+  void* dst[SP3_PROLOGUE_MAX_COPIES];
+  int64_t bytes[SP3_PROLOGUE_MAX_COPIES];
+  int64_t ld;
+  int32_t* state;
+  int32_t n_colsum, n_copies;
+  int32_t rows, M, append_P;
+  float thresh;
+  int32_t state_M, state_wm;
+} sp3_step_prologue_desc;
+int sp3_step_prologue(const sp3_step_prologue_desc* desc_host, void* stream);
+int sp3_step_prologue_map(const sp3_step_prologue_desc* desc_host, int32_t* start, int32_t* kind, int32_t* n_jobs);
 int sp3_prob_merge(const float* stats, float* scale, int rows, int M, int cap, const int32_t* dyn_n, void* stream);
 int sp3_colsum_prob(const void* P_packed, const float* scale, int rows, int M, int cap, const int32_t* dyn_n, float* mem_attn, void* stream);
 int sp3_cos_sim_state(const float* k, const float* k_raw, int Tmax, int P, int C, const int32_t* state, float* scratch, float* score,
@@ -185,6 +204,8 @@
                    float* conf, float* raw, void* stream);
 int sp3_head_final_bf16(const void* feat, const float* w, const float* b, int64_t pixels, int C, float* pts, float* conf,
                         float* raw, void* stream);
+int sp3_head_final_patch_bf16(const void* feat, const float* w, const float* b, int B, int OH, int OW, int C, float* pts, float* conf,
+                              float* raw, void* patch_rows, int p, int swap, void* stream);
 
 int sp3_preprocess_image(const uint8_t* src, int64_t src_row_stride, int crop_l, int crop_t, int H1, int W1,
                          const int32_t* hbounds, const int32_t* hcoef, int hksize, int W2,
diff --git a/spann3r_amd/csrc/dpt.hip b/spann3r_amd/csrc/dpt.hip
--- a/spann3r_amd/csrc/dpt.hip
+++ b/spann3r_amd/csrc/dpt.hip
@@ -136,10 +136,14 @@
   }
 }
 
-template <int LP, int PPT>
+struct HeadPatchArgs {
+  __bf16* rows;
+  int OH, OW, p, swap;
+};
+template <int LP, int PPT, bool PATCH>
 __global__ __launch_bounds__(256) void head_final_bf16x8_kernel(const __bf16* __restrict__ feat, const float* __restrict__ w,
                                                                 const float* __restrict__ bias, int64_t pixels, float* __restrict__ pts,
-                                                                float* __restrict__ conf, float* __restrict__ raw) {
+                                                                float* __restrict__ conf, float* __restrict__ raw, const HeadPatchArgs pa) {
   constexpr int C = 8 * LP, PPB = 256 / LP;
   const int li = threadIdx.x % LP, pl = threadIdx.x / LP;
   float wr[4][8];
@@ -149,17 +153,19 @@
     wr[f][0] = a.x; wr[f][1] = a.y; wr[f][2] = a.z; wr[f][3] = a.w; wr[f][4] = b.x; wr[f][5] = b.y; wr[f][6] = b.z; wr[f][7] = b.w;
   }
   const float b0 = bias[0], b1 = bias[1], b2 = bias[2], b3 = bias[3];
-  const int64_t p0 = (int64_t)blockIdx.x * PPB * PPT + pl;
+  const int64_t p0 = PATCH ? ((int64_t)blockIdx.x * PPB + pl) * PPT : (int64_t)blockIdx.x * PPB * PPT + pl;
+  constexpr int QS = PATCH ? 1 : PPB;
   bf16x8 x[PPT];
 #pragma unroll
   for (int q = 0; q < PPT; ++q) {
-    int64_t pix = p0 + (int64_t)q * PPB;
+    int64_t pix = p0 + (int64_t)q * QS;
     pix = pix < pixels ? pix : pixels - 1;
     x[q] = *reinterpret_cast<const bf16x8*>(feat + pix * C + li * 8);
   }
+  float pv[PPT];
 #pragma unroll
   for (int q = 0; q < PPT; ++q) {
-    const int64_t pix = p0 + (int64_t)q * PPB;
+    const int64_t pix = p0 + (int64_t)q * QS;
     float a[4];
 #pragma unroll
     for (int f = 0; f < 4; ++f) {
@@ -172,13 +178,43 @@
     for (int o = 1; o < LP; o <<= 1) {
       a[0] += __shfl_xor(a[0], o); a[1] += __shfl_xor(a[1], o); a[2] += __shfl_xor(a[2], o); a[3] += __shfl_xor(a[3], o);
     }
-    if (li == 0 && pix < pixels) {
+    pv[q] = 0.f;
+    if (li < (PATCH ? 4 : 1) && pix < pixels) {
       const float X = a[0] + b0, Y = a[1] + b1, Z = a[2] + b2, Cc = a[3] + b3;
-      if (raw) *reinterpret_cast<float4*>(raw + pix * 4) = make_float4(X, Y, Z, Cc);
       const float d = sqrtf(X * X + Y * Y + Z * Z);
       const float sc = expm1f(d) / fmaxf(d, 1e-8f);
-      pts[pix * 3 + 0] = X * sc; pts[pix * 3 + 1] = Y * sc; pts[pix * 3 + 2] = Z * sc;
-      conf[pix] = 1.0f + expf(Cc);
+      const float px = X * sc, py = Y * sc, pz = Z * sc;
+      if (li == 0) {
+        if (raw) *reinterpret_cast<float4*>(raw + pix * 4) = make_float4(X, Y, Z, Cc);
+        pts[pix * 3 + 0] = px; pts[pix * 3 + 1] = py; pts[pix * 3 + 2] = pz;
+        conf[pix] = 1.0f + expf(Cc);
+      }
+      pv[q] = li == 1 ? px : (li == 2 ? py : pz);
+    }
+  }
+  if constexpr (PATCH) {
+    static_assert(PPT == 4, "one 8-byte piece = 4 consecutive k of a patch row");
+    if (li >= 1 && li < 4 && p0 < pixels) {
+      const int per = pa.OH * pa.OW, b = (int)(p0 / per), rem = (int)(p0 - (int64_t)b * per);
+      const int y = rem / pa.OW, x0 = rem - y * pa.OW;
+      const int c = li - 1, K = 3 * pa.p * pa.p;
+      if (!pa.swap) {
+        const int nw = pa.OW / pa.p, ty = y / pa.p, tx = x0 / pa.p;
+        const int row = (b * (pa.OH / pa.p) + ty) * nw + tx;
+        const int k = (c * pa.p + (y - ty * pa.p)) * pa.p + (x0 - tx * pa.p);
+        bf16x4 o;
+        o[0] = (__bf16)pv[0]; o[1] = (__bf16)pv[1]; o[2] = (__bf16)pv[2]; o[3] = (__bf16)pv[3];
+        *reinterpret_cast<bf16x4*>(pa.rows + packed_off(row, k, K, true)) = o;
+      } else {
+        const int nw = pa.OH / pa.p, tx = y / pa.p;
+#pragma unroll
+        for (int q = 0; q < 4; ++q) {
+          const int iy = x0 + q, ty = iy / pa.p;
+          const int row = (b * (pa.OW / pa.p) + ty) * nw + tx;
+          const int k = (c * pa.p + (iy - ty * pa.p)) * pa.p + (y - tx * pa.p);
+          pa.rows[packed_off(row, k, K, true)] = (__bf16)pv[q];
+        }
+      }
     }
   }
 }
@@ -239,8 +275,8 @@
   SP3_CHECK(feat && w && b && pts && conf && pixels > 0 && C > 0 && C % 32 == 0, "sp3_head_final_bf16: bad arguments");
   if (C == 128 && (reinterpret_cast<uintptr_t>(feat) & 15) == 0 && (reinterpret_cast<uintptr_t>(w) & 15) == 0 && (!raw || (reinterpret_cast<uintptr_t>(raw) & 15) == 0)) {
     constexpr int LP = 16, PPT = 4, PPB = 256 / LP;
-    hipLaunchKernelGGL((head_final_bf16x8_kernel<LP, PPT>), dim3((unsigned)((pixels + PPB * PPT - 1) / (PPB * PPT))), dim3(256), 0, ST(stream),
-                       reinterpret_cast<const __bf16*>(feat), w, b, pixels, pts, conf, raw);
+    hipLaunchKernelGGL((head_final_bf16x8_kernel<LP, PPT, false>), dim3((unsigned)((pixels + PPB * PPT - 1) / (PPB * PPT))), dim3(256), 0, ST(stream),
+                       reinterpret_cast<const __bf16*>(feat), w, b, pixels, pts, conf, raw, HeadPatchArgs{});
     SP3_LAUNCH_CHECK("sp3_head_final_bf16");
     return 0;
   }
@@ -250,3 +286,20 @@
   SP3_LAUNCH_CHECK("sp3_head_final_bf16");
   return 0;
 }
+
+extern "C" int sp3_head_final_patch_bf16(const void* feat, const float* w, const float* b, int B, int OH, int OW, int C, float* pts, float* conf,
+                                         float* raw, void* patch_rows, int p, int swap, void* stream) {
+  SP3_CHECK(feat && w && b && pts && conf && patch_rows && B > 0 && OH > 0 && OW > 0 && p > 0, "sp3_head_final_patch_bf16: bad arguments");
+  SP3_CHECK(C == 128 && (reinterpret_cast<uintptr_t>(feat) & 15) == 0 && (reinterpret_cast<uintptr_t>(w) & 15) == 0 &&
+            (!raw || (reinterpret_cast<uintptr_t>(raw) & 15) == 0), "sp3_head_final_patch_bf16: needs a 16-byte aligned 128-channel map (C=%d)", C);
+  SP3_CHECK(OH % p == 0 && OW % p == 0, "Input image size (%d,%d) is not a multiple of patch size (%d)", swap ? OW : OH, swap ? OH : OW, p);
+  SP3_CHECK(p % 4 == 0, "sp3_head_final_patch_bf16: patch size %d (a lane group stores 4 consecutive pixels of a patch row)", p);
+  SP3_CHECK((int64_t)B * OH * OW < (1ll << 31) / 3, "sp3_head_final_patch_bf16: map too large");
+  constexpr int LP = 16, PPT = 4, PPB = 256 / LP;
+  const int64_t pixels = (int64_t)B * OH * OW;
+  hipLaunchKernelGGL((head_final_bf16x8_kernel<LP, PPT, true>), dim3((unsigned)((pixels + PPB * PPT - 1) / (PPB * PPT))), dim3(256), 0, ST(stream),
+                     reinterpret_cast<const __bf16*>(feat), w, b, pixels, pts, conf, raw,
+                     HeadPatchArgs{reinterpret_cast<__bf16*>(patch_rows), OH, OW, p, swap});
+  SP3_LAUNCH_CHECK("sp3_head_final_patch_bf16");
+  return 0;
+}
diff --git a/spann3r_amd/csrc/memory.hip b/spann3r_amd/csrc/memory.hip
--- a/spann3r_amd/csrc/memory.hip
+++ b/spann3r_amd/csrc/memory.hip
@@ -184,15 +184,15 @@
   }
 }
 
-__global__ __launch_bounds__(1024) void colsum_softmax_kernel(const float* __restrict__ S, int64_t ld, int rows, int M,
-                                                              const float4* __restrict__ rowz, float thr, float* __restrict__ mem_attn,
-                                                              float* __restrict__ mem_count, int app_P) {
+__device__ __forceinline__ void colsum_softmax_body(const int bx, const float* __restrict__ S, int64_t ld, int rows, int M,
+                                                    const float4* __restrict__ rowz, float thr, float* __restrict__ mem_attn,
+                                                    float* __restrict__ mem_count, int app_P) {
   __shared__ float sh[16][64];
   const int lane = threadIdx.x & 63, w = threadIdx.x >> 6;
-  const int j = blockIdx.x * 64 + lane;
+  const int j = bx * 64 + lane;
   const int jc = j < M ? j : M - 1;
   float acc = 0.f;
-  for (int r0 = w; r0 < rows && blockIdx.x * 64 < M; r0 += 16 * 8) {
+  for (int r0 = w; r0 < rows && bx * 64 < M; r0 += 16 * 8) {
     float sv[8];
     float4 rz[8];
 #pragma unroll
@@ -219,6 +219,12 @@
     if (j < M) mem_count[j] += 1.0f;
     else if (j < M + app_P) { mem_count[j] = 0.f; mem_attn[j] = 0.f; }
   }
+}
+
+__global__ __launch_bounds__(1024) void colsum_softmax_kernel(const float* __restrict__ S, int64_t ld, int rows, int M,
+                                                              const float4* __restrict__ rowz, float thr, float* __restrict__ mem_attn,
+                                                              float* __restrict__ mem_count, int app_P) {
+  colsum_softmax_body(blockIdx.x, S, ld, rows, M, rowz, thr, mem_attn, mem_count, app_P);
 }
 
 __global__ __launch_bounds__(256) void colsum_accum_kernel(const float* __restrict__ P, int64_t ld, int rows, int M,
@@ -345,9 +351,10 @@
   }
 }
 
-__global__ void bank_state_kernel(int* __restrict__ state, int M, int wm) {
+__device__ __forceinline__ void bank_state_body(int* __restrict__ state, int M, int wm) {
   if (threadIdx.x == 0) { state[0] = M; state[1] = wm; }
 }
+__global__ void bank_state_kernel(int* __restrict__ state, int M, int wm) { bank_state_body(state, M, wm); }
 
 __global__ __launch_bounds__(256) void mem_append_kernel(float* __restrict__ count, float* __restrict__ attn, int M, int P) {
   const int j = blockIdx.x * 256 + threadIdx.x;
@@ -356,12 +363,45 @@
 }
 
 struct CopyMultiArgs { const char* src[8]; char* dst[8]; int64_t bytes[8]; };
+__device__ __forceinline__ void copy_body(const int bx, const int nb, const char* __restrict__ src, char* __restrict__ dst, int64_t bytes) {
+  const int64_t n16 = bytes >> 4;
+  const uint4* s = reinterpret_cast<const uint4*>(src);
+  uint4* d = reinterpret_cast<uint4*>(dst);
+  for (int64_t i = (int64_t)bx * blockDim.x + threadIdx.x; i < n16; i += (int64_t)nb * blockDim.x) d[i] = s[i];
+}
 __global__ __launch_bounds__(256) void copy_multi_kernel(const CopyMultiArgs a) {
   const int e = blockIdx.y;
-  const int64_t n16 = a.bytes[e] >> 4;
-  const uint4* s = reinterpret_cast<const uint4*>(a.src[e]);
-  uint4* d = reinterpret_cast<uint4*>(a.dst[e]);
-  for (int64_t i = (int64_t)blockIdx.x * 256 + threadIdx.x; i < n16; i += (int64_t)gridDim.x * 256) d[i] = s[i];
+  copy_body(blockIdx.x, gridDim.x, a.src[e], a.dst[e], a.bytes[e]);
+}
+
+constexpr int PROLOGUE_JOBS = SP3_PROLOGUE_MAX_COLSUM + SP3_PROLOGUE_MAX_COPIES + 1;
+constexpr int PROLOGUE_COPY_VECS = 2;
+struct ProloguePlan {
+  int n_jobs;
+  int start[PROLOGUE_JOBS + 1];
+  int kind[PROLOGUE_JOBS], index[PROLOGUE_JOBS];
+};
+struct PrologueArgs {
+  sp3_step_prologue_desc d;
+  int start[PROLOGUE_JOBS + 1];
+};
+
+__global__ __launch_bounds__(1024) void step_prologue_kernel(const PrologueArgs a) {
+  const int w = blockIdx.x;
+  int p = 0;
+#pragma unroll
+  for (int i = 1; i < PROLOGUE_JOBS; ++i) p = w >= a.start[i] ? i : p;
+  const int local = w - a.start[p];
+  const sp3_step_prologue_desc& d = a.d;
+  if (p < d.n_colsum) {
+    colsum_softmax_body(local, d.S[p], d.ld, d.rows, d.M, reinterpret_cast<const float4*>(d.rowz[p]), d.thresh, d.mem_attn[p], d.mem_count[p],
+                        d.append_P);
+  } else if (p < d.n_colsum + d.n_copies) {
+    const int e = p - d.n_colsum;
+    copy_body(local, a.start[p + 1] - a.start[p], reinterpret_cast<const char*>(d.src[e]), reinterpret_cast<char*>(d.dst[e]), d.bytes[e]);
+  } else {
+    bank_state_body(d.state, d.state_M, d.state_wm);
+  }
 }
 
 constexpr int PRUNE_MAX = 16384;
@@ -774,6 +814,63 @@
   return 0;
 }
 
+namespace {
+int prologue_plan(const sp3_step_prologue_desc& d, ProloguePlan& pl) {
+  SP3_CHECK(d.n_colsum >= 0 && d.n_colsum <= SP3_PROLOGUE_MAX_COLSUM && d.n_copies >= 0 && d.n_copies <= SP3_PROLOGUE_MAX_COPIES,
+            "sp3_step_prologue: %d column-sum jobs (<= %d), %d copies (<= %d)", d.n_colsum, SP3_PROLOGUE_MAX_COLSUM, d.n_copies, SP3_PROLOGUE_MAX_COPIES);
+  SP3_CHECK(d.n_colsum + d.n_copies + (d.state ? 1 : 0) > 0, "sp3_step_prologue: no job");
+  int n = 0;
+  pl.start[0] = 0;
+  auto add = [&](int kind, int index, int64_t blocks) { pl.kind[n] = kind; pl.index[n] = index; pl.start[n + 1] = pl.start[n] + (int)blocks; ++n; };
+  if (d.n_colsum) {
+    SP3_CHECK(d.rows > 0 && d.M > 0 && d.ld >= d.M && d.append_P >= 0, "sp3_step_prologue: bad column-sum geometry rows=%d M=%d ld=%lld append_P=%d",
+              d.rows, d.M, (long long)d.ld, d.append_P);
+    for (int i = 0; i < d.n_colsum; ++i) {
+      SP3_CHECK(d.S[i] && d.rowz[i] && d.mem_attn[i] && (reinterpret_cast<uintptr_t>(d.rowz[i]) & 15) == 0 && (d.append_P == 0 || d.mem_count[i]),
+                "sp3_step_prologue: column-sum job %d: null pointer, rowz not 16-byte aligned, or append without mem_count", i);
+      add(0, i, ((int64_t)d.M + d.append_P + 63) / 64);
+    }
+  }
+  for (int i = 0; i < d.n_copies; ++i) {
+    SP3_CHECK(d.src[i] && d.dst[i] && d.bytes[i] > 0 && d.bytes[i] % 16 == 0 &&
+              ((reinterpret_cast<uintptr_t>(d.src[i]) | reinterpret_cast<uintptr_t>(d.dst[i])) & 15) == 0,
+              "sp3_step_prologue: copy %d must be non-empty, 16-byte aligned and a multiple of 16 bytes", i);
+    const int64_t per = 1024 * PROLOGUE_COPY_VECS, nb = (d.bytes[i] / 16 + per - 1) / per;
+    add(1, i, nb > 256 ? 256 : nb);
+  }
+  if (d.state) {
+    SP3_CHECK(d.state_M >= 0 && d.state_wm >= 0, "sp3_step_prologue: bad fill level");
+    add(2, 0, 1);
+  }
+  pl.n_jobs = n;
+  for (int i = n + 1; i <= PROLOGUE_JOBS; ++i) pl.start[i] = 0x7fffffff;
+  return 0;
+}
+}
+
+extern "C" int sp3_step_prologue_map(const sp3_step_prologue_desc* dp, int32_t* start, int32_t* kind, int32_t* n_jobs) {
+  SP3_CHECK(dp && start && kind && n_jobs, "sp3_step_prologue_map: null pointer");
+  ProloguePlan pl;
+  if (int rc = prologue_plan(*dp, pl)) return rc;
+  *n_jobs = pl.n_jobs;
+  for (int i = 0; i <= pl.n_jobs; ++i) start[i] = pl.start[i];
+  for (int i = 0; i < pl.n_jobs; ++i) kind[i] = pl.kind[i];
+  return 0;
+}
+
+extern "C" int sp3_step_prologue(const sp3_step_prologue_desc* dp, void* stream) {
+  SP3_CHECK(dp != nullptr, "sp3_step_prologue: null descriptor");
+  ProloguePlan pl;
+  if (int rc = prologue_plan(*dp, pl)) return rc;
+  PrologueArgs a;
+  a.d = *dp;
+  const int blocks = pl.start[pl.n_jobs];
+  for (int i = 0; i <= PROLOGUE_JOBS; ++i) a.start[i] = pl.start[i];
+  hipLaunchKernelGGL(step_prologue_kernel, dim3(blocks), dim3(1024), 0, ST(stream), a);
+  SP3_LAUNCH_CHECK("sp3_step_prologue");
+  return 0;
+}
+
 extern "C" int sp3_mem_append(float* count, float* attn, int M, int P, void* stream) {
   SP3_CHECK(count && attn && M >= 0 && P > 0, "sp3_mem_append: bad arguments");
   hipLaunchKernelGGL(mem_append_kernel, dim3((M + P + 255) / 256), dim3(256), 0, ST(stream), count, attn, M, P);
diff --git a/spann3r_amd/engine.py b/spann3r_amd/engine.py
--- a/spann3r_amd/engine.py
+++ b/spann3r_amd/engine.py
@@ -615,7 +615,7 @@
         ops.upsample2x(oc, up, B=B, H=H, W_=W_, C_=F, outH=OH, outW=OW)
         return up, OH, OW
 
-    def dpt_head(self, dec, B, nh, nw, num, want_raw=False):
+    def dpt_head(self, dec, B, nh, nw, num, want_raw=False, patch_swap=None):
         self.activate()
         cfg, w = self.cfg, self.w
         F, Lc = cfg.dpt_feat, cfg.dpt_last
@@ -690,8 +690,16 @@
         pts = self.ws("dpt_pts%d" % num, (B, OH, OW, 3))
         conf = self.ws("dpt_conf%d" % num, (B, OH, OW))
         raw = self.ws("dpt_raw%d" % num, (B, OH, OW, 4)) if want_raw else None
-        ops.head_final(c, w[pre + "h4.w"], w[pre + "h4.b"], B * OH * OW, Lc, pts, conf, raw)
+        self.patch_rows_done = patch_swap is not None and self.adt == torch.bfloat16 and ops.head_final_takes_patch_rows(c, Lc)
+        if self.patch_rows_done:
+            ops.head_final_patch(c, w[pre + "h4.w"], w[pre + "h4.b"], B, OH, OW, Lc, pts, conf, raw,
+                                 self.value_patch_rows(B, nh * nw), cfg.patch, patch_swap)
+        else:
+            ops.head_final(c, w[pre + "h4.w"], w[pre + "h4.b"], B * OH * OW, Lc, pts, conf, raw)
         return pts, conf, raw
+
+    def value_patch_rows(self, B, P):
+        return self.wsp("im2col_val", B * P, 3 * self.cfg.patch * self.cfg.patch)
 
     def encode_cur_value_feat(self, tok, out, res, pos32=None):
         self.activate()
@@ -716,7 +724,7 @@
                  ln=ops.LnFold(stA, Cv, w["value_out.s"], 1e-6))
         return out
 
-    def encode_cur_value(self, pts3d, out, res):
+    def encode_cur_value(self, pts3d, out, res, rows_done=False):
         self.activate()
         cfg, w = self.cfg, self.w
         B, H, W_, _ = pts3d.shape
@@ -725,9 +733,10 @@
         P = nh * nw
         R = B * P
         _, pos32, zero_pos = self.positions(B, nh, nw)
-        col = self.wsp("im2col_val", R, 3 * p * p)
-        sb, sy, sx, sc = pts3d.stride()
-        ops.im2col_patch(pts3d, col, B=B, C_=3, H=H, W_=W_, p=p, strides=(sb, sc, sy, sx))
+        col = self.value_patch_rows(B, P)
+        if not rows_done:
+            sb, sy, sx, sc = pts3d.stride()
+            ops.im2col_patch(pts3d, col, B=B, C_=3, H=H, W_=W_, p=p, strides=(sb, sc, sy, sx))
         x, xp, st = self._vit(col, R, B, P, "pospatch", "val", cfg.val_depth, pos32 if cfg.mem_pos_enc else zero_pos, tag="_val")
         ops.gemm(xp, w["value_out.w"], out, M=R, N=E, K=E, lda=E, ldc=E, bias=w["value_out.b"], res1=res, ldr1=E,
                  ln=ops.LnFold(st, E, w["value_out.s"], 1e-6))
diff --git a/spann3r_amd/lib.py b/spann3r_amd/lib.py
--- a/spann3r_amd/lib.py
+++ b/spann3r_amd/lib.py
@@ -91,6 +91,20 @@
         ("gamma_q", C.c_void_p), ("beta_q", C.c_void_p),
         ("eps", C.c_float), ("alpha", C.c_float),
         ("M", C.c_int32), ("P", C.c_int32), ("C", C.c_int32), ("cap", C.c_int32), ("wdtype", C.c_int32), ("state", C.c_void_p),
+    ]
+
+
+PROLOGUE_MAX_COLSUM = PROLOGUE_MAX_COPIES = 8
+
+
+class StepPrologueDesc(C.Structure):
+    _fields_ = [
+        ("S", C.c_void_p * PROLOGUE_MAX_COLSUM), ("rowz", C.c_void_p * PROLOGUE_MAX_COLSUM),
+        ("mem_attn", C.c_void_p * PROLOGUE_MAX_COLSUM), ("mem_count", C.c_void_p * PROLOGUE_MAX_COLSUM),
+        ("src", C.c_void_p * PROLOGUE_MAX_COPIES), ("dst", C.c_void_p * PROLOGUE_MAX_COPIES), ("bytes", C.c_int64 * PROLOGUE_MAX_COPIES),
+        ("ld", C.c_int64), ("state", C.c_void_p),
+        ("n_colsum", C.c_int32), ("n_copies", C.c_int32), ("rows", C.c_int32), ("M", C.c_int32), ("append_P", C.c_int32),
+        ("thresh", C.c_float), ("state_M", C.c_int32), ("state_wm", C.c_int32),
     ]
 
 
@@ -134,6 +148,8 @@
     "sp3_colsum_accum": [C.c_void_p, C.c_int64, C.c_int, C.c_int, C.c_void_p, C.c_void_p],
     "sp3_cos_sim": [C.c_void_p, C.c_void_p, C.c_int, C.c_int, C.c_int, C.c_void_p, C.c_void_p, C.c_void_p],
     "sp3_mem_append": [C.c_void_p, C.c_void_p, C.c_int, C.c_int, C.c_void_p],
+    "sp3_step_prologue": [C.POINTER(StepPrologueDesc), C.c_void_p],
+    "sp3_step_prologue_map": [C.POINTER(StepPrologueDesc), C.c_void_p, C.c_void_p, C.c_void_p],
     "sp3_bank_state_set": [C.c_void_p, C.c_int, C.c_int, C.c_void_p],
     "sp3_prob_merge": [C.c_void_p, C.c_void_p, C.c_int, C.c_int, C.c_int, C.c_void_p, C.c_void_p],
     "sp3_colsum_prob": [C.c_void_p, C.c_void_p, C.c_int, C.c_int, C.c_int, C.c_void_p, C.c_void_p, C.c_void_p],
@@ -153,6 +169,8 @@
     "sp3_upsample2x_bf16": [C.c_void_p, C.c_void_p, C.c_int, C.c_int, C.c_int, C.c_int, C.c_int, C.c_int, C.c_void_p],
     "sp3_head_final_bf16": [C.c_void_p, C.c_void_p, C.c_void_p, C.c_int64, C.c_int, C.c_void_p, C.c_void_p, C.c_void_p,
                             C.c_void_p],
+    "sp3_head_final_patch_bf16": [C.c_void_p, C.c_void_p, C.c_void_p, C.c_int, C.c_int, C.c_int, C.c_int, C.c_void_p, C.c_void_p, C.c_void_p,
+                                  C.c_void_p, C.c_int, C.c_int, C.c_void_p],
     "sp3_fill_f32": [C.c_void_p, C.c_float, C.c_int64, C.c_void_p],
     "sp3_cast_f32_to_bf16": [C.c_void_p, C.c_void_p, C.c_int64, C.c_void_p],
     "sp3_copy2d_f32": [C.c_void_p, C.c_int64, C.c_void_p, C.c_int64, C.c_int, C.c_int, C.c_void_p],
diff --git a/spann3r_amd/model.py b/spann3r_amd/model.py
--- a/spann3r_amd/model.py
+++ b/spann3r_amd/model.py
@@ -400,14 +400,35 @@
         self._after_write()
         self._push_state()
 
-    def finish_staged(self, similar):
+    def finish_staged(self, similar, copies=()):
         if similar:
             self.events.append("skip")
-            self._flush_attn()
+            self.step_prologue(copies, commit=False)
             return
-        self.commit()
+        self.step_prologue(copies, commit=True)
         self._after_write()
         self._push_state()
+
+    def step_prologue(self, copies, commit, predict_wm=True):
+        pend, self._pending_attn = self._pending_attn, None
+        bk = self.bank
+        colsum = None
+        fuse = commit and pend is not None and pend[2] == self.M
+        if pend is not None:
+            S, ld, M, zk = pend
+            colsum = (list(S), ld, self.P, M, list(zk), self.attn_thresh, list(bk["attn"]), list(bk["count"]), self.P if fuse else 0)
+        state = None
+        if commit and self.state is not None:
+            level = (self.M + self.P, min(self.wm + 1, self.work_mem_size) if predict_wm else self.wm)
+            if level != self._state_pushed:
+                state, self._state_pushed = (self.state,) + level, level
+        if copies or colsum is not None or state is not None:
+            ops.step_prologue(copies, colsum, state)
+        if commit:
+            if not fuse:
+                for b in range(self.B):
+                    ops.mem_append(bk["count"][b], bk["attn"][b], self.M, self.P)
+            self.M += self.P
 
     def _after_write(self):
         self.wm += 1
@@ -733,12 +754,13 @@
             st[2].wait_stream(main)
             with torch.cuda.stream(st[2]):
                 pts2, conf2, _ = eng.dpt_head(dec2, B, self.hh, self.hw, 2)
-        pts1, conf1, _ = eng.dpt_head(dec1, B, self.hh, self.hw, 1)
+        pts1, conf1, _ = eng.dpt_head(dec1, B, self.hh, self.hw, 1, patch_swap=None if eng.cfg.use_feat else self.swap)
         if eng.cfg.use_feat:
             eng.encode_cur_value_feat(dec1[-1], self.v, self.k1,
                                       pos32=eng.positions(B, self.nh, self.nw)[1] if eng.cfg.mem_pos_enc else None)
         else:
-            eng.encode_cur_value(pts1.swapaxes(1, 2) if self.swap else pts1, self.v, self.k1)
+            eng.encode_cur_value(pts1.swapaxes(1, 2) if self.swap else pts1, self.v, self.k1,
+                                 rows_done=eng.patch_rows_done)
         mem.stage_write(self.k1, self.v)
         if not self.defer2:
             main.wait_stream(st[2])
@@ -781,18 +803,16 @@
         outs = self._step_outputs(srcs)
         copies = list(zip(srcs, outs))
         copies += list(post_copies() if callable(post_copies) else post_copies)
-        for c0 in range(0, len(copies), 8):
-            ops.copy_multi(copies[c0:c0 + 8])
         res1 = {"pts3d": outs[0], "conf": outs[1]}
         res2 = {} if pts2 is None else {"pts3d": outs[2], "conf": outs[3]}
         if self.swap:
             res1 = {k: v.swapaxes(1, 2) for k, v in res1.items()}
             res2 = {k: v.swapaxes(1, 2) for k, v in res2.items()}
         if self.training:
-            mem.commit()
+            mem.step_prologue(copies, commit=True, predict_wm=False)
             mem._push_state()
         else:
-            mem.finish_staged(mem.sim_verdict() if need_sim else False)
+            mem.finish_staged(mem.sim_verdict() if need_sim else False, copies)
         return res1, res2
 
 
diff --git a/spann3r_amd/ops.py b/spann3r_amd/ops.py
--- a/spann3r_amd/ops.py
+++ b/spann3r_amd/ops.py
@@ -680,6 +680,58 @@
     _timed("copy_multi", 0.0, 2.0 * sum(Bt), lambda: L.check(L.load().sp3_copy_multi(n, S, D, Bt, L.stream_ptr()), "sp3_copy_multi"))
 
 
+def _prologue_desc(copies, colsum, state):
+    if len(copies) > L.PROLOGUE_MAX_COPIES or (colsum is not None and len(colsum[0]) > L.PROLOGUE_MAX_COLSUM):
+        raise ValueError("step_prologue: one launch takes up to %d copies and %d batch elements" % (L.PROLOGUE_MAX_COPIES, L.PROLOGUE_MAX_COLSUM))
+    d = L.StepPrologueDesc()
+    nbytes = 0.0
+    d.n_copies = len(copies)
+    for i, (s_, d_) in enumerate(copies):
+        nb = s_.numel() * s_.element_size()
+        if not (s_.is_contiguous() and d_.is_contiguous()) or nb != d_.numel() * d_.element_size():
+            raise ValueError("step_prologue: copy %d must be contiguous and of equal size" % i)
+        d.src[i], d.dst[i], d.bytes[i] = s_.data_ptr(), d_.data_ptr(), nb
+        nbytes += 2.0 * nb
+    if colsum is not None:
+        S, ld, rows, M, rowz, thresh, mem_attn, mem_count, append_P = colsum
+        d.n_colsum = len(S)
+        d.ld, d.rows, d.M, d.thresh, d.append_P = ld, rows, M, float(thresh), append_P
+        for b in range(len(S)):
+            d.S[b], d.rowz[b], d.mem_attn[b] = S[b].data_ptr(), rowz[b].data_ptr(), mem_attn[b].data_ptr()
+            d.mem_count[b] = L.ptr(mem_count[b]) if append_P else None
+        nbytes += 4.0 * rows * M * len(S)
+    if state is not None:
+        t, M_, wm = state
+        d.state, d.state_M, d.state_wm = t.data_ptr(), int(M_), int(wm)
+    return d, nbytes
+
+
+def step_prologue(copies=(), colsum=None, state=None):
+    copies = list(copies)
+    n = L.PROLOGUE_MAX_COPIES
+    nb = len(colsum[0]) if colsum is not None else 0
+    first = True
+    while first or copies or nb > 0:
+        cs = None
+        if colsum is not None and nb > 0:
+            b0 = len(colsum[0]) - nb
+            sl = slice(b0, b0 + L.PROLOGUE_MAX_COLSUM)
+            cs = (colsum[0][sl], colsum[1], colsum[2], colsum[3], colsum[4][sl], colsum[5], colsum[6][sl], colsum[7][sl], colsum[8])
+            nb -= len(cs[0])
+        d, nbytes = _prologue_desc(copies[:n], cs, state if first else None)
+        copies = copies[n:]
+        first = False
+        _timed("step_prologue", 0.0, nbytes, lambda: L.check(L.load().sp3_step_prologue(C.byref(d), L.stream_ptr()), "sp3_step_prologue"))
+
+
+def step_prologue_map(copies=(), colsum=None, state=None):
+    d, _ = _prologue_desc(list(copies), colsum, state)
+    n = L.PROLOGUE_MAX_COLSUM + L.PROLOGUE_MAX_COPIES + 1
+    start, kind, nj = (C.c_int32 * (n + 1))(), (C.c_int32 * n)(), C.c_int32()
+    L.check(L.load().sp3_step_prologue_map(C.byref(d), start, kind, C.byref(nj)), "sp3_step_prologue_map")
+    return list(start[:nj.value + 1]), list(kind[:nj.value])
+
+
 def colsum_softmax(S, ld, rows, M, rowz, thresh, mem_attn, mem_count=None, append_P=0):
     _timed("colsum_softmax", 4.0 * rows * M, 4.0 * rows * M,
            lambda: L.check(L.load().sp3_colsum_softmax(S.data_ptr(), ld, rows, M, rowz.data_ptr(), float(thresh), mem_attn.data_ptr(),
@@ -833,6 +885,19 @@
     return out
 
 
+def head_final_takes_patch_rows(feat, C_):
+    return feat.dtype == torch.bfloat16 and C_ == 128
+
+
+def head_final_patch(feat, w, b, B, OH, OW, C_, pts, conf, raw, patch_rows, p, swap):
+    assert patch_rows.dtype == torch.bfloat16 and patch_rows.M == B * (OH // p) * (OW // p) and patch_rows.K == 3 * p * p
+    pixels = B * OH * OW
+    _timed("head_final", 8.0 * pixels * C_, pixels * (2.0 * C_ + 22.0),
+           lambda: L.check(L.load().sp3_head_final_patch_bf16(feat.data_ptr(), w.data_ptr(), b.data_ptr(), B, OH, OW, C_, pts.data_ptr(),
+                                                              conf.data_ptr(), L.ptr(raw), patch_rows.data_ptr(), p, int(bool(swap)),
+                                                              L.stream_ptr()), "sp3_head_final_patch_bf16"))
+
+
 def head_final(feat, w, b, pixels, C_, pts, conf, raw=None):
     fn = L.load().sp3_head_final_bf16 if feat.dtype == torch.bfloat16 else L.load().sp3_head_final
     _timed("head_final", 8.0 * pixels * C_, pixels * (float(feat.element_size()) * C_ + 16.0),
```

Result: no change. 642.1 frames/s, median of 6 (+0.5%).
